# fabianschenk/REVO

Hardware: AMD Instinct MI355X
Metric: tracked frames/sec at 640x480, 4-level pyramid; ATE vs reference (higher is better)
Workload: dtype f32

## Files before the change

### revo_amd/csrc/revo_batch.hip

```cpp
#include "revo_host_impl.h"

static bool env_defer() {
  return env_int("REVO_EDT_DEFER", 1, 0, 1) && env_int("REVO_DEFER", 2, 0, 3) != 0;
}
extern "C" int revo_batch_create(revo_ctx* c, int n_pairs, revo_batch** out) {
  if (!c || !out || n_pairs <= 0) return fail(REVO_ERR_INVALID_ARG, "bad argument");
  HIPCHECK(hipSetDevice(c->device));
  Partial<revo_batch> b(new revo_batch());
  b->ctx.hold(c); b->n_pairs = n_pairs;
  { FrameSet* fs = nullptr; TRY(frameset_create(c, 2 * n_pairs, false, &fs)); b->fs.reset(fs); }
  TRY(b->stream.create());
  TRY(b->ev0.create(hipEventDefault)); TRY(b->ev1.create(hipEventDefault));
  TRY(b->descs.create());
  TRY(b->trk.create());
  b->cluster = pick_cluster(c, n_pairs);
  b->defer = env_defer();
  TRY(b->d_mail.alloc(mail_bytes(n_pairs, b->cluster) / sizeof(unsigned long long)));
  HIPCHECK(hipMemset(b->d_mail, 0, mail_bytes(n_pairs, b->cluster)));
  for (int f = 0; f < 2 * n_pairs; ++f) b->views.push_back(revo_pyr{c, b->fs.get(), f, false, (f % 2) == 0, 0.0, false, false});
  TRY(b->descs.reserve(n_pairs, b->stream));
  TRY(b->h_flags.alloc(n_pairs));
  for (int i = 0; i < n_pairs; ++i) fill_desc(&b->descs.h[i], &b->views[2 * i], &b->views[2 * i + 1], nullptr, nullptr);
  HIPCHECK(hipStreamSynchronize(c->stream));
  HIPCHECK(hipStreamSynchronize(nullptr));
  *out = b.release();
  return REVO_OK;
}
revo_batch::~revo_batch() {
  hipSetDevice(ctx->device);
  if (stream) hipStreamSynchronize(stream);
}
extern "C" void revo_batch_destroy(revo_batch* b) {
  if (b) HandleDelete()(b);
}

static int batch_wait_tracker(revo_batch* b, hipStream_t s) { return b->trk.wait_elsewhere(s); }
static int batch_wait_build(revo_batch* b, hipStream_t s) {
  return b->defer ? REVO_OK : b->fs->ready.wait_elsewhere(s);
}
static int batch_mark_tracker(revo_batch* b, hipStream_t s) { return b->trk.record(s); }

static int enqueue_batch_tail(revo_batch* b, hipStream_t s) {
  const PyrGeom& g = b->ctx->geom;
  if (b->defer) {
    std::lock_guard<std::mutex> lk(b->fs->edt_mu);
    b->fs->edt_pending = true; b->fs->edt_count = b->n_pairs;
    b->fs->ref_lists_pending = true;
  } else {
    launch_tile_points(g, b->fs->p, b->fs->B, s);
    launch_keyframe(g, b->fs->p, 0, 2, b->n_pairs, s);
  }
  return REVO_OK;
}

static int batch_build(revo_batch* b, const uint8_t* d_bgr, const float* d_depth, const uint16_t* d_depth_u16, float alpha,
                       void* stream, bool borrow) {
  HIPCHECK(hipSetDevice(b->ctx->device));
  hipStream_t s = stream ? (hipStream_t)stream : b->stream;
  TRY(wait_edt_before_rebuild(b->fs.get(), s));
  TRY(batch_wait_tracker(b, s));
  enqueue_build(b->ctx, b->fs.get(), d_bgr, d_depth, d_depth_u16, alpha, s, borrow, false, 0, -1, b->defer);
  TRY(enqueue_batch_tail(b, s));
  HIPCHECK(hipGetLastError());
  TRY(b->fs->mark_built(s));
  for (auto& v : b->views) { v.table_built = false; v.ref_list_built = false; }
  return REVO_OK;
}
static int batch_build_f32(revo_batch* b, const uint8_t* d_bgr, const float* d_depth, void* stream, bool borrow) {
  if (!b || !d_bgr || !d_depth) return fail(REVO_ERR_INVALID_ARG, "null argument");
  return batch_build(b, d_bgr, d_depth, nullptr, 0.f, stream, borrow);
}
extern "C" int revo_batch_build(revo_batch* b, const uint8_t* d_bgr, const float* d_depth, void* stream) {
  return batch_build_f32(b, d_bgr, d_depth, stream, false);
}
extern "C" int revo_batch_build_borrow(revo_batch* b, const uint8_t* d_bgr, const float* d_depth, void* stream) {
  return batch_build_f32(b, d_bgr, d_depth, stream, true);
}

static int batch_upload_init(revo_batch* b, const float* h_init_RT, hipStream_t s) {
  if (!h_init_RT && b->identity_uploaded) return REVO_OK;
  b->identity_uploaded = (h_init_RT == nullptr);
  TRY(b->descs.reserve(b->n_pairs, s));
  for (int i = 0; i < b->n_pairs; ++i) {
    PairDesc& d = b->descs.h[i];
    if (h_init_RT) { memcpy(d.R, h_init_RT + 12 * i, sizeof(float) * 9); memcpy(d.T, h_init_RT + 12 * i + 9, sizeof(float) * 3); }
    else { memset(d.R, 0, sizeof(d.R)); d.R[0] = d.R[4] = d.R[8] = 1.f; memset(d.T, 0, sizeof(d.T)); }
  }
  return b->descs.upload(b->n_pairs, s);
}

extern "C" int revo_batch_prepare(revo_batch* b, void* stream) {
  if (!b) return fail(REVO_ERR_INVALID_ARG, "null argument");
  HIPCHECK(hipSetDevice(b->ctx->device));
  hipStream_t s = stream ? (hipStream_t)stream : b->stream;
  return run_pending_edt(b->ctx, b->fs.get(), s);
}

extern "C" int revo_batch_track_only(revo_batch* b, const float* h_init_RT, revo_pair_result* d_results, void* stream) {
  if (!b || !d_results) return fail(REVO_ERR_INVALID_ARG, "null argument");
  HIPCHECK(hipSetDevice(b->ctx->device));
  hipStream_t s = stream ? (hipStream_t)stream : b->stream;
  TRY(batch_wait_tracker(b, s));
  int rc = batch_upload_init(b, h_init_RT, s);
  if (rc) return rc;
  TrackParams tp = b->ctx->tp;
  tp.eval_only = 0;
  TRY(batch_wait_build(b, s));
  TRY(run_pending_edt(b->ctx, b->fs.get(), s));
  b->last_results = d_results;
  rc = chained_track_launch(b->ctx->device, b->ctx->knobs.track_depth, s, [&](unsigned* d_resident) {
    if (b->tev0) (void)hipEventRecord(b->tev0, s);
    const int n_wg = launch_track(b->descs.d, tp, d_results, nullptr, b->n_pairs, b->d_mail, &b->mail_epoch, b->cluster, d_resident, s);
    if (b->tev1) (void)hipEventRecord(b->tev1, s);
    b->tev0 = b->tev1 = nullptr;
    return n_wg;
  });
  if (rc) return rc;
  return batch_mark_tracker(b, s);
}
extern "C" void revo_batch_time_next_grid_(revo_batch* b, void* ev0, void* ev1) {
  if (b) { b->tev0 = (hipEvent_t)ev0; b->tev1 = (hipEvent_t)ev1; }
}

extern "C" int revo_batch_build_u16(revo_batch* b, const uint8_t* d_bgr, const uint16_t* d_depth_raw,
                                    double depth_scale_factor, void* stream) {
  if (!b || !d_bgr || !d_depth_raw) return fail(REVO_ERR_INVALID_ARG, "null argument");
  if (!(depth_scale_factor > 0.0)) return fail(REVO_ERR_INVALID_ARG, "depth_scale_factor must be positive");
  return batch_build(b, d_bgr, nullptr, d_depth_raw, (float)(1.0f / depth_scale_factor), stream, false);
}

extern "C" int revo_batch_track(revo_batch* b, const uint8_t* d_bgr, const float* d_depth, const float* h_init_RT,
                                revo_pair_result* d_results, void* stream) {
  int rc = revo_batch_build(b, d_bgr, d_depth, stream);
  if (rc) return rc;
  return revo_batch_track_only(b, h_init_RT, d_results, stream);
}

extern "C" int revo_batch_sync(revo_batch* b, void* stream) {
  if (!b) return fail(REVO_ERR_INVALID_ARG, "null batch");
  HIPCHECK(hipSetDevice(b->ctx->device));
  hipStream_t s = stream ? (hipStream_t)stream : b->stream;
  HIPCHECK(hipStreamSynchronize(s));
  if (b->fs->edt_pending) { int rc2 = run_pending_edt(b->ctx, b->fs.get(), s); if (rc2) return rc2; HIPCHECK(hipStreamSynchronize(s)); }
// ... 1 lines not shown
    TRY(batch_wait_tracker(b, s));
    HIPCHECK(hipMemcpyAsync(b->h_flags, b->last_results, sizeof(revo_pair_result) * b->n_pairs, hipMemcpyDeviceToHost, s));
    HIPCHECK(hipStreamSynchronize(s));
    b->last_results = nullptr;
    for (int i = 0; i < b->n_pairs; ++i)
      if (b->h_flags[i].flags & 8)
        return fail(REVO_ERR_HIP, "tracker: pair " + std::to_string(i) + ": the workgroups of the pair could not exchange "
                    "partial sums in time (device shared with another process?) -- its pose is not valid");
  }
  return REVO_OK;
}

int infows_create(int n, bool own_out, std::unique_ptr<InfoWs>* out) {
  Partial<InfoWs> w(new InfoWs());
  w->n = n;
  TRY(w->descs.reserve(n, nullptr));
  TRY(w->rt.reserve(n, nullptr));
  TRY(w->d_part.alloc(INFO_PART_DOUBLES * INFO_MAX_GROUPS * (size_t)n));
  TRY(w->d_cnt.alloc(INFO_MAX_GROUPS * (size_t)n));
  TRY(w->d_ticket.alloc(align_up((size_t)n, 4)));
  if (own_out) {
    TRY(w->d_out.alloc(n));
    TRY(w->h_out.alloc(n));
  }
  TRY(w->rt.create());
  TRY(w->ev_done.create());
  out->reset(w.release());
  return REVO_OK;
}
InfoParams info_params(const TrackParams& tp, int lvl) {
  InfoParams ip;
  ip.fx = tp.cam[lvl].fx; ip.fy = tp.cam[lvl].fy; ip.cx = tp.cam[lvl].cx; ip.cy = tp.cam[lvl].cy;
  ip.w = tp.cam[lvl].w; ip.h = tp.cam[lvl].h;
  ip.edge_distance = tp.edge_distance[lvl]; ip.huber_edge = tp.huber_edge;
  ip.use_edge_filter = tp.use_edge_filter; ip.level = lvl;
  return ip;
}
int infows_upload_rt(InfoWs* w, int n, const float* h_RT, hipStream_t s) {
  TRY(w->rt.reserve(n, s));
  for (int i = 0; i < n; ++i) {
    memcpy(w->rt.h[i].v, h_RT + 12 * i, sizeof(float) * 12);
    memset(w->rt.h[i].v + 12, 0, sizeof(float) * 4);
  }
  return w->rt.upload(n, s);
}

extern "C" int revo_batch_pair_info(revo_batch* b, const revo_pair_result* d_results, const float* h_RT, int lvl,
                                    revo_pair_info* d_info, void* stream) {
  if (!b || !d_info) return fail(REVO_ERR_INVALID_ARG, "null argument");
  if ((d_results != nullptr) == (h_RT != nullptr)) return fail(REVO_ERR_INVALID_ARG, "exactly one of d_results and h_RT must be given");
  if ((uintptr_t)d_info % 16) return fail(REVO_ERR_INVALID_ARG, "d_info is not 16-byte aligned");
  revo_ctx* c = b->ctx;
  if (lvl < 0 || lvl >= c->geom.n_levels) return fail(REVO_ERR_LEVEL, "level out of range");
  HIPCHECK(hipSetDevice(c->device));
  hipStream_t s = stream ? (hipStream_t)stream : b->stream;
  if (!b->info_ws) {
    TRY(infows_create(b->n_pairs, false, &b->info_ws));
    HIPCHECK(hipMemcpy(b->info_ws->descs.d, b->descs.h, sizeof(PairDesc) * b->n_pairs, hipMemcpyHostToDevice));
  }
  InfoWs* w = b->info_ws.get();
  TRY(batch_wait_tracker(b, s));
  if (h_RT) TRY(infows_upload_rt(w, b->n_pairs, h_RT, s));
  TRY(batch_wait_build(b, s));
  TRY(run_pending_edt(c, b->fs.get(), s));
  InfoParams ip;
  { std::lock_guard<std::mutex> lk(c->mu); ip = info_params(c->tp, lvl); }
  launch_pair_info(w->descs.d, h_RT ? (const void*)w->rt.d : (const void*)d_results, h_RT ? 16 : (int)(sizeof(revo_pair_result) / 4),
                   h_RT ? 12 : (int)(offsetof(revo_pair_result, flags) / 4), ip, b->n_pairs, w->d_part, w->d_cnt, w->d_ticket, d_info, s);
  HIPCHECK(hipGetLastError());
  return batch_mark_tracker(b, s);
}

extern "C" int revo_batch_profile_build(revo_batch* b, const uint8_t* d_bgr, const float* d_depth, int reps, revo_stage_times* out) {
  if (!b || !d_bgr || !d_depth || !out || reps <= 0) return fail(REVO_ERR_INVALID_ARG, "bad argument");
  revo_ctx* c = b->ctx;
  HIPCHECK(hipSetDevice(c->device));
  hipStream_t s = b->stream;
  TRY(wait_edt_before_rebuild(b->fs.get(), s));
  TRY(batch_wait_tracker(b, s));
  memset(out, 0, sizeof(*out));
  PyrGeom g = c->geom;
  g.frame0 = 0;
  FrameSet* fs = b->fs.get();
  const int B = fs->B, L = g.n_levels;
  fs->p.depth[0] = const_cast<float*>(d_depth);
  struct Stage { const char* name; int a, w; };
  std::vector<Stage> st;
  st.push_back({"k_gray_depth", 0, 0});
  for (int l = 1; l < L; ++l) st.push_back({"k_pyrdown_gray", l, 1});
  st.push_back({"k_canny_nms4", 0, 0});
  st.push_back({"hysteresis", 0, 0});
  st.push_back({"k_fill", 0, 0});
  const bool stage = c->knobs.stage_edge_depths && fs->p.stage[0] != nullptr && L > 1;
  PyrGeom gp = g;
  gp.pts_staged = stage ? 1 : 0;
  if (stage) st.push_back({"k_edge_prefix", 0, 0});
  for (int l = 1; l < L; ++l) st.push_back({"k_pyrdown_depth", l, 2});
  st.push_back({"k_tile_count", 0, 1});
  st.push_back({"k_pts_tiles", 0, 2});
  st.push_back({"k_edt_cols", 0, 1});
  st.push_back({"k_edt_rows", 0, 2});
  const int n = (int)st.size();
  if (n > REVO_MAX_STAGES) return fail(REVO_ERR_CAPACITY, "too many stages");
  std::vector<OwnedEvent> ev(n + 1);
  for (auto& e : ev) TRY(e.create(hipEventDefault));
  std::vector<double> sum(n, 0.0);
  for (int r = 0; r < reps; ++r) {
    HIPCHECK(hipEventRecord(ev[0], s));
    for (int i = 0; i < n; ++i) {
      const std::string nm = st[i].name;
      if (nm == "k_gray_depth") launch_gray_depth(g, fs->p, d_bgr, d_depth, nullptr, 0.f, B, s);
      else if (nm == "k_pyrdown_gray") launch_pyrdown(g, fs->p, st[i].a, B, s, 1);
      else if (nm == "k_pyrdown_depth") launch_pyrdown(g, fs->p, st[i].a, B, s, 2, stage);
      else if (nm == "k_edge_prefix") launch_edge_prefix(g, fs->p, B, s);
      else if (nm == "k_canny_nms4") launch_canny_nms(g, fs->p, B, s);
      else if (nm == "hysteresis") launch_hyst(g, fs->p, B, s);
      else if (nm == "k_fill") launch_fill(g, fs->p, B, s);
      else if (nm == "k_tile_count" || nm == "k_pts_tiles") launch_tile_points(gp, fs->p, B, s, st[i].w);
      else launch_keyframe(g, fs->p, 0, 2, b->n_pairs, s, st[i].w);
      HIPCHECK(hipGetLastError());
      HIPCHECK(hipEventRecord(ev[i + 1], s));
    }
    HIPCHECK(hipStreamSynchronize(s));
    for (int i = 0; i < n; ++i) {
      float ms = 0.f;
      HIPCHECK(hipEventElapsedTime(&ms, ev[i], ev[i + 1]));
      sum[i] += ms * 1e3;
    }
  }
  out->n = n;
  for (int i = 0; i < n; ++i) {
    out->us[i] = (float)(sum[i] / reps);
    if (std::string(st[i].name).rfind("k_pyrdown", 0) == 0) snprintf(out->name[i], sizeof(out->name[i]), "%s[%d]", st[i].name, st[i].a);
    else snprintf(out->name[i], sizeof(out->name[i]), "%s", st[i].name);
  }
  {
    std::lock_guard<std::mutex> lk(fs->edt_mu);
    fs->edt_pending = false;
    fs->ref_lists_pending = false;
    TRY(fs->edt.record(s));
    fs->ref.recorded = false;
  }
  TRY(fs->mark_built(s));
  for (auto& v : b->views) { v.table_built = false; v.ref_list_built = false; }
  return REVO_OK;
}

extern "C" int revo_batch_frame(revo_batch* b, int frame, revo_pyr** out) {
  if (!b || !out || frame < 0 || frame >= 2 * b->n_pairs) return fail(REVO_ERR_INVALID_ARG, "bad frame index");
  *out = &b->views[frame];
  return REVO_OK;
}

extern "C" int revo_batch_time_tracker(revo_batch* b, const float* h_init_RT, revo_pair_result* d_results, void* stream,
                                       int reps, float* ms_mean) {
  if (!b || !d_results || !ms_mean || reps <= 0) return fail(REVO_ERR_INVALID_ARG, "bad argument");
  HIPCHECK(hipSetDevice(b->ctx->device));
  hipStream_t s = stream ? (hipStream_t)stream : b->stream;
  TRY(batch_wait_tracker(b, s));
  int rc = batch_upload_init(b, h_init_RT, s);
  if (rc) return rc;
  TrackParams tp = b->ctx->tp;
  tp.eval_only = 0;
  TRY(batch_wait_build(b, s));
  TRY(run_pending_edt(b->ctx, b->fs.get(), s));
  float total = 0.f;
  for (int r = 0; r < reps; ++r) {
    HIPCHECK(hipEventRecord(b->ev0, s));
    rc = chained_track_launch(b->ctx->device, b->ctx->knobs.track_depth, s, [&](unsigned* d_resident) {
      return launch_track(b->descs.d, tp, d_results, nullptr, b->n_pairs, b->d_mail, &b->mail_epoch, b->cluster, d_resident, s);
    });
    if (rc) return rc;
    HIPCHECK(hipEventRecord(b->ev1, s));
    HIPCHECK(hipEventSynchronize(b->ev1));
    float ms = 0.f;
    HIPCHECK(hipEventElapsedTime(&ms, b->ev0, b->ev1));
    total += ms;
  }
  *ms_mean = total / (float)reps;
  return batch_mark_tracker(b, s);
}
```

### revo_amd/csrc/revo_dev.h

```cpp
#pragma once
#include <hip/hip_runtime.h>
#include <stdint.h>
#include "../../include/revo_hip.h"

#define REVO_L REVO_MAX_LEVELS

struct LevelGeom {
  int w, h;
  int npix;
  float fx, fy, cx, cy;
  int patch;
  int hist_w, hist_h;
  int nchunk;
  int chunk_rows;
  int wpr;
  int nms_block_base;
  int has_orig;
  int pix_base;
  int edt_rows;
  int edt_block_base;
  int strip_base;
  int cc_base;
  int band_rows, nbands, band_base;
};

struct PyrGeom {
  int frame0;
  int fstride;
  int n_levels;
  int total_nms_blocks, total_pix, total_edt_blocks, total_strips, total_cc;
  int total_bands, any_banded;
  int hyst_force;
  int hyst_heavy_runs;
  int total_tiles;
  int pts_staged;
  float depth_min, depth_max;
  int canny_low, canny_high;
  int use_edge_hist;
  float n_percentage;
  double fill_thr[REVO_L];
  LevelGeom lv[REVO_L];
};

struct FramePlanes {
  uint8_t* gray[REVO_L];
  float* depth[REVO_L];
  uint2* cs[REVO_L];
  uint8_t* edges[REVO_L];
  uint8_t* edges_orig[REVO_L];
  int* scratch[REVO_L];
  float4* pts[REVO_L];
  float4* pts_trk[REVO_L];
  float* dt[REVO_L];
  float4* table[REVO_L];
  uint8_t* hist[REVO_L];
  int* chunk[REVO_L];
  unsigned* cmask[REVO_L];
  uint8_t* vb[REVO_L];
  int* npts;
  int* hist_nz;
  int* strip_tot;
  uint32_t* ebits[REVO_L];
  int* need_full;
  int* hyst_heavy;
  int* tile_base;
  float* stage[REVO_L];
  unsigned short* epre[REVO_L];
  int* stage_base;
};

struct PairDesc {
  const float4* pts[REVO_L];
  const int* npts;
  const float* dt[REVO_L];
  float R[9];
  float T[3];
};

struct TrackParams {
  int pyr_min_lvl, pyr_max_lvl;
  int lvl_begin, lvl_end;
  int check_init;
  int eval_only;
  int kspec[REVO_L];
  int redundant_n;
  float lambda_success_fac, lambda_fail_fac;
  float lambda_initial[REVO_L], step_size_min[REVO_L], convergence_eps[REVO_L];
  int max_its[REVO_L];
  float edge_distance[REVO_L];
  float huber_edge;
  int use_edge_filter;
  struct { float fx, fy, cx, cy; int w, h; } cam[REVO_L];
  int exact_sums;
};

struct EvalOut {
  float A[36];
  float b[6];
  float error;
  float mean_err;
  float sum_w, sum_u;
  int good, bad;
};

#define REVO_MAX_WIDTH 2048
#define NMS_ROWS 6
#define EDT_ROW_PX 1280
#define EDT_ROW_THREADS (EDT_ROW_PX / 4)
#ifndef REVO_HYST_LDS_MAX
#define REVO_HYST_LDS_MAX 158720
#endif
#ifndef TRACK_THREADS
#define TRACK_THREADS 512
#endif
#ifndef TRACK_MAX_CLUSTER
#define TRACK_MAX_CLUSTER 32
#endif
#define TRACK_KMAX 4
#define TRACK_NVAL 48
#define TRACK_NVAL_X 132
#define TRACK_MAIL_NVAL TRACK_NVAL_X

void launch_gray_depth(const PyrGeom& g, const FramePlanes& p, const uint8_t* d_bgr, const float* d_depth_f32,
                       const uint16_t* d_depth_u16, float u16_alpha, int B, hipStream_t s);
void launch_pyrdown(const PyrGeom& g, const FramePlanes& p, int lvl, int B, hipStream_t s, int parts = 3, bool stage_edges = false);
void launch_edge_prefix(const PyrGeom& g, const FramePlanes& p, int B, hipStream_t s);
void launch_canny_nms(const PyrGeom& g, const FramePlanes& p, int B, hipStream_t s);
void launch_hyst(const PyrGeom& g, const FramePlanes& p, int B, hipStream_t s);
void launch_fill(const PyrGeom& g, const FramePlanes& p, int B, hipStream_t s);
void launch_compact(const PyrGeom& g, const FramePlanes& p, int B, hipStream_t s);
void launch_tile_points(const PyrGeom& g, const FramePlanes& p, int B, hipStream_t s, int which = 3);
void launch_pyrdown_bgr(const uint8_t* src, int w, int h, uint8_t* dst, hipStream_t s);
void launch_colored_pcl(const PyrGeom& g, const FramePlanes& p, int frame, int lvl, int dense, const uint8_t* bgr_lvl,
                        int* chunk, unsigned* cmask, int* total, int cap, float* out8, hipStream_t s);
void launch_keyframe(const PyrGeom& g, const FramePlanes& p, int f0, int fstride, int count, hipStream_t s, int which = 3);
int launch_track(const PairDesc* d_descs, const TrackParams& prm, revo_pair_result* d_out, EvalOut* d_eval,
                 int n_pairs, unsigned long long* d_mail, unsigned* epoch_io, int cluster, unsigned* d_resident, hipStream_t s);
void launch_track_gate(unsigned* d_resident, unsigned want, hipStream_t s);
int launch_track_one(const PairDesc& desc, const TrackParams& prm, revo_pair_result* out, EvalOut* eval_out,
                     unsigned long long* d_mail, unsigned* epoch_io, int cluster, unsigned* seq_ptr, unsigned seq_val,
                     unsigned* d_resident, hipStream_t s);
void launch_solve6(const float* d_Ab , int n, float* d_x , hipStream_t s);
int track_blocks_per_cu();
void launch_grad_table(const PyrGeom& g, const FramePlanes& p, int f0, int fstride, int count, hipStream_t s);
struct VoteArgs { float RT[3][12]; const float4* pts[3]; const int* n[3]; };
void launch_vote(const PyrGeom& g, const FramePlanes& curr, int curr_frame, int lvl, int n_clouds, const VoteArgs& va,
                 int* d_marks , int* d_hist8 , unsigned* d_done ,
                 int* h_out8 , unsigned seq_val, int use_orig_edges,
                 hipStream_t s);
void launch_copy_cloud(float4* dst, const float4* src, int* dst_n, const int* src_n, hipStream_t s);
struct VoteDesc {
  float RT[3][12]; const float4* pts[3]; const int* n[3]; int n_clouds;
  const uint8_t* edges; const float* depth;
  int* marks; int* hist8; unsigned* done;
  int* host_out;
};
struct CloudCopyDesc { float4* dst; const float4* src; int* dst_n; const int* src_n; };
struct CopySeg { const void* src; void* dst; size_t bytes; };
void launch_vote_multi(const PyrGeom& g, int lvl, int n, const VoteDesc* d_descs, unsigned seq_val, hipStream_t s);
void launch_copy_cloud_multi(int n, const CloudCopyDesc* d_descs, hipStream_t s);
void launch_copy_segments(int n, const CopySeg* d_segs, hipStream_t s);

#define INFO_THREADS 256
#define INFO_CHUNK 1024
#define INFO_MAX_GROUPS 32
#define INFO_PART_DOUBLES 64
struct InfoParams {
  float fx, fy, cx, cy;
  int w, h;
  float edge_distance, huber_edge;
  int use_edge_filter, level;
};
static inline int info_groups(int npix) {
  const int g = (npix + 8 * INFO_CHUNK - 1) / (8 * INFO_CHUNK);
  return g < 1 ? 1 : (g > INFO_MAX_GROUPS ? INFO_MAX_GROUPS : g);
}
void launch_pair_info(const PairDesc* d_descs, const void* d_pose, int pose_stride, int flag_word, const InfoParams& prm,
                      int n_pairs, double* d_part, int* d_cnt, unsigned* d_ticket, revo_pair_info* d_out, hipStream_t s);
```

### revo_amd/csrc/revo_frame.hip

```cpp
#include "revo_host_impl.h"

typedef unsigned v4u __attribute__((ext_vector_type(4)));
__global__ void __launch_bounds__(256) k_upload_rows(uint8_t* __restrict__ dst, const uint8_t* __restrict__ src, size_t src_stride,
                                                     size_t row_bytes, int rows) {
  const size_t vec = row_bytes / 16, tail0 = vec * 16;
  for (int y = blockIdx.y; y < rows; y += gridDim.y) {
    const uint8_t* s = src + (size_t)y * src_stride;
    uint8_t* d = dst + (size_t)y * row_bytes;
    const bool aligned = (((uintptr_t)s | (uintptr_t)d) & 15) == 0;
    if (aligned) {
      for (size_t i = blockIdx.x * blockDim.x + threadIdx.x; i < vec; i += (size_t)gridDim.x * blockDim.x)
        ((v4u*)d)[i] = __builtin_nontemporal_load((const v4u*)s + i);
      for (size_t i = tail0 + blockIdx.x * blockDim.x + threadIdx.x; i < row_bytes; i += (size_t)gridDim.x * blockDim.x) d[i] = s[i];
    } else {
      for (size_t i = blockIdx.x * blockDim.x + threadIdx.x; i < row_bytes; i += (size_t)gridDim.x * blockDim.x) d[i] = s[i];
    }
  }
}
static hipError_t upload_rows(void* dst, const void* src, size_t src_stride, size_t row_bytes, int rows, int max_blocks, hipStream_t s) {
  void* dsrc = nullptr;
  hipError_t e = hipHostGetDevicePointer(&dsrc, const_cast<void*>(src), 0);
  if (e != hipSuccess) { (void)hipGetLastError(); return e; }
  if (src_stride == row_bytes) {
    const size_t bytes = row_bytes * rows;
// ... 41 lines not shown
    std::lock_guard<std::mutex> lk(c->mu);
    c->framesets_created += 1;
  }
  const size_t brow = (size_t)w * 3, drow = (size_t)w * (is_u16 ? 2 : 4);
  hipStream_t bs = c->build_stream;
  auto page_locked = [](const void* p) {
    hipPointerAttribute_t at;
    if (hipPointerGetAttributes(&at, p) != hipSuccess) { (void)hipGetLastError(); return false; }
    return at.type == hipMemoryTypeHost;
  };
  const bool direct = c->knobs.direct_h2d && page_locked(bgr) && page_locked(depth) &&
                      page_locked(bgr + (size_t)(h - 1) * bgr_stride + brow - 1) &&
                      page_locked((const char*)depth + (size_t)(h - 1) * depth_stride + drow - 1);
  sec.lap(1);
  if (direct) {
    {
      std::lock_guard<std::mutex> lk(c->mu);
      if (!c->frame_copy_stream) TRY(c->frame_copy_stream.create());
    }
    TRY(fs->h2d.create());
    hipStream_t cs = c->frame_copy_stream;
    TRY(fs->ready.wait(cs));
    TRY(fs->wait_previous_users(cs));
    sec.lap(6);
    if (c->knobs.h2d_kernel && upload_rows(fs->d_bgr, bgr, bgr_stride, brow, h, c->knobs.upload_blocks, cs) == hipSuccess) {}
    else if (bgr_stride == brow) HIPCHECK(hipMemcpyAsync(fs->d_bgr, bgr, brow * h, hipMemcpyHostToDevice, cs));
    else HIPCHECK(hipMemcpy2DAsync(fs->d_bgr, brow, bgr, bgr_stride, brow, h, hipMemcpyHostToDevice, cs));
    sec.lap(7);
    if (c->knobs.h2d_kernel && upload_rows(fs->d_depth, depth, depth_stride, drow, h, c->knobs.upload_blocks, cs) == hipSuccess) {}
    else if (depth_stride == drow) HIPCHECK(hipMemcpyAsync(fs->d_depth, depth, drow * h, hipMemcpyHostToDevice, cs));
    else HIPCHECK(hipMemcpy2DAsync(fs->d_depth, drow, depth, depth_stride, drow, h, hipMemcpyHostToDevice, cs));
    sec.lap(8);
    HIPCHECK(hipEventRecord(fs->h2d, cs));
    sec.lap(9);
    HIPCHECK(hipStreamWaitEvent(bs, fs->h2d, 0));
    sec.lap(2);
    TRY(wait_event_polled(fs->h2d));
    sec.lap(3);
  } else {
    TRY(fs->ready.sync());
    for (int y = 0; y < h; ++y) memcpy(fs->h_bgr + (size_t)y * brow, bgr + (size_t)y * bgr_stride, brow);
    for (int y = 0; y < h; ++y) memcpy((char*)fs->h_depth.p + (size_t)y * drow, (const char*)depth + (size_t)y * depth_stride, drow);
    TRY(fs->wait_previous_users(bs));
    HIPCHECK(hipMemcpyAsync(fs->d_bgr, fs->h_bgr, brow * h, hipMemcpyHostToDevice, bs));
    HIPCHECK(hipMemcpyAsync(fs->d_depth, fs->h_depth, drow * h, hipMemcpyHostToDevice, bs));
  }
  const float alpha = is_u16 ? (float)(1.0f / scale) : 0.0f;
  enqueue_build(c, fs, fs->d_bgr, is_u16 ? nullptr : fs->d_depth, is_u16 ? (const uint16_t*)fs->d_depth : nullptr, alpha, bs, true);
  HIPCHECK(hipGetLastError());
  TRY(fs->mark_built(bs));
  sec.lap(4);
  revo_pyr* p = new revo_pyr{c, fs, 0, true, false, ts, false, false};
  ctx_ref(c);
  *out = p;
  return REVO_OK;
}

extern "C" int revo_pyramid_create(revo_ctx* ctx, const uint8_t* bgr, size_t bgr_stride, const float* depth_m,
                                   size_t depth_stride, double timestamp, revo_pyr** out) {
  return pyramid_create_common(ctx, bgr, bgr_stride, depth_m, depth_stride, false, 1.0, timestamp, out);
}
extern "C" int revo_pyramid_create_u16(revo_ctx* ctx, const uint8_t* bgr, size_t bgr_stride, const uint16_t* depth_raw,
                                       size_t depth_stride, double depth_scale_factor, double timestamp, revo_pyr** out) {
  if (!(depth_scale_factor > 0)) return fail(REVO_ERR_INVALID_ARG, "depth_scale_factor must be > 0");
  return pyramid_create_common(ctx, bgr, bgr_stride, depth_raw, depth_stride, true, depth_scale_factor, timestamp, out);
}

extern "C" void revo_pyramid_destroy(revo_pyr* p) {
  if (!p) return;
  if (p->owns_fs) {
    hipSetDevice(p->ctx->device);
    std::lock_guard<std::mutex> lk(p->ctx->mu);
    p->fs->release_to(p->ctx->pool, p->ctx->stream, p->ctx->vote_stream);
  }
  revo_ctx* c = p->owns_fs ? p->ctx : nullptr;
  delete p;
  if (c) ctx_unref(c);
}

extern "C" int revo_pyramid_make_keyframe(revo_pyr* p) {
  if (!p) return fail(REVO_ERR_INVALID_ARG, "null pyramid");
  HIPCHECK(hipSetDevice(p->ctx->device));
  TRY(wait_ready(p->ctx, p));
  if (!p->dt_ready) launch_keyframe(p->ctx->geom, p->fs->p, p->frame, 1, 1, p->ctx->stream);
  HIPCHECK(hipGetLastError());
  p->dt_ready = false;
  p->is_kf = true;
  p->table_built = false;
  return REVO_OK;
}
extern "C" int revo_pyramid_prepare_keyframe_(revo_pyr* p) {
  if (!p) return fail(REVO_ERR_INVALID_ARG, "null pyramid");
  if (!p->owns_fs || p->is_kf || p->dt_ready) return REVO_OK;
  HIPCHECK(hipSetDevice(p->ctx->device));
  TRY(wait_ready(p->ctx, p));
  launch_keyframe(p->ctx->geom, p->fs->p, p->frame, 1, 1, p->ctx->stream);
  HIPCHECK(hipGetLastError());
  p->dt_ready = true;
  return REVO_OK;
}
extern "C" int revo_pyramid_is_keyframe(const revo_pyr* p) { return p && p->is_kf; }
extern "C" double revo_pyramid_timestamp(const revo_pyr* p) { return p ? p->ts : 0.0; }

extern "C" int revo_pyramid_read(revo_pyr* p, revo_plane what, int lvl, void* dst, size_t cap, size_t* count) {
  if (!p) return fail(REVO_ERR_INVALID_ARG, "null pyramid");
  revo_ctx* c = p->ctx;
  HIPCHECK(hipSetDevice(c->device));
  if (lvl < 0 || lvl >= c->geom.n_levels) return fail(REVO_ERR_LEVEL, "level out of range");
  const LevelGeom& v = c->geom.lv[lvl];
  const FramePlanes& P = p->fs->p;
  const size_t f = (size_t)p->frame;
  TRY(wait_ready(c, p));
  HIPCHECK(hipStreamSynchronize(c->stream));
  const void* src = nullptr;
  size_t n = v.npix, esz = 1;
  switch (what) {
    case REVO_PLANE_GRAY: src = P.gray[lvl] + f * v.npix; break;
    case REVO_PLANE_DEPTH: src = P.depth[lvl] + f * v.npix; esz = 4; break;
    case REVO_PLANE_EDGES: src = P.edges[lvl] + f * v.npix; break;
    case REVO_PLANE_EDGES_ORIG:
      src = (v.has_orig ? P.edges_orig[lvl] : P.edges[lvl]) + f * v.npix;
      break;
    case REVO_PLANE_DT:
      if (!p->is_kf) return fail(REVO_ERR_NOT_KEYFRAME, "distance transform not built: call makeKeyframe");
      src = P.dt[lvl] + f * v.npix; esz = 4; break;
    case REVO_PLANE_GRADTABLE:
      if (!p->is_kf) return fail(REVO_ERR_NOT_KEYFRAME, "optimizationStructure not built");
      if (!p->table_built) {
        launch_grad_table(c->geom, P, p->frame, 1, 1, c->stream);
        HIPCHECK(hipGetLastError());
        HIPCHECK(hipStreamSynchronize(c->stream));
        p->table_built = true;
      }
      src = P.table[lvl] + f * v.npix; esz = 16; break;
    case REVO_PLANE_EDGES3D: {
      if (!p->ref_list_built) {
        PyrGeom g1 = c->geom;
        g1.frame0 = p->frame;
        launch_compact(g1, P, 1, c->stream);
        HIPCHECK(hipGetLastError());
        HIPCHECK(hipStreamSynchronize(c->stream));
        p->ref_list_built = true;
      }
      int np = 0;
      HIPCHECK(hipMemcpy(&np, P.npts + f * REVO_L + lvl, sizeof(int), hipMemcpyDeviceToHost));
      n = (size_t)np; src = P.pts[lvl] + f * v.npix; esz = 16; break;
    }
    case REVO_PLANE_EDGES3D_TILED: {
      int np = 0;
      HIPCHECK(hipMemcpy(&np, P.npts + f * REVO_L + lvl, sizeof(int), hipMemcpyDeviceToHost));
      n = (size_t)np; src = P.pts_trk[lvl] + f * v.npix; esz = 16; break;
    }
    case REVO_PLANE_HIST:
      if (v.patch <= 0) { n = 0; src = P.hist[lvl]; break; }
      n = (size_t)v.hist_w * v.hist_h; src = P.hist[lvl] + f * n; break;
    default: return fail(REVO_ERR_INVALID_ARG, "unknown plane");
  }
  if (count) *count = n;
  if (dst) {
    if (n * esz > cap) return fail(REVO_ERR_CAPACITY, "host buffer too small");
    if (n) HIPCHECK(hipMemcpy(dst, src, n * esz, hipMemcpyDeviceToHost));
  }
  return REVO_OK;
}

extern "C" int revo_pyramid_colored_pcl(revo_pyr* p, int lvl, int dense, float* dst8, size_t cap_points, size_t* count) {
  if (!p) return fail(REVO_ERR_INVALID_ARG, "null pyramid");
  revo_ctx* c = p->ctx;
  HIPCHECK(hipSetDevice(c->device));
  if (lvl < 0 || lvl >= c->geom.n_levels) return fail(REVO_ERR_LEVEL, "level out of range");
  if (!(p->owns_fs || p->has_colour) || !p->fs->d_bgr)
    return fail(REVO_ERR_INVALID_ARG, "batch views keep no colour image (rgbFullSize): use revo_pyramid_create");
  TRY(wait_ready(c, p));
  std::lock_guard<std::mutex> lk(c->mu);
  const PyrGeom& g = c->geom;
  const size_t n0 = g.lv[0].npix, slots = (size_t)g.lv[0].w * g.lv[0].nchunk;
  if (!c->d_pcl) {
    size_t off = 0;
    auto take = [&](size_t bytes) { size_t o = off; off += (bytes + 255) & ~(size_t)255; return o; };
    const size_t o_out = take(n0 * 32), o_a = take(n0 / 4 * 3 + 3), o_b = take(n0 / 16 * 3 + 3), o_ch = take(slots * 4),
                 o_m = take(slots * 4), o_t = take(4);
    TRY(c->d_pcl.alloc(off));
    c->d_pcl_out = (float*)(c->d_pcl + o_out);
    c->d_pcl_clr[0] = (uint8_t*)(c->d_pcl + o_a); c->d_pcl_clr[1] = (uint8_t*)(c->d_pcl + o_b);
    c->d_pcl_chunk = (int*)(c->d_pcl + o_ch); c->d_pcl_mask = (unsigned*)(c->d_pcl + o_m); c->d_pcl_total = (int*)(c->d_pcl + o_t);
  }
  hipStream_t s = c->stream;
  const uint8_t* clr = p->fs->d_bgr + (size_t)p->frame * n0 * 3;
  for (int l = 0; l < lvl; ++l) {
    uint8_t* d = c->d_pcl_clr[l & 1];
    launch_pyrdown_bgr(clr, g.lv[l].w, g.lv[l].h, d, s);
    clr = d;
  }
  const int cap = (int)std::min<size_t>(dst8 ? cap_points : 0, (size_t)g.lv[lvl].npix);
  launch_colored_pcl(g, p->fs->p, p->frame, lvl, dense ? 1 : 0, clr, c->d_pcl_chunk, c->d_pcl_mask, c->d_pcl_total,
                     dst8 ? cap : g.lv[lvl].npix, c->d_pcl_out, s);
  HIPCHECK(hipGetLastError());
  int total = 0;
  HIPCHECK(hipMemcpyAsync(&total, c->d_pcl_total, sizeof(int), hipMemcpyDeviceToHost, s));
  HIPCHECK(hipStreamSynchronize(s));
  if (count) *count = (size_t)total;
  if (dst8) {
    if ((size_t)total > cap_points) return fail(REVO_ERR_CAPACITY, "host buffer too small");
    if (total) HIPCHECK(hipMemcpy(dst8, c->d_pcl_out, (size_t)total * 32, hipMemcpyDeviceToHost));
  }
  return REVO_OK;
}

extern "C" int revo_map_source_(revo_pyr* p, MapSource* out) {
  if (!p || !out) return fail(REVO_ERR_INVALID_ARG, "null pyramid");
  revo_ctx* c = p->ctx;
  HIPCHECK(hipSetDevice(c->device));
  if (!(p->owns_fs || p->has_colour) || !p->fs->d_bgr)
    return fail(REVO_ERR_INVALID_ARG, "batch views keep no colour image (rgbFullSize): use revo_pyramid_create");
  TRY(wait_ready(c, p));
  const size_t n0 = c->geom.lv[0].npix, f = (size_t)p->frame;
  out->ctx = c;
  out->depth = p->fs->p.depth[0] + f * n0;
  out->edges = p->fs->p.edges[0] + f * n0;
  out->bgr = p->fs->d_bgr + f * n0 * 3;
  return REVO_OK;
}
extern "C" int revo_map_source_kind_(const revo_pyr* p, const revo_ctx** ctx, int* batch_view) {
  if (!p || !ctx || !batch_view) return fail(REVO_ERR_INVALID_ARG, "null pyramid");
  *ctx = p->ctx;
  *batch_view = (!(p->owns_fs || p->has_colour) || !p->fs->d_bgr) ? 1 : 0;
  return REVO_OK;
}
extern "C" int revo_map_ctx_geom_(const revo_ctx* c, MapCtxGeom* out) {
  if (!c || !out) return fail(REVO_ERR_INVALID_ARG, "null context");
  const LevelGeom& l = c->geom.lv[0];
  *out = MapCtxGeom{c->device, l.w, l.h, l.fx, l.fy, l.cx, l.cy, c->geom.depth_min, c->geom.depth_max, (void*)c->stream};
  return REVO_OK;
}
```

### revo_amd/csrc/revo_host.hip

```cpp
#include "revo_host_impl.h"

static thread_local std::string g_err;
extern "C" const char* revo_last_error(void) { return g_err.c_str(); }
extern "C" const char* revo_version(void) { return "0.1.0 gfx950"; }
extern "C" void revo_set_error_(const char* msg) { g_err = msg ? msg : ""; }

extern "C" void revo_pyr_settings_default(revo_pyr_settings* s) {
  memset(s, 0, sizeof(*s));
  s->width = 640; s->height = 480;
  s->fx = 517.306408f; s->fy = 516.469215f; s->cx = 318.643040f; s->cy = 255.313989f;
  s->pyr_min_lvl = 2; s->pyr_max_lvl = 0;
  s->canny_threshold1 = 150; s->canny_threshold2 = 100;
  s->depth_min = 0.1f; s->depth_max = 5.2f;
  s->use_edge_hist = 1; s->n_percentage = 0.3f;
  s->hist_patch[0] = 20; s->hist_patch[1] = 10; s->hist_patch[2] = 5;
}
extern "C" void revo_opt_settings_default(revo_opt_settings* s) {
  memset(s, 0, sizeof(*s));
  s->lambda_success_fac = 0.5f; s->lambda_fail_fac = 2.0f;
  const float ed[6] = {30, 20, 10, 5, 5, 5};
  for (int i = 0; i < REVO_L; ++i) {
    s->lambda_initial[i] = 0.f; s->step_size_min[i] = 1e-16f; s->convergence_eps[i] = 0.999f;
    s->max_its_per_lvl[i] = 100; s->edge_distance_lvl[i] = ed[i];
  }
// ... 161 lines not shown
  const int prev = (int)((ch.n + TRACK_MAX_DEPTH - 1) % TRACK_MAX_DEPTH), cur = (int)(ch.n % TRACK_MAX_DEPTH);
  if (depth > 1 && ch.n > 0 && ch.has[prev] && ch.st[prev] != s) launch_track_gate(ch.d_resident, ch.started_total, s);
  const int n_wg = launch(f, ch.d_resident);
  HIPCHECK(hipGetLastError());
  ch.started_total += (unsigned)n_wg;
  HIPCHECK(hipEventRecord(ch.ev[cur], s));
  ch.has[cur] = true;
  ch.st[cur] = s;
  ch.n += 1;
  return REVO_OK;
}
extern "C" int revo_debug_gate_timeouts_(int device) {
  TrackChain& ch = g_chain[device & 63];
  std::lock_guard<std::mutex> lk(ch.mu);
  if (!ch.d_resident) return -1;
  unsigned v = 0;
  if (hipMemcpy(&v, ch.d_resident + 1, sizeof(unsigned), hipMemcpyDeviceToHost) != hipSuccess) return -2;
  return (int)v;
}
extern "C" int revo_debug_census_(int device, unsigned out3[3]) {
  TrackChain& ch = g_chain[device & 63];
  std::lock_guard<std::mutex> lk(ch.mu);
  if (!ch.d_resident || !out3) return -1;
  if (hipMemcpy(out3, ch.d_resident, 2 * sizeof(unsigned), hipMemcpyDeviceToHost) != hipSuccess) return -2;
  out3[2] = ch.started_total;
  return 0;
}
int frameset_create(revo_ctx* c, int B, bool with_staging, FrameSet** out, bool host_staging) {
  const PyrGeom& g = c->geom;
  Partial<FrameSet> fs(new FrameSet());
  fs->B = B;
  for (int pass = 0; pass < 2; ++pass) {
    size_t off = 0;
    auto take = [&](size_t bytes) -> void* {
      void* p = pass ? (void*)(fs->blob + off) : nullptr;
      off = align_up(off + bytes, 256);
      return p;
    };
    for (int l = 0; l < g.n_levels; ++l) {
      const LevelGeom& v = g.lv[l];
      const size_t n = (size_t)v.npix * B;
      fs->p.gray[l] = (uint8_t*)take(n);
      fs->p.depth[l] = (float*)take(n * 4);
      fs->p.cs[l] = (uint2*)take((size_t)v.h * v.wpr * 8 * B);
      fs->p.edges[l] = (uint8_t*)take(n);
      fs->p.edges_orig[l] = (uint8_t*)take(n);
      fs->p.scratch[l] = (int*)take(n * 4);
      fs->p.pts[l] = (float4*)take(n * 16);
      fs->p.pts_trk[l] = (float4*)take(n * 16);
      fs->p.dt[l] = (float*)take(n * 4);
      fs->p.table[l] = (float4*)take(n * 16);
      fs->p.hist[l] = (uint8_t*)take((size_t)std::max(1, v.hist_w * v.hist_h) * B);
      fs->p.chunk[l] = (int*)take((size_t)v.w * v.nchunk * B * 4);
      fs->p.cmask[l] = (unsigned*)take((size_t)v.w * v.nchunk * B * 4);
      fs->p.vb[l] = (uint8_t*)take((n + 7) / 8);
      fs->p.ebits[l] = (uint32_t*)take((size_t)v.h * v.wpr * 4 * B);
      if (B > 1 && l < g.n_levels - 1) {
        fs->p.stage[l] = (float*)take(n * 4);
        fs->p.epre[l] = (unsigned short*)take((size_t)v.h * v.wpr * 2 * B);
      }
    }
    fs->own_depth0 = fs->p.depth[0];
    fs->p.npts = (int*)take(sizeof(int) * REVO_L * B);
    fs->p.hist_nz = (int*)take(sizeof(int) * REVO_L * B);
    fs->p.strip_tot = (int*)take(sizeof(int) * (size_t)g.total_strips * B);
    fs->p.tile_base = (int*)take(sizeof(int) * (size_t)g.total_tiles * B);
    fs->p.need_full = (int*)take(sizeof(int) * REVO_L * B);
    fs->p.hyst_heavy = (int*)take(sizeof(int) * B);
    fs->p.stage_base = (int*)take(sizeof(int) * (size_t)g.total_tiles * B);
    if (with_staging) {
      fs->d_bgr = (uint8_t*)take((size_t)g.lv[0].npix * 3 * B);
      fs->d_depth = (float*)take((size_t)g.lv[0].npix * 4 * B);
    }
    if (!pass) {
      fs->blob_bytes = off;
      hipError_t e = hipMalloc((void**)&fs->blob.p, off);
      if (e != hipSuccess) return fail(REVO_ERR_HIP, std::string("hipMalloc: ") + hipGetErrorString(e));
    }
  }
  if (with_staging && host_staging) {
    TRY(fs->h_bgr.alloc((size_t)g.lv[0].npix * 3 * B));
    TRY(fs->h_depth.alloc((size_t)g.lv[0].npix * B));
  }
  for (StreamMark* m : {&fs->ready, &fs->free_trk, &fs->free_vote, &fs->edt, &fs->ref}) TRY(m->create());
  hipMemsetAsync(fs->p.npts, 0, sizeof(int) * REVO_L * B, c->stream);
  HIPCHECK(hipStreamSynchronize(c->stream));
  *out = fs.release();
  return REVO_OK;
}

void enqueue_build(revo_ctx* c, FrameSet* fs, const uint8_t* d_bgr, const float* d_depth_f32, const uint16_t* d_depth_u16,
                   float alpha, hipStream_t s, bool borrow_depth, bool with_points, int frame0, int nframes, bool gray_only) {
  PyrGeom g = c->geom;
  g.frame0 = frame0;
  const int B = nframes < 0 ? fs->B : nframes;
  fs->p.depth[0] = (borrow_depth && d_depth_f32) ? const_cast<float*>(d_depth_f32) : fs->own_depth0;
  launch_gray_depth(g, fs->p, d_bgr, d_depth_f32, d_depth_u16, alpha, B, s);
  for (int l = 1; l < g.n_levels; ++l) launch_pyrdown(g, fs->p, l, B, s, gray_only ? 1 : 3);
  launch_canny_nms(g, fs->p, B, s);
  launch_hyst(g, fs->p, B, s);
  launch_fill(g, fs->p, B, s);
  if (with_points) launch_tile_points(g, fs->p, B, s);
}

extern "C" int revo_ctx_create(int device, const revo_pyr_settings* pyr, const revo_opt_settings* opt,
                               const revo_tracker_settings* trk, revo_ctx** out) {
  if (!pyr || !out) return fail(REVO_ERR_INVALID_ARG, "null argument");
  int ndev = 0;
  if (hipGetDeviceCount(&ndev) != hipSuccess || ndev <= 0)
    return fail(REVO_ERR_HIP, "no HIP device: librevo_hip has no CPU fallback");
  if (device < 0 || device >= ndev) return fail(REVO_ERR_INVALID_ARG, "device ordinal out of range");
  HIPCHECK(hipSetDevice(device));
  Partial<revo_ctx> owner(new revo_ctx());
  revo_ctx* c = owner.get();
  c->device = device;
  c->ps = *pyr;
  c->knobs.track_depth = env_track_depth();
  c->knobs.cluster_one = env_int("REVO_TRACK_CLUSTER_ONE", 0, 0, TRACK_MAX_CLUSTER);
  c->knobs.redundant_one = env_int("REVO_TRACK_REDUNDANT_ONE", 1024, 0, 1 << 30);
  c->knobs.direct_h2d = env_int("REVO_DIRECT_H2D", 1, 0, 1);
  c->knobs.stage_edge_depths = env_int("REVO_STAGE_EDGE_DEPTHS", 0, 0, 1);
  {
    const char* e1 = getenv("REVO_TRACK_KSPEC_ONE");
    const char* eb = getenv("REVO_TRACK_KSPEC");
    const size_t n1 = e1 ? strlen(e1) : 0;
    c->knobs.kspec_one_set = n1 > 0 || !(eb && *eb);
    for (int i = 0; i < REVO_L; ++i) {
      int k = i < 2 ? 3 : TRACK_KMAX;
      if (n1 == 1) k = e1[0] - '0'; else if (n1 > 1) k = e1[std::min<size_t>(i, n1 - 1)] - '0';
      c->knobs.kspec_one[i] = std::max(1, std::min(TRACK_KMAX, k));
    }
  }
  c->knobs.upload_blocks = env_int("REVO_UPLOAD_BLOCKS", 64, 1, 4096);
  c->knobs.h2d_kernel = env_int("REVO_H2D_KERNEL", 0, 0, 1);
  c->knobs.h2d_max_run_mb = env_int("REVO_H2D_MAX_RUN_MB", 64, 1, 4096);
  if (opt) c->os = *opt; else revo_opt_settings_default(&c->os);
  if (trk) c->ts = *trk; else revo_tracker_settings_default(&c->ts);
  std::string why;
  if (build_geom(c->ps, &c->geom, &why)) return fail(REVO_ERR_INVALID_ARG, why);
  build_track_params(c, &c->tp);
  TRY(c->stream.create());
  TRY(c->build_stream.create());
  TRY(c->vote_stream.create());
  TRY(c->ev_vote.create());
  TRY(c->h_desc.alloc(1));
  TRY(c->h_res.alloc(3));
  TRY(c->h_seq.alloc(4));
  memset(c->h_seq, 0, sizeof(unsigned) * 4);
  TRY(c->h_eval.alloc(1));
  hipDeviceProp_t prop;
  HIPCHECK(hipGetDeviceProperties(&prop, device));
  c->num_cus = prop.multiProcessorCount;
  c->blocks_per_cu = std::min(track_blocks_per_cu(), 2);
  TRY(c->d_mail.alloc(mail_bytes(1, TRACK_MAX_CLUSTER) / sizeof(unsigned long long)));
  HIPCHECK(hipMemset(c->d_mail, 0, mail_bytes(1, TRACK_MAX_CLUSTER)));
  size_t maxpix = 0;
  for (int l = 0; l < c->geom.n_levels; ++l) maxpix = std::max(maxpix, (size_t)c->geom.lv[l].npix);
  TRY(c->d_marks.alloc(maxpix));
  TRY(c->d_hist8.alloc(8));
  TRY(c->d_vote_done.alloc(1));
  HIPCHECK(hipMemset(c->d_marks, 0, sizeof(int) * maxpix));
  HIPCHECK(hipMemset(c->d_hist8, 0, sizeof(int) * 8));
  HIPCHECK(hipMemset(c->d_vote_done, 0, sizeof(unsigned)));
  TRY(c->h_hist8.alloc(16));
  memset(c->h_hist8, 0, sizeof(int) * 16);
  HIPCHECK(hipDeviceSynchronize());
  *out = owner.release();
  return REVO_OK;
}

revo_ctx::~revo_ctx() {
  hipSetDevice(device);
  for (hipStream_t s : {(hipStream_t)build_stream, (hipStream_t)stream, (hipStream_t)vote_stream, (hipStream_t)frame_copy_stream})
    if (s) (void)hipStreamSynchronize(s);
  for (auto& p : past) past_free(p);
  for (auto& p : past_pool) past_free(p);
  for (FrameSet* fs : pool) delete fs;
}
void ctx_ref(revo_ctx* c) { c->refs.fetch_add(1); }
void ctx_unref(revo_ctx* c) { if (c->refs.fetch_sub(1) == 1) HandleDelete()(c); }
extern "C" void revo_ctx_destroy(revo_ctx* c) {
  if (!c) return;
  pairs_jobs_release(c);
  ctx_unref(c);
}
extern "C" int revo_ctx_reserve_framesets_(revo_ctx* c, int total) {
  if (!c) return fail(REVO_ERR_INVALID_ARG, "null context");
  HIPCHECK(hipSetDevice(c->device));
  for (;;) {
    {
      std::lock_guard<std::mutex> lk(c->mu);
      if (c->framesets_created >= total) return REVO_OK;
      c->framesets_created += 1;
    }
    FrameSet* fs = nullptr;
    const int rc = frameset_create(c, 1, true, &fs);
    std::lock_guard<std::mutex> lk(c->mu);
    if (rc) { c->framesets_created -= 1; return rc; }
    c->pool.push_back(fs);
  }
}
extern "C" int revo_ctx_device_(const revo_ctx* c) { return c ? c->device : -1; }
extern "C" void revo_ctx_retain_(revo_ctx* c) { if (c) ctx_ref(c); }
extern "C" void revo_ctx_release_(revo_ctx* c) { if (c) ctx_unref(c); }

extern "C" int revo_ctx_set_tracker(revo_ctx* c, const revo_opt_settings* opt, const revo_tracker_settings* trk) {
  if (!c) return fail(REVO_ERR_INVALID_ARG, "null context");
  std::lock_guard<std::mutex> lk(c->mu);
  if (opt) c->os = *opt;
  if (trk) c->ts = *trk;
  const int exact = c->tp.exact_sums;
  build_track_params(c, &c->tp);
  c->tp.exact_sums = exact;
  while (!c->past.empty()) { c->past_pool.push_back(c->past.front()); c->past.pop_front(); }
  return REVO_OK;
}

extern "C" int revo_ctx_histogram_level(const revo_ctx* c) { return c ? c->ts.histogram_level : -1; }

extern "C" int revo_ctx_set_exact_sums(revo_ctx* c, int on) {
  if (!c) return fail(REVO_ERR_INVALID_ARG, "null context");
  std::lock_guard<std::mutex> lk(c->mu);
  c->tp.exact_sums = on ? 1 : 0;
  return REVO_OK;
}
extern "C" int revo_ctx_exact_sums(const revo_ctx* c) { return c ? c->tp.exact_sums : -1; }

extern "C" int revo_ctx_camera(const revo_ctx* c, int lvl, float out6[6]) {
  if (!c || !out6) return fail(REVO_ERR_INVALID_ARG, "null argument");
  if (lvl < 0 || lvl >= c->geom.n_levels) return fail(REVO_ERR_LEVEL, "level out of range");
  const LevelGeom& v = c->geom.lv[lvl];
  out6[0] = v.fx; out6[1] = v.fy; out6[2] = v.cx; out6[3] = v.cy; out6[4] = (float)v.w; out6[5] = (float)v.h;
  return REVO_OK;
}

static void enqueue_list_side(revo_ctx* c, FrameSet* fs, int f0, int fstride, int count, hipStream_t s) {
  PyrGeom gp = c->geom;
  gp.frame0 = f0; gp.fstride = fstride;
  const bool stage = c->knobs.stage_edge_depths && fs->p.stage[0] != nullptr && c->geom.n_levels > 1;
  if (stage) launch_edge_prefix(gp, fs->p, count, s);
  for (int l = 1; l < c->geom.n_levels; ++l) launch_pyrdown(gp, fs->p, l, count, s, 2, stage);
  gp.pts_staged = stage ? 1 : 0;
  launch_tile_points(gp, fs->p, count, s);
}
int run_pending_edt(revo_ctx* c, FrameSet* fs, hipStream_t s, bool need_ref_lists) {
  std::lock_guard<std::mutex> lk(fs->edt_mu);
  bool behind_build = false;
  if (!fs->edt_pending) {
    TRY(fs->edt.wait_elsewhere(s));
  } else {
    TRY(fs->ready.wait(s));
    behind_build = true;
    enqueue_list_side(c, fs, 1, 2, fs->edt_count, s);
    launch_keyframe(c->geom, fs->p, 0, 2, fs->edt_count, s);
    HIPCHECK(hipGetLastError());
    TRY(fs->edt.record(s));
    fs->edt_pending = false;
  }
  if (!need_ref_lists) return REVO_OK;
  if (!fs->ref_lists_pending) return fs->ref.wait_elsewhere(s);
  if (!behind_build) TRY(fs->ready.wait(s));
  enqueue_list_side(c, fs, 0, 2, fs->edt_count, s);
  HIPCHECK(hipGetLastError());
  TRY(fs->ref.record(s));
  fs->ref_lists_pending = false;
  return REVO_OK;
}
int wait_edt_before_rebuild(FrameSet* fs, hipStream_t s) {
  std::lock_guard<std::mutex> lk(fs->edt_mu);
  TRY(fs->edt.wait_elsewhere(s));
  return fs->ref.wait_elsewhere(s);
}
int wait_event_polled(hipEvent_t ev) {
  const auto t0 = std::chrono::steady_clock::now();
  for (unsigned spin = 0;; ++spin) {
    const hipError_t e = hipEventQuery(ev);
    if (e == hipSuccess) return REVO_OK;
    if (e != hipErrorNotReady) { (void)hipGetLastError(); return fail(REVO_ERR_HIP, std::string("hipEventQuery: ") + hipGetErrorString(e)); }
    (void)hipGetLastError();
    for (int k = 0; k < 32; ++k) __builtin_ia32_pause();
    if ((spin & 1023) == 1023 && std::chrono::steady_clock::now() - t0 > std::chrono::seconds(2)) break;
  }
  HIPCHECK(hipEventSynchronize(ev));
  return REVO_OK;
}
static std::atomic<unsigned long long> g_wait_fallbacks{0}, g_wait_max_ns{0}, g_wait_calls{0};
extern "C" void revo_debug_wait_stats_(unsigned long long out[3]) {
  out[0] = g_wait_calls.load(); out[1] = g_wait_fallbacks.load(); out[2] = g_wait_max_ns.load();
}
int wait_seq(hipStream_t s, volatile unsigned* word, unsigned want) {
  static const int spin_limit = env_int("REVO_WAIT_SPINS", 200000, 1000, 2000000000);
  const auto t0 = std::chrono::steady_clock::now();
  g_wait_calls.fetch_add(1, std::memory_order_relaxed);
  auto note = [&]() {
    const unsigned long long ns = (unsigned long long)std::chrono::duration_cast<std::chrono::nanoseconds>(std::chrono::steady_clock::now() - t0).count();
    unsigned long long cur = g_wait_max_ns.load(std::memory_order_relaxed);
    while (ns > cur && !g_wait_max_ns.compare_exchange_weak(cur, ns)) {}
  };
  for (int spin = 0; spin < spin_limit; ++spin) {
    if (*word == want) { std::atomic_thread_fence(std::memory_order_acquire); note(); return REVO_OK; }
    __builtin_ia32_pause();
  }
  g_wait_fallbacks.fetch_add(1, std::memory_order_relaxed);
  HIPCHECK(hipStreamSynchronize(s));
  note();
  if (*word != want) return fail(REVO_ERR_HIP, "a kernel finished without publishing its result");
  return REVO_OK;
}
```

### revo_amd/csrc/revo_host_impl.h

```cpp
#pragma once
#include <hip/hip_runtime.h>

#include <cmath>
#include <cstdio>
#include <chrono>
#include <cstring>
#include <atomic>
#include <deque>
#include <mutex>
#include <string>
#include <vector>

#include "revo_dev.h"
#include "revo_internal.h"
#include "revo_mat4.h"
#include "revo_multi.h"
#include "revo_map.h"

struct FrameSet {
  int B = 0;
  DevMem<char> blob;
  size_t blob_bytes = 0;
  FramePlanes p{};
  float* own_depth0 = nullptr;
  uint8_t* d_bgr = nullptr;
  float* d_depth = nullptr;
  PinnedMem<uint8_t> h_bgr;
  PinnedMem<float> h_depth;
  StreamMark ready;
  std::mutex edt_mu;
  std::atomic<bool> edt_pending{false};
  int edt_count = 0;
  StreamMark edt;
  std::atomic<bool> ref_lists_pending{false};
  StreamMark ref;
  StreamMark free_trk;
  StreamMark free_vote;
  OwnedEvent h2d;
  int wait_previous_users(hipStream_t s) const { TRY(free_trk.wait(s)); return free_vote.wait(s); }
  int mark_built(hipStream_t s) { return ready.record(s); }
  void release_to(std::vector<FrameSet*>& pool, hipStream_t trk, hipStream_t vote) {
    (void)free_trk.record(trk);
    (void)free_vote.record(vote);
    pool.push_back(this);
  }
};

struct InfoRt { float v[16]; };
struct InfoWs {
  int n = 0;
  HostRows<PairDesc> descs;
  HostRows<InfoRt> rt;
  DevMem<double> d_part; DevMem<int> d_cnt; DevMem<unsigned> d_ticket;
  DevMem<revo_pair_info> d_out; PinnedMem<revo_pair_info> h_out;
  OwnedEvent ev_done;
};

struct Past {
  float4* d_pts; int* d_n; int n; float T_w[16]; double ts;
  size_t cap;
};

struct Knobs {
  int track_depth;
  int cluster_one;
  int redundant_one;
  int direct_h2d;
  int h2d_max_run_mb;
  bool kspec_one_set;
  int kspec_one[REVO_L];
  int upload_blocks;
  int h2d_kernel;
  int stage_edge_depths;
};

struct revo_ctx {
  std::atomic<int> refs{1};
  int device;
  Knobs knobs;
  revo_pyr_settings ps; revo_opt_settings os; revo_tracker_settings ts;
  PyrGeom geom;
  TrackParams tp;
  std::mutex mu;
  int framesets_created = 0;
  unsigned seq_next = 1;
  unsigned mail_epoch = 0;
  int num_cus, blocks_per_cu;
  unsigned long long jobs_submitted = 0;
  float* d_pcl_out; uint8_t* d_pcl_clr[2]; int* d_pcl_chunk; unsigned* d_pcl_mask; int* d_pcl_total;
  OwnedStream stream;
  std::unique_ptr<InfoWs> info_ws;
  DevMem<char> d_pcl;
  DevMem<unsigned> d_vote_done; PinnedMem<int> h_hist8; DevMem<int> d_hist8; DevMem<int> d_marks;
  DevMem<unsigned long long> d_mail;
  PinnedMem<unsigned> h_seq;
  PinnedMem<EvalOut> h_eval;
  PinnedMem<revo_pair_result> h_res;
  PinnedMem<PairDesc> h_desc;
  std::vector<FrameSet*> pool;
  OwnedStream build_stream;
  std::vector<Past> past_pool;
  std::deque<Past> past;
  OwnedStream frame_copy_stream;
  std::vector<struct revo_pairs_job*> jobs;
  OwnedStream copy_stream2, copy_stream, pair_streams[2];
  OwnedEvent ev_vote;
  OwnedStream vote_stream;
  ~revo_ctx();
};
void ctx_ref(revo_ctx* c);
void ctx_unref(revo_ctx* c);
struct CtxRef {
  revo_ctx* c = nullptr;
  ~CtxRef() { if (c) ctx_unref(c); }
  void hold(revo_ctx* x) { ctx_ref(x); c = x; }
  revo_ctx* operator->() const { return c; }
  operator revo_ctx*() const { return c; }
};

struct revo_pyr {
  revo_ctx* ctx;
  FrameSet* fs;
  int frame;
  bool owns_fs;
  bool is_kf;
  double ts;
  bool table_built;
  bool ref_list_built;
  bool dt_ready = false;
  bool has_colour = false;
};

struct revo_batch {
  CtxRef ctx;
  int n_pairs = 0;
  std::unique_ptr<FrameSet> fs;
  std::vector<revo_pyr> views;
  OwnedStream stream;
  StreamMark trk;
  OwnedEvent ev1, ev0;
  std::unique_ptr<InfoWs> info_ws;
  DevMem<unsigned long long> d_mail;
  HostRows<PairDesc> descs;
  PinnedMem<revo_pair_result> h_flags;
  unsigned mail_epoch = 0;
  bool identity_uploaded = false;
  int cluster = 1;
  bool defer = true;
  hipEvent_t tev0 = nullptr, tev1 = nullptr;
  const revo_pair_result* last_results = nullptr;
  ~revo_batch();
};

int pick_cluster(const revo_ctx* c, int n_pairs);
int chained_track_launch_(int device, int depth, hipStream_t s, int (*launch)(void* f, unsigned* d_resident), void* f);
template <typename F>
int chained_track_launch(int device, int depth, hipStream_t s, F&& launch) {
  return chained_track_launch_(device, depth, s, [](void* f, unsigned* d) { return (*(std::remove_reference_t<F>*)f)(d); }, (void*)&launch);
}
int wait_seq(hipStream_t s, volatile unsigned* word, unsigned want);
int wait_event_polled(hipEvent_t ev);
int frameset_create(revo_ctx* c, int B, bool with_staging, FrameSet** out, bool host_staging = true);
void enqueue_build(revo_ctx* c, FrameSet* fs, const uint8_t* d_bgr, const float* d_depth_f32, const uint16_t* d_depth_u16,
                   float alpha, hipStream_t s, bool borrow_depth = false, bool with_points = true, int frame0 = 0,
                   int nframes = -1, bool gray_only = false);
int run_pending_edt(revo_ctx* c, FrameSet* fs, hipStream_t s, bool need_ref_lists = false);
int wait_edt_before_rebuild(FrameSet* fs, hipStream_t s);
int decode_track(const revo_pair_result& r, float R[9], float T[3], float* err, int* status, revo_residual_info* info, int32_t* iters);
int past_take(std::vector<Past>& pool, size_t need, size_t cap, Past* out, bool newest = false);
void past_free(Past& p);
int infows_create(int n, bool own_out, std::unique_ptr<InfoWs>* out);
InfoParams info_params(const TrackParams& tp, int lvl);
int infows_upload_rt(InfoWs* w, int n, const float* h_RT, hipStream_t s);
void pairs_jobs_release(revo_ctx* c);

inline size_t align_up(size_t v, size_t a) { return (v + a - 1) / a * a; }
inline size_t mail_bytes(int n_pairs, int cluster) { return sizeof(unsigned long long) * (size_t)n_pairs * 2 * cluster * TRACK_MAIL_NVAL; }

inline void fill_desc(PairDesc* d, const revo_pyr* ref, const revo_pyr* curr, const float* R, const float* T) {
  const PyrGeom& g = ref->ctx->geom;
  memset(d, 0, sizeof(*d));
  for (int l = 0; l < g.n_levels; ++l) {
    d->pts[l] = curr->fs->p.pts_trk[l] + (size_t)curr->frame * g.lv[l].npix;
    d->dt[l] = ref->fs->p.dt[l] + (size_t)ref->frame * g.lv[l].npix;
  }
  d->npts = curr->fs->p.npts + (size_t)curr->frame * REVO_L;
  if (R) memcpy(d->R, R, sizeof(float) * 9); else { d->R[0] = d->R[4] = d->R[8] = 1.f; }
  if (T) memcpy(d->T, T, sizeof(float) * 3);
}

inline int check_pair(const revo_ctx* c, const revo_pyr* ref, const revo_pyr* curr) {
  if (!c || !ref || !curr) return fail(REVO_ERR_INVALID_ARG, "null argument");
  if (ref->ctx != c || curr->ctx != c) return fail(REVO_ERR_INVALID_ARG, "pyramid belongs to another context");
  if (!ref->is_kf) return fail(REVO_ERR_NOT_KEYFRAME, "optimizationStructure not built! (reference frame is not a keyframe)");
  return REVO_OK;
}

inline int wait_ready_on(revo_ctx* c, const revo_pyr* p, hipStream_t s) {
  TRY(p->fs->ready.wait(s));
  return run_pending_edt(c, p->fs, s, (p->frame & 1) == 0);
}
inline int wait_ready(revo_ctx* c, const revo_pyr* p) { return wait_ready_on(c, p, c->stream); }

struct RowCopier {
  hipMemcpyKind kind; int rows; hipStream_t stream; size_t max_run;
  char* dst = nullptr; const char* src = nullptr; size_t bytes = 0;
  hipError_t flush() {
    if (!bytes) return hipSuccess;
    const hipError_t e = hipMemcpyAsync(dst, src, bytes, kind, stream);
    bytes = 0;
    return e;
  }
  hipError_t add(void* d, const void* s, size_t src_stride, size_t row_bytes) {
    if (src_stride != row_bytes) {
      const hipError_t e = flush();
      if (e != hipSuccess) return e;
      return hipMemcpy2DAsync(d, row_bytes, s, src_stride, row_bytes, rows, kind, stream);
    }
    const size_t n = row_bytes * rows;
    if (bytes && bytes + n <= max_run && src + bytes == (const char*)s && dst + bytes == (char*)d) { bytes += n; return hipSuccess; }
    const hipError_t e = flush();
    if (e != hipSuccess) return e;
    dst = (char*)d; src = (const char*)s; bytes = n;
    return hipSuccess;
  }
};

inline void vote_cloud_pose(const float inv[16], const Past& past, float RT[12]) {
  float tf[16];
  mat4_mul(inv, past.T_w, tf);
  for (int cc = 0; cc < 3; ++cc) for (int r = 0; r < 3; ++r) RT[cc * 3 + r] = tf[cc * 4 + r];
  RT[9] = tf[12]; RT[10] = tf[13]; RT[11] = tf[14];
}
inline int vote_decide(const int32_t ov[4], int nframes, float* ratio) {
  const float wts[4] = {0.f, 1.f, 1.25f, 1.5f};
  float overlapMeasure = 0.0f;
  const int hsize = 1 + nframes;
  for (int k = 1; k < hsize; ++k) overlapMeasure += (ov[k] * wts[k]);
  if (ratio) *ratio = nframes >= 3 && ov[0] > 0 ? overlapMeasure / (float)ov[0] : INFINITY;
  return (overlapMeasure >= ov[0] || hsize < 4) ? REVO_TRACKER_STATE_OK : REVO_TRACKER_STATE_NEW_KF;
}
```

### revo_amd/csrc/revo_mdev.hip

```cpp
#include "revo_host_impl.h"

struct revo_mdev {
  CtxRef c;
  int S = 0, cluster = 1, hl = 0;
  TrackParams tp;
  revo_tracker_settings ts;
  std::vector<revo_pyr> kf_views;
  std::vector<FrameSet*> pool, all;
  unsigned mail_epoch = 0;
  unsigned seq = 0;
  std::vector<std::deque<Past>> past;
  std::vector<Past> past_pool;
  size_t cloud_cap = 0;
  OwnedEvent ev_trk, ev_h2d, ev_prod;
  std::unique_ptr<InfoWs> info_ws;
  HostRows<CopySeg> segs;
  HostRows<CloudCopyDesc> cdesc;
  PinnedMem<int> h_vout;
  DevMem<unsigned> d_done; DevMem<int> d_hist8; DevMem<int> d_marks;
  HostRows<VoteDesc> vdesc;
  DevMem<unsigned long long> d_mail;
  PinnedMem<revo_pair_result> h_res; DevMem<revo_pair_result> d_res;
  HostRows<PairDesc> descs;
  std::unique_ptr<FrameSet> kf;
// ... 101 lines not shown
  hipSetDevice(c->device);
  fs->release_to(m->pool, c->stream, c->vote_stream);
}

extern "C" int revo_mdev_track_(revo_mdev* m, int n, MultiTrack* pairs) {
  if (n <= 0) return REVO_OK;
  revo_ctx* c = m->c;
  HIPCHECK(hipSetDevice(c->device));
  hipStream_t s = c->stream;
  FrameSet* waited[64];
  int nw = 0;
  for (int i = 0; i < n; ++i) {
    FrameSet* fs = (FrameSet*)pairs[i].set;
    const revo_pyr curr{c, fs, pairs[i].frame, false, false, 0.0, false, false};
    fill_desc(&m->descs.h[i], &m->kf_views[pairs[i].stream], &curr, pairs[i].R, pairs[i].T);
    bool seen = false;
    for (int k = 0; k < nw && !seen; ++k) seen = waited[k] == fs;
    if (!seen) {
      TRY(fs->ready.wait(s));
      if (nw < 64) waited[nw++] = fs;
    }
  }
  TRY(m->descs.upload(n, s, false));
  if (m->mail_epoch > 0xffffffffu - 4 * 8192u) {
    HIPCHECK(hipMemsetAsync(m->d_mail, 0, mail_bytes(m->S, m->cluster), s));
    m->mail_epoch = 0;
  }
  int rc = chained_track_launch(c->device, c->knobs.track_depth, s, [&](unsigned* d_resident) {
    return launch_track(m->descs.d, m->tp, m->d_res, nullptr, n, m->d_mail, &m->mail_epoch, m->cluster, d_resident, s);
  });
  if (rc) return rc;
  HIPCHECK(hipMemcpyAsync(m->h_res, m->d_res, sizeof(revo_pair_result) * n, hipMemcpyDeviceToHost, s));
  HIPCHECK(hipEventRecord(m->ev_trk, s));
  if ((rc = wait_event_polled(m->ev_trk))) return rc;
  for (int i = 0; i < n; ++i) {
    const revo_pair_result& r = m->h_res[i];
    if (r.flags & 8)
      return fail(REVO_ERR_HIP, "tracker: stream " + std::to_string(pairs[i].stream) + ": the workgroups of the pair could not exchange "
                  "partial sums in time (device shared with another process?) -- its pose is not valid");
    if ((rc = decode_track(r, pairs[i].R, pairs[i].T, nullptr, &pairs[i].status, nullptr, nullptr))) return rc;
  }
  return REVO_OK;
}

extern "C" int revo_mdev_pair_info_enqueue_(revo_mdev* m, int n) {
  if (n <= 0) return REVO_OK;
  revo_ctx* c = m->c;
  HIPCHECK(hipSetDevice(c->device));
  if (!m->info_ws) TRY(infows_create(m->S, true, &m->info_ws));
  InfoWs* w = m->info_ws.get();
  hipStream_t s = c->stream;
  launch_pair_info(m->descs.d, m->d_res, (int)(sizeof(revo_pair_result) / 4), (int)(offsetof(revo_pair_result, flags) / 4),
                   info_params(m->tp, 0), n, w->d_part, w->d_cnt, w->d_ticket, w->d_out, s);
  HIPCHECK(hipGetLastError());
  HIPCHECK(hipMemcpyAsync(w->h_out, w->d_out, sizeof(revo_pair_info) * n, hipMemcpyDeviceToHost, s));
  HIPCHECK(hipEventRecord(w->ev_done, s));
  return REVO_OK;
}
extern "C" int revo_mdev_pair_info_wait_(revo_mdev* m, int n, revo_pair_info* out) {
  if (n <= 0) return REVO_OK;
  if (!m->info_ws) return fail(REVO_ERR_INVALID_ARG, "no information launch to wait for");
  const int rc = wait_event_polled(m->info_ws->ev_done);
  if (rc) return rc;
  memcpy(out, m->info_ws->h_out, sizeof(revo_pair_info) * n);
  return REVO_OK;
}

extern "C" int revo_mdev_vote_(revo_mdev* m, int n, MultiVote* votes) {
  revo_ctx* c = m->c;
  HIPCHECK(hipSetDevice(c->device));
  const int nfh = m->ts.n_frames_hist_voting;
  hipStream_t vs = c->vote_stream;
  TRY(m->vdesc.reserve(m->S, vs));
  int nv = 0, idx[1024];
  const LevelGeom& lv = c->geom.lv[m->hl];
  const int use_orig = lv.has_orig;
  for (int i = 0; i < n; ++i) {
    MultiVote& v = votes[i];
    v.status = REVO_TRACKER_STATE_OK;
    const std::deque<Past>& past = m->past[v.stream];
    if (past.empty() || !m->ts.check_tracking_results) continue;
    FrameSet* fs = (FrameSet*)v.set;
    TRY(fs->ready.wait_elsewhere(vs));
    VoteDesc& d = m->vdesc.h[nv];
    memset(&d, 0, sizeof(d));
    float inv[16];
    mat4_inverse(v.T_w_curr, inv);
    int nframes = 0;
    for (int fr = 0; fr < nfh && fr < (int)past.size() && fr < 3; ++fr) {
      vote_cloud_pose(inv, past[fr], d.RT[fr]);
      d.pts[fr] = past[fr].d_pts;
      d.n[fr] = past[fr].d_n;
      ++nframes;
    }
    d.n_clouds = nframes;
    const size_t f = (size_t)v.frame * lv.npix;
    d.edges = (use_orig ? fs->p.edges_orig[m->hl] : fs->p.edges[m->hl]) + f;
    d.depth = fs->p.depth[m->hl] + f;
    d.marks = m->d_marks + (size_t)v.stream * m->cloud_cap;
    d.hist8 = m->d_hist8 + 8 * v.stream;
    d.done = m->d_done + v.stream;
    d.host_out = m->h_vout + 16 * v.stream;
    idx[nv++] = i;
  }
  if (!nv) return REVO_OK;
  const unsigned seq = ++m->seq ? m->seq : ++m->seq;
  TRY(m->vdesc.upload(nv, vs));
  launch_vote_multi(c->geom, m->hl, nv, m->vdesc.d, seq, vs);
  HIPCHECK(hipGetLastError());
  for (int k = 0; k < nv; ++k) {
    MultiVote& v = votes[idx[k]];
    const int* o = m->h_vout + 16 * v.stream;
    { int rc = wait_seq(vs, (volatile unsigned*)(o + 8), seq); if (rc) return rc; }
    v.status = vote_decide(o + 4, m->vdesc.h[k].n_clouds, nullptr);
  }
  return REVO_OK;
}

extern "C" int revo_mdev_add_clouds_(revo_mdev* m, int n, const MultiFrame* f) {
  if (n <= 0) return REVO_OK;
  revo_ctx* c = m->c;
  HIPCHECK(hipSetDevice(c->device));
  hipStream_t vs = c->vote_stream;
  TRY(m->cdesc.reserve(n, vs));
  const size_t keep = 3 + (size_t)std::max(0, m->ts.n_frames_hist_voting);
  for (int i = 0; i < n; ++i) {
    FrameSet* fs = (FrameSet*)f[i].set;
    TRY(fs->ready.wait_elsewhere(vs));
    Past p{};
    TRY(past_take(m->past_pool, m->cloud_cap, m->cloud_cap, &p, true));
    const size_t fr = (size_t)f[i].frame;
    m->cdesc.h[i] = CloudCopyDesc{p.d_pts, fs->p.pts_trk[m->hl] + fr * m->cloud_cap, p.d_n, fs->p.npts + fr * REVO_L + m->hl};
    p.n = -1;
    memcpy(p.T_w, f[i].T_w, sizeof(float) * 16);
    p.ts = f[i].ts;
    std::deque<Past>& q = m->past[f[i].stream];
    q.push_back(p);
    if (q.size() > keep) { m->past_pool.push_back(q[3]); q.erase(q.begin() + 3); }
  }
  TRY(m->cdesc.upload(n, vs));
  launch_copy_cloud_multi(n, m->cdesc.d, vs);
  HIPCHECK(hipGetLastError());
  return REVO_OK;
}

extern "C" void revo_mdev_clear_past_(revo_mdev* m, int stream, int keep) {
  if (keep < 0) keep = m->ts.n_frames_hist_voting;
  std::deque<Past>& q = m->past[stream];
  while ((int)q.size() > std::max(0, keep)) { m->past_pool.push_back(q.front()); q.pop_front(); }
}

extern "C" int revo_mdev_promote_(revo_mdev* m, int n, const MultiFrame* f) {
  if (n <= 0) return REVO_OK;
  revo_ctx* c = m->c;
  HIPCHECK(hipSetDevice(c->device));
  hipStream_t s = c->stream;
  const PyrGeom& g = c->geom;
  std::vector<CopySeg> segs;
  for (int i = 0; i < n; ++i) {
    FrameSet* src = (FrameSet*)f[i].set;
    TRY(src->ready.wait_elsewhere(s));
    const size_t sf = (size_t)f[i].frame, df = (size_t)f[i].stream;
    const FramePlanes& a = src->p;
    const FramePlanes& b = m->kf->p;
    auto add = [&](const void* sp, void* dp, size_t per_frame) {
      if (per_frame) segs.push_back(CopySeg{(const char*)sp + sf * per_frame, (char*)dp + df * per_frame, per_frame});
    };
    for (int l = 0; l < g.n_levels; ++l) {
      const LevelGeom& v = g.lv[l];
      const size_t np = (size_t)v.npix, words = (size_t)v.h * v.wpr, cols = (size_t)v.w * v.nchunk;
      add(a.gray[l], b.gray[l], np);
      add(a.depth[l], b.depth[l], np * 4);
      add(a.cs[l], b.cs[l], words * 8);
      add(a.edges[l], b.edges[l], np);
      add(a.edges_orig[l], b.edges_orig[l], np);
      add(a.pts_trk[l], b.pts_trk[l], np * 16);
      if (v.patch > 0) add(a.hist[l], b.hist[l], (size_t)v.hist_w * v.hist_h);
      add(a.chunk[l], b.chunk[l], cols * 4);
      add(a.cmask[l], b.cmask[l], cols * 4);
      if (l < g.n_levels - 1) add(a.vb[l], b.vb[l], np / 8);
    }
    add(a.npts, b.npts, sizeof(int) * REVO_L);
    add(a.hist_nz, b.hist_nz, sizeof(int) * REVO_L);
    add(a.strip_tot, b.strip_tot, sizeof(int) * (size_t)g.total_strips);
    add(a.tile_base, b.tile_base, sizeof(int) * (size_t)g.total_tiles);
    add(src->d_bgr, m->kf->d_bgr, (size_t)g.lv[0].npix * 3);
  }
  TRY(m->segs.reserve((int)segs.size(), s));
  memcpy(m->segs.h, segs.data(), sizeof(CopySeg) * segs.size());
  TRY(m->segs.upload((int)segs.size(), s));
  launch_copy_segments((int)segs.size(), m->segs.d, s);
  for (int i = 0; i < n; ++i) {
    launch_keyframe(g, m->kf->p, f[i].stream, 1, 1, s);
    revo_pyr& v = m->kf_views[f[i].stream];
    v.ts = f[i].ts; v.table_built = false; v.ref_list_built = false;
  }
  HIPCHECK(hipGetLastError());
  return REVO_OK;
}

extern "C" revo_pyr* revo_mdev_keyframe_(revo_mdev* m, int stream) { return &m->kf_views[stream]; }
```

### revo_amd/csrc/revo_pyramid.hip

```cpp
#include "revo_dev.h"
#include "revo_nms_px.h"
#include "revo_edt_px.h"
#include <type_traits>

namespace {

#ifdef REVO_BUILD_PRIO
#define BUILD_PRIO() __builtin_amdgcn_s_setprio(REVO_BUILD_PRIO)
#else
#define BUILD_PRIO()
#endif

__device__ __forceinline__ int level_of(const PyrGeom& g, int v, int LevelGeom::*base) {
  int l = 0;
#pragma unroll
  for (int k = 1; k < REVO_L; ++k)
    if (k < g.n_levels && v >= g.lv[k].*base) l = k;
  return l;
}
__device__ __forceinline__ int clampi(int v, int lo, int hi) { return v < lo ? lo : (v > hi ? hi : v); }
__device__ __forceinline__ int reflect101(int i, int n) {
  if (i < 0) i = -i;
  if (i >= n) i = 2 * n - 2 - i;
  return i;
}

__device__ __forceinline__ uint32_t gray4(uint32_t a, uint32_t b, uint32_t c) {
  const int B0 = a & 255, G0 = (a >> 8) & 255, R0 = (a >> 16) & 255, B1 = a >> 24;
  const int G1 = b & 255, R1 = (b >> 8) & 255, B2 = (b >> 16) & 255, G2 = b >> 24;
  const int R2 = c & 255, B3 = (c >> 8) & 255, G3 = (c >> 16) & 255, R3 = c >> 24;
  const uint32_t y0 = (uint32_t)(B0 * 1868 + G0 * 9617 + R0 * 4899 + 8192) >> 14;
  const uint32_t y1 = (uint32_t)(B1 * 1868 + G1 * 9617 + R1 * 4899 + 8192) >> 14;
  const uint32_t y2 = (uint32_t)(B2 * 1868 + G2 * 9617 + R2 * 4899 + 8192) >> 14;
  const uint32_t y3 = (uint32_t)(B3 * 1868 + G3 * 9617 + R3 * 4899 + 8192) >> 14;
  return y0 | (y1 << 8) | (y2 << 16) | (y3 << 24);
}
__global__ void __launch_bounds__(256) k_gray_depth(const uint8_t* __restrict__ bgr, const float* __restrict__ depth_f32,
                                                    const uint16_t* __restrict__ depth_u16, float alpha,
                                                    uint8_t* __restrict__ gray, float* __restrict__ depth_out, int npix, int frame0) {
  BUILD_PRIO();
  const int f = frame0 + blockIdx.z;
  const int g16 = blockIdx.x * 256 + threadIdx.x;
  if (g16 * 16 >= npix) return;
  const uint4* src = reinterpret_cast<const uint4*>(bgr + (size_t)f * npix * 3) + (size_t)g16 * 3;
  const uint4 p = src[0], q = src[1], r = src[2];
  reinterpret_cast<uint4*>(gray + (size_t)f * npix)[g16] =
      make_uint4(gray4(p.x, p.y, p.z), gray4(p.w, q.x, q.y), gray4(q.z, q.w, r.x), gray4(r.y, r.z, r.w));
  if (depth_out == depth_f32) return;
  float4* dst = reinterpret_cast<float4*>(depth_out + (size_t)f * npix) + (size_t)g16 * 4;
  if (depth_u16) {
    const uint4* raw = reinterpret_cast<const uint4*>(depth_u16 + (size_t)f * npix) + (size_t)g16 * 2;
    const uint4 u = raw[0], v = raw[1];
    const uint32_t wds[8] = {u.x, u.y, u.z, u.w, v.x, v.y, v.z, v.w};
#pragma unroll
    for (int k = 0; k < 4; ++k) {
      float4 d;
      d.x = (float)(wds[2 * k] & 0xffff) * alpha + 0.0f;
      d.y = (float)(wds[2 * k] >> 16) * alpha + 0.0f;
      d.z = (float)(wds[2 * k + 1] & 0xffff) * alpha + 0.0f;
      d.w = (float)(wds[2 * k + 1] >> 16) * alpha + 0.0f;
      dst[k] = d;
    }
  } else {
    const float4* in = reinterpret_cast<const float4*>(depth_f32 + (size_t)f * npix) + (size_t)g16 * 4;
    const float4 d0 = in[0], d1 = in[1], d2 = in[2], d3 = in[3];
    dst[0] = d0; dst[1] = d1; dst[2] = d2; dst[3] = d3;
  }
}

struct EdgeStage {
  const uint2* cs;
  const unsigned short* epre;
  const int* base;
  float* out;
  int wpr, tiles_total;
};
template <bool GRAY, bool DEPTH, bool STAGE = false>
__global__ void __launch_bounds__(256) k_pyrdown(const uint8_t* __restrict__ src, int sw, int sh, uint8_t* __restrict__ dst,
                                                 int dw, int dh, const float* __restrict__ dsrc, float* __restrict__ ddst, int frame0,
                                                 int fstride, uint8_t* __restrict__ vsrc, float dmin, float dmax, EdgeStage es) {
  BUILD_PRIO();
  static_assert(!STAGE || DEPTH, "staging rides on the depth half");
  const int f = frame0 + fstride * blockIdx.z;
  src += (size_t)f * sw * sh;
  dst += (size_t)f * dw * dh;
// ... 165 lines not shown
  auto load_raw = [&](int r) -> Raw {
    const uint32_t rr = (uint32_t)clampi(r, 0, h - 1);
    Raw q;
    q.m0 = *reinterpret_cast<const uint32_t*>(gray + (__umul24(rr, (uint32_t)w) + (uint32_t)xo));
    q.prev = *reinterpret_cast<const uint32_t*>(gray + (__umul24(rr, (uint32_t)w) + (uint32_t)o_prev));
    q.next = *reinterpret_cast<const uint32_t*>(gray + (__umul24(rr, (uint32_t)w) + (uint32_t)o_next));
    return q;
  };
  const uint32_t sel_prev = has_prev ? 0x03020100u : 0x04040404u, sel_next = has_next ? 0x03020100u : 0x07070707u;
  auto make_hrow = [&](Raw q) -> HRow4 {
    return hrow4(__builtin_amdgcn_perm(q.m0, q.prev, sel_prev), q.m0, __builtin_amdgcn_perm(q.m0, q.next, sel_next));
  };
  HRow4 H0, H1, H2;
  MRow4 M0, M1, M2;
  DRow4 D0, D1, D2;
  {
    const Raw r0 = load_raw(y0 - 2), r1 = load_raw(y0 - 1), r2 = load_raw(y0), r3 = load_raw(y0 + 1);
    H0 = make_hrow(r0); H1 = make_hrow(r1); H2 = make_hrow(r2);
    mag_row4(H0, H1, H2, has_prev, has_next, active && y0 - 1 >= 0, M0, D0);
    H0 = make_hrow(r3);
  }
  Raw ahead = load_raw(y0 + 2);
  mag_row4(H1, H2, H0, has_prev, has_next, active, M1, D1);
  uint2* out = pl.cs[l] + (size_t)f * h * lv.wpr;
  const uint32_t ow = (uint32_t)y0 * (uint32_t)lv.wpr + (uint32_t)(xg >> 3);
  const int sh = 4 * (threadIdx.x & 7);
  const int low_high = max(g.canny_low, g.canny_high);
  auto emit = [&](int i, uint32_t cb, uint32_t sb) {
    uint32_t cw = cb << sh, sw = sb << sh;
    cw |= (uint32_t)__builtin_amdgcn_update_dpp(0, (int)cw, 0xB1, 0xf, 0xf, true);
    sw |= (uint32_t)__builtin_amdgcn_update_dpp(0, (int)sw, 0xB1, 0xf, 0xf, true);
    cw |= (uint32_t)__builtin_amdgcn_update_dpp(0, (int)cw, 0x4E, 0xf, 0xf, true);
    sw |= (uint32_t)__builtin_amdgcn_update_dpp(0, (int)sw, 0x4E, 0xf, 0xf, true);
    cw |= (uint32_t)__builtin_amdgcn_update_dpp(0, (int)cw, 0x141, 0xf, 0xf, true);
    sw |= (uint32_t)__builtin_amdgcn_update_dpp(0, (int)sw, 0x141, 0xf, 0xf, true);
    if ((threadIdx.x & 7) == 0 && y0 + i < h) out[ow + (uint32_t)(i * lv.wpr)] = make_uint2(cw, sw);
  };
#define NMS_STEP4(i, Ha, Hb, Hc, Ma, Mb, Mc, Db, Dc)                                  \
  {                                                                                   \
    Hc = make_hrow(ahead);                                                            \
    if ((i) < NMS_R - 1) ahead = load_raw(y0 + (i) + 3);                              \
    mag_row4(Ha, Hb, Hc, has_prev, has_next, active && y0 + (i) + 1 < h, Mc, Dc);      \
    uint32_t cb, sb;                                                                  \
    nms_row4(Ma, Mb, minus1_row4(Mb), Mc, minus1_row4(Mc), Db, g.canny_low, low_high, &cb, &sb); \
    emit((i), cb, sb);                                                                \
  }
  NMS_STEP4(0, H2, H0, H1, M0, M1, M2, D1, D2)
  NMS_STEP4(1, H0, H1, H2, M1, M2, M0, D2, D0)
  NMS_STEP4(2, H1, H2, H0, M2, M0, M1, D0, D1)
  NMS_STEP4(3, H2, H0, H1, M0, M1, M2, D1, D2)
  NMS_STEP4(4, H0, H1, H2, M1, M2, M0, D2, D0)
  NMS_STEP4(5, H1, H2, H0, M2, M0, M1, D0, D1)
#undef NMS_STEP4
}

#ifndef HYST_THREADS
#define HYST_THREADS 1024
#endif
__device__ __forceinline__ uint32_t dil3(uint32_t a, uint32_t al, uint32_t ar) {
  return a | __builtin_amdgcn_alignbit(a, al, 31) | __builtin_amdgcn_alignbit(ar, a, 1);
}
__device__ __forceinline__ uint32_t run_fill(uint32_t C, uint32_t S) {
  const uint32_t up = ((C + S) ^ C) & C;
  const uint32_t rC = __builtin_bitreverse32(C), rS = __builtin_bitreverse32(S);
  const uint32_t dn = __builtin_bitreverse32(((rC + rS) ^ rC) & rC);
  return up | dn | S;
}
__device__ __forceinline__ int hist_wide_tile(const uint32_t* row, int pitch, int patch, int last, uint32_t ma, uint32_t mb) {
  int cnt = 0;
  for (int y = 0; y < patch; ++y, row += pitch) {
    cnt += __popc(row[0] & ma) + __popc(row[last] & mb);
    for (int k = 1; k < last; ++k) cnt += __popc(row[k]);
  }
  return cnt;
}

#ifdef REVO_HYST_PROFILE
#define HP(i) if (threadIdx.x == 0) hp[i] = clock64()
#define HA(i) if (threadIdx.x == 0) { const long long now_ = clock64(); ha[i] += now_ - hlast; hlast = now_; }
#else
#define HP(i)
#define HA(i)
#endif
template <bool C_IN_LDS, bool E_GLOBAL = false>
__device__ __forceinline__ void hyst_level(const PyrGeom& g, const FramePlanes& pl, const int l, const int f, uint32_t* s_mem) {
  static_assert(!(C_IN_LDS && E_GLOBAL), "the candidate bitmap is in LDS only when the edge bitmap is");
#ifdef REVO_HYST_PROFILE
  long long hp[12], ha[8], hlast = 0;
  for (int i = 0; i < 12; ++i) hp[i] = 0;
  for (int i = 0; i < 8; ++i) ha[i] = 0;
  int dbg_sweeps = 0, dbg_bands = 0;
#endif
  HP(0);
  const LevelGeom& lv = g.lv[l];
  const int w = lv.w, h = lv.h, wpr = lv.wpr;
  const int pitch = wpr;
  const int nwords = h * wpr;
  const int e_words = (h + 2) * pitch + 2;
  uint32_t* Cl = s_mem;
  uint32_t* Ebase = C_IN_LDS ? s_mem + (REVO_HYST_LDS_MAX / 4 - e_words)
                  : (E_GLOBAL ? reinterpret_cast<uint32_t*>(pl.scratch[l] + (size_t)f * g.lv[l].npix) : s_mem);
  uint32_t* E = Ebase + 1;
  const uint2* cs = pl.cs[l] + (size_t)f * h * wpr;
  const int tid = threadIdx.x;
  for (int i = tid; i < pitch + 1; i += HYST_THREADS) { Ebase[i] = 0u; Ebase[e_words - 1 - i] = 0u; }
  for (int i = tid; i < nwords; i += HYST_THREADS) {
    const uint2 v = cs[i];
    E[pitch + i] = v.y;
    if (C_IN_LDS) Cl[i] = v.x & ~v.y;
  }
  __syncthreads();
  HP(1);
  bool done = false;
#ifdef REVO_HYST_PROFILE
  int dbg_runs = -1, dbg_t = 0, dbg_a = 0;
#endif
  if (C_IN_LDS) {
    unsigned short* Bs = reinterpret_cast<unsigned short*>(Cl + nwords);
    uint32_t* parent = Cl + nwords + (nwords + 2) / 2;
    const int table_words = (int)(REVO_HYST_LDS_MAX / 4) - (nwords + (nwords + 2) / 2);
    const int cap = min(table_words / 2, table_words - e_words);
    const int cap_keep = (table_words - e_words) / 2;
    __shared__ int s_wsum[HYST_THREADS / 64];
    __shared__ int s_total, s_promoted;
#ifdef REVO_HYST_PROFILE
    __shared__ int s_dbg[4];
    if (tid < 4) s_dbg[tid] = 0;
#endif
    auto weak = [&](int wi) -> uint32_t { return Cl[wi]; };
    auto starts = [](uint32_t wk) -> uint32_t { return wk & ~(wk << 1); };
    const float inv_wpr = 1.0f / (float)wpr;
    const uint32_t FLAG = 0x80000000u, IDM = 0x7fffffffu;
#ifdef REVO_HYST_PROFILE
    hlast = clock64();
#endif
    for (int sweep = 0; sweep < 64 && !done; ++sweep) {
#ifdef REVO_HYST_PROFILE
      ++dbg_sweeps;
#endif
      {
        const int wpt = (nwords + HYST_THREADS - 1) / HYST_THREADS;
        const int w0 = min(nwords, tid * wpt), w1 = min(nwords, w0 + wpt);
        int mine = 0;
        for (int wi = w0; wi < w1; ++wi) mine += __popc(starts(weak(wi)));
        int incl = mine;
#pragma unroll
        for (int o = 1; o < 64; o <<= 1) {
          const int v = __shfl_up(incl, o);
          if ((tid & 63) >= o) incl += v;
        }
        __syncthreads();
        if ((tid & 63) == 63) s_wsum[tid >> 6] = incl;
        if (tid == 0) s_promoted = 0;
        __syncthreads();
        int before = incl - mine;
        for (int k = 0; k < (tid >> 6); ++k) before += s_wsum[k];
        if (tid == HYST_THREADS - 1) { s_total = before + mine; Bs[nwords] = (unsigned short)min(65535, before + mine); }
        for (int wi = w0; wi < w1; ++wi) {
          Bs[wi] = (unsigned short)before;
          before += __popc(starts(weak(wi)));
        }
        __syncthreads();
      }
      const int nruns = s_total;
      HA(0);
#ifdef REVO_HYST_PROFILE
      if (sweep == 0) dbg_runs = nruns;
// ... 144 lines not shown
    __syncthreads();
  }
  if (!done) {
    __shared__ unsigned short s_list[HYST_THREADS];
    __shared__ unsigned char s_act[2][HYST_THREADS];
    __shared__ int s_n;
  const int max_strips = HYST_THREADS / wpr;
  const int rpt = (h + max_strips - 1) / max_strips;
  const int nstrips = (h + rpt - 1) / rpt;
  const int n_items = nstrips * wpr;
  s_act[0][tid] = 0; s_act[1][tid] = 0;
  if (tid == 0) s_n = 0;
  __syncthreads();
  int n_list = n_items;
#ifndef REVO_HYST_MAXIT
#define REVO_HYST_MAXIT 8192
#endif
  for (int it = 0; it < REVO_HYST_MAXIT; ++it) {
    const int wb = it & 1;
    bool changed = false;
    if (tid < n_list) {
      const int item = it == 0 ? tid : (int)s_list[tid];
      const int strip = item / wpr, c = item - strip * wpr;
      const int r0 = strip * rpt, r1 = min(h, r0 + rpt) - 1;
      uint32_t* Ec = E + pitch + c;
      const uint32_t lm = c > 0 ? ~0u : 0u, rm = c < wpr - 1 ? ~0u : 0u;
      auto Cat = [&](int r) -> uint32_t { return C_IN_LDS ? (Cl[r * wpr + c] | Ec[r * pitch]) : cs[r * wpr + c].x; };
      uint32_t prev_d = dil3(Ec[(r0 - 1) * pitch], Ec[(r0 - 1) * pitch - 1] & lm, Ec[(r0 - 1) * pitch + 1] & rm);
      uint32_t cur = Ec[r0 * pitch], cl = Ec[r0 * pitch - 1] & lm, cr = Ec[r0 * pitch + 1] & rm;
      for (int r = r0; r <= r1; ++r) {
        const uint32_t nx = Ec[(r + 1) * pitch], nl = Ec[(r + 1) * pitch - 1] & lm, nr = Ec[(r + 1) * pitch + 1] & rm;
        const uint32_t Cw = Cat(r);
        const uint32_t hz = __builtin_amdgcn_alignbit(cur, cl, 31) | __builtin_amdgcn_alignbit(cr, cur, 1);
        const uint32_t F = run_fill(Cw, cur | (Cw & (prev_d | dil3(nx, nl, nr) | hz)));
        if (F != cur) { Ec[r * pitch] = F; changed = true; }
        prev_d = dil3(F, cl, cr);
        cur = nx; cl = nl; cr = nr;
      }
      prev_d = dil3(cur, cl, cr);
      cur = Ec[r1 * pitch]; cl = Ec[r1 * pitch - 1] & lm; cr = Ec[r1 * pitch + 1] & rm;
      for (int r = r1; r >= r0; --r) {
        const uint32_t nx = Ec[(r - 1) * pitch], nl = Ec[(r - 1) * pitch - 1] & lm, nr = Ec[(r - 1) * pitch + 1] & rm;
        const uint32_t Cw = Cat(r);
        const uint32_t hz = __builtin_amdgcn_alignbit(cur, cl, 31) | __builtin_amdgcn_alignbit(cr, cur, 1);
        const uint32_t F = run_fill(Cw, cur | (Cw & (prev_d | dil3(nx, nl, nr) | hz)));
        if (F != cur) { Ec[r * pitch] = F; changed = true; }
        prev_d = dil3(F, cl, cr);
        cur = nx; cl = nl; cr = nr;
      }
      if (changed) s_act[wb][item] = 1;
    }
    if (!__syncthreads_or(changed ? 1 : 0)) break;
    bool act = false;
    if (tid < n_items) {
      const int strip = tid / wpr, c = tid - strip * wpr;
      const unsigned char* a = s_act[wb];
#pragma unroll
      for (int ds = -1; ds <= 1; ++ds)
#pragma unroll
        for (int dc = -1; dc <= 1; ++dc) {
          const int ss = strip + ds, cc = c + dc;
          if (ss >= 0 && ss < nstrips && cc >= 0 && cc < wpr) act = act || a[ss * wpr + cc] != 0;
        }
    }
    const unsigned long long m = __ballot(act);
    int base = 0;
    if ((tid & 63) == 0 && m) base = atomicAdd(&s_n, __popcll(m));
    base = __shfl(base, 0);
    if (act) s_list[base + __popcll(m & ((1ull << (tid & 63)) - 1ull))] = (unsigned short)tid;
    s_act[wb ^ 1][tid] = 0;
    __syncthreads();
    n_list = s_n;
    __syncthreads();
    if (tid == 0) s_n = 0;
  }
  __syncthreads();
  }
  __syncthreads();
  HP(5);
  uint8_t* edges = pl.edges[l] + (size_t)f * lv.npix;
  uint8_t* orig = lv.has_orig ? pl.edges_orig[l] + (size_t)f * lv.npix : nullptr;
  const bool rows16 = (w & 15) == 0;
  const float inv_w = 1.0f / (float)w;
  for (int i = tid; i < lv.npix / 16; i += HYST_THREADS) {
    const int p = i * 16;
    int y = (int)(((float)p + 0.5f) * inv_w);
    y += (y + 1) * w <= p ? 1 : (y * w > p ? -1 : 0);
    const int x = p - y * w;
    uint32_t o[4];
    if (rows16) {
      const uint32_t bits = (E[(y + 1) * pitch + (x >> 5)] >> (x & 31)) & 0xffffu;
#pragma unroll
      for (int q = 0; q < 4; ++q) o[q] = ((((bits >> (4 * q)) & 0xfu) * 0x00204081u) & 0x01010101u) * 0xffu;
    } else {
#pragma unroll
      for (int q = 0; q < 4; ++q) {
        int xx = x + 4 * q, yy = y;
        while (xx >= w) { xx -= w; yy += 1; }
        const uint32_t bits = (E[(yy + 1) * pitch + (xx >> 5)] >> (xx & 31)) & 0xfu;
        o[q] = ((bits * 0x00204081u) & 0x01010101u) * 0xffu;
      }
    }
    const uint4 v = make_uint4(o[0], o[1], o[2], o[3]);
    *reinterpret_cast<uint4*>(edges + p) = v;
    if (orig) *reinterpret_cast<uint4*>(orig + p) = v;
  }
  {
    uint2* csw = pl.cs[l] + (size_t)f * h * wpr;
    for (int i = tid; i < nwords; i += HYST_THREADS) csw[i].y = E[pitch + i];
  }
  HP(6);
  if (lv.patch > 0) {
    const int ntiles = lv.hist_w * lv.hist_h;
    int nz = 0;
    const float inv_hw = 1.0f / (float)lv.hist_w;
    for (int t0 = 0; t0 < ntiles; t0 += HYST_THREADS) {
      const int t = t0 + tid;
      if (t < ntiles) {
        int ty = (int)(((float)t + 0.5f) * inv_hw);
        ty += (ty + 1) * lv.hist_w <= t ? 1 : (ty * lv.hist_w > t ? -1 : 0);
        const int tx = t - ty * lv.hist_w;
        const int xa = tx * lv.patch, xb = xa + lv.patch;
        const int wa = xa >> 5, wb = (xb - 1) >> 5;
        const uint32_t ma = ~0u << (xa & 31), mb = (xb & 31) ? ~0u >> (32 - (xb & 31)) : ~0u;
        const uint32_t m0 = wa == wb ? ma & mb : ma, m1 = wb > wa + 1 ? ~0u : (wb > wa ? mb : 0u), m2 = wb > wa + 1 ? mb : 0u;
        const int o1 = wb > wa ? 1 : 0, o2 = wb > wa + 1 ? 2 : 0;
        const uint32_t* row = E + (ty * lv.patch + 1) * pitch + wa;
        int cnt = 0;
        if (wb - wa > 2) cnt = hist_wide_tile(row, pitch, lv.patch, wb - wa, ma, mb);
        else
        for (int y = 0; y < lv.patch; ++y, row += pitch) cnt += __popc(row[0] & m0) + __popc(row[o1] & m1) + __popc(row[o2] & m2);
        const uint8_t v = (uint8_t)(cnt & 255);
        pl.hist[l][(size_t)f * ntiles + t] = v;
        nz += v != 0;
      }
    }
    __shared__ int s_nz;
    if (tid == 0) s_nz = 0;
    __syncthreads();
    if (nz) atomicAdd(&s_nz, nz);
    __syncthreads();
    if (tid == 0) pl.hist_nz[f * REVO_L + l] = s_nz;
  }
#ifdef REVO_HYST_PROFILE
  HP(7);
  if (threadIdx.x == 0 && l == 0 && f < 64)
    printf("hyst f=%d: load %lld uf_total %lld [scan %lld record %lld link %lld compress %lld flag %lld resolve %lld] runs %d sweeps %d bands %d uf %d rebuild %lld out %lld hist %lld touched %d atomics %d\n", f,
           hp[1] - hp[0], hp[5] - hp[1], ha[0], ha[1], ha[2], ha[3], ha[4], ha[5], dbg_runs, dbg_sweeps, dbg_bands, (int)done, ha[6], hp[6] - hp[5], hp[7] - hp[6], dbg_t, dbg_a);
#endif
}
template <bool C_IN_LDS, bool E_GLOBAL = false>
__global__ void __launch_bounds__(HYST_THREADS) k_hyst(PyrGeom g, FramePlanes pl, int only_flagged, int n_frames) {
  BUILD_PRIO();
  extern __shared__ uint32_t s_mem[];
  const int n_items = g.n_levels * n_frames;
  if (only_flagged) {
    __shared__ int s_any;
    if (threadIdx.x == 0) s_any = 0;
    __syncthreads();
    for (int item = threadIdx.x; item < n_items; item += HYST_THREADS)
      if (pl.need_full[(g.frame0 + item % n_frames) * REVO_L + item / n_frames]) s_any = 1;
    __syncthreads();
    if (!s_any) return;
  }
  for (int item = blockIdx.x; item < n_items; item += gridDim.x) {
    const int l = item / n_frames;
    const int f = g.frame0 + item % n_frames;
    if (only_flagged && !pl.need_full[f * REVO_L + l]) continue;
    hyst_level<C_IN_LDS, E_GLOBAL>(g, pl, l, f, s_mem);
    __syncthreads();
  }
}

#ifndef HB_THREADS
#define HB_THREADS 1024
#endif
#ifndef HB_LDS_WORDS
#define HB_LDS_WORDS 16384
#endif
struct BandRef { int l, R0, R1; };
__device__ __forceinline__ BandRef band_ref(const PyrGeom& g, int bi) {
  int l = 0;
#pragma unroll
  for (int k = 1; k < REVO_L; ++k)
    if (k < g.n_levels && bi >= g.lv[k].band_base) l = k;
  const LevelGeom& lv = g.lv[l];
  const int b = bi - lv.band_base;
  BandRef r;
  r.l = l; r.R0 = b * lv.band_rows; r.R1 = min(lv.h, r.R0 + lv.band_rows);
  return r;
}
__device__ __forceinline__ int band_capb(const LevelGeom& lv) {
  const int hb = lv.band_rows, nwb = hb * lv.wpr;
  const int table_words = HB_LDS_WORDS - (nwb + (nwb + 2) / 2);
  const int e_words = (hb + 2) * lv.wpr + 2;
  int cap = min(table_words / 2, table_words - e_words);
  cap = min(cap, 65535);
  const int h_last = lv.h - (lv.nbands - 1) * lv.band_rows;
  cap = min(cap, ((h_last * lv.w - 4 - 2 * lv.wpr) / 8) * 5);
  return max(cap, 0) & ~31;
}
struct BandRec { int* hdr; int* bs_first; int* bs_last; uint32_t* flags; unsigned short* root; uint32_t* rec; };
__device__ __forceinline__ BandRec band_rec(const FramePlanes& pl, const LevelGeom& lv, int l, int f, int R0, int capb) {
  int* base = pl.scratch[l] + (size_t)f * lv.npix + (size_t)R0 * lv.w;
  BandRec r;
  r.hdr = base; r.bs_first = base + 4; r.bs_last = base + 4 + lv.wpr;
  r.flags = reinterpret_cast<uint32_t*>(base + 4 + 2 * lv.wpr);
  r.root = reinterpret_cast<unsigned short*>(base + 4 + 2 * lv.wpr + capb / 32);
  r.rec = reinterpret_cast<uint32_t*>(base + 4 + 2 * lv.wpr + capb / 32 + capb / 2);
  return r;
}

__device__ __forceinline__ void hyst_band(const PyrGeom& g, const FramePlanes& pl, const BandRef br, const int f, uint32_t* s_mem) {
  __shared__ int s_wsum[HB_THREADS / 64];
  __shared__ int s_total;
  const int l = br.l;
  const LevelGeom& lv = g.lv[l];
  const int h = lv.h, wpr = lv.wpr, pitch = wpr;
  const int hb = br.R1 - br.R0, nwb = hb * wpr, e_words = (hb + 2) * pitch + 2;
  const int tid = threadIdx.x;
  uint32_t* Cl = s_mem;
  uint32_t* Ebase = s_mem + (HB_LDS_WORDS - e_words);
  uint32_t* E = Ebase + 1;
  const uint2* cs = pl.cs[l] + ((size_t)f * h + br.R0) * wpr;
  const int capb = band_capb(lv);
  const BandRec rec_out = band_rec(pl, lv, l, f, br.R0, capb);
  auto load_e = [&](bool with_cl) {
    if (tid == 0) { Ebase[0] = 0u; Ebase[e_words - 1] = 0u; }
    for (int c = tid; c < wpr; c += HB_THREADS) {
      E[c] = br.R0 > 0 ? cs[c - wpr].y : 0u;
      E[(hb + 1) * pitch + c] = br.R1 < h ? cs[nwb + c].y : 0u;
    }
    for (int i0 = tid; i0 < nwb; i0 += 4 * HB_THREADS) {
      uint2 v[4];
#pragma unroll
      for (int k = 0; k < 4; ++k) v[k] = cs[min(i0 + k * HB_THREADS, nwb - 1)];
#pragma unroll
      for (int k = 0; k < 4; ++k) {
        const int i = i0 + k * HB_THREADS;
        if (i < nwb) {
          if (with_cl) { E[pitch + i] = v[k].y; Cl[i] = v[k].x & ~v[k].y; }
          else E[pitch + i] = v[k].y | (v[k].x & ~Cl[i]);
        }
      }
    }
  };
  load_e(true);
  __syncthreads();
  unsigned short* Bs = reinterpret_cast<unsigned short*>(Cl + nwb);
  uint32_t* parent = Cl + nwb + (nwb + 2) / 2;
  const int table_words = HB_LDS_WORDS - (nwb + (nwb + 2) / 2);
  const int cap_keep = (table_words - e_words) / 2;
// ... 82 lines not shown
    }
    __syncthreads();
    for (int me = tid; me < nr; me += HB_THREADS) {
      parent[me] = key_of(find(me));
      rec_out.rec[me] = rec[me];
    }
    __syncthreads();
    if (nr > cap_keep) {
      load_e(false);
      __syncthreads();
    }
    for (int wi = tid; wi < nwb; wi += HB_THREADS) {
      const uint32_t wk = Cl[wi];
      if (!wk) continue;
      int r = (int)(((float)wi + 0.5f) * inv_wpr);
      r += (r + 1) * wpr <= wi ? 1 : (r * wpr > wi ? -1 : 0);
      const int c = wi - r * wpr;
      const uint32_t lm = c > 0 ? ~0u : 0u, rm = c < wpr - 1 ? ~0u : 0u;
      const uint32_t* Xc = E + pitch + wi;
      const uint32_t sd = dil3(Xc[-pitch], Xc[-pitch - 1] & lm, Xc[-pitch + 1] & rm) | dil3(Xc[pitch], Xc[pitch - 1] & lm, Xc[pitch + 1] & rm) |
                          __builtin_amdgcn_alignbit(Xc[0], Xc[-1] & lm, 31) | __builtin_amdgcn_alignbit(Xc[1] & rm, Xc[0], 1);
      if (!(wk & sd)) continue;
      const uint32_t touched = run_fill(wk, wk & sd);
      int me = (int)Bs[wi];
      for (uint32_t m = starts(wk); m; m &= m - 1, ++me)
        if (touched & m & (0u - m)) {
          uint32_t* root = &parent[parent[me] & 0xffffu];
          if (!(*root & FLAG)) atomicOr(root, FLAG);
        }
    }
    __syncthreads();
    for (int wi = tid; wi < nwb; wi += HB_THREADS) {
      const uint32_t wk = Cl[wi];
      if (!wk) continue;
      int me = (int)Bs[wi];
      uint32_t prom = 0;
      for (uint32_t m = starts(wk); m; m &= m - 1, ++me)
        if (parent[parent[me] & 0xffffu] & FLAG) prom |= m & (0u - m);
      if (prom) E[pitch + wi] |= run_fill(wk, prom);
    }
    __syncthreads();
  }
  uint32_t* eb = pl.ebits[l] + ((size_t)f * h + br.R0) * wpr;
  for (int i = tid; i < nwb; i += HB_THREADS) eb[i] = E[pitch + i];
  if (tid == 0) { rec_out.hdr[0] = nr; rec_out.hdr[1] = 0; rec_out.hdr[2] = 1; }
  for (int c = tid; c < wpr; c += HB_THREADS) { rec_out.bs_first[c] = Bs[c]; rec_out.bs_last[c] = Bs[(hb - 1) * wpr + c]; }
  for (int i = tid; i < (nr + 31) / 32; i += HB_THREADS) {
    uint32_t bits = 0;
    for (int k = 0; k < 32; ++k) {
      const int me = 32 * i + k;
      if (me < nr && (int)(parent[me] & 0xffffu) == me && (parent[me] & FLAG)) bits |= 1u << k;
    }
    rec_out.flags[i] = bits;
  }
  for (int me = tid; me < nr; me += HB_THREADS) rec_out.root[me] = (unsigned short)(parent[me] & 0xffffu);
}
__global__ void __launch_bounds__(HB_THREADS) k_hyst_band(PyrGeom g, FramePlanes pl) {
  extern __shared__ uint32_t s_mem[];
  const int nB = gridDim.x / g.total_bands;
  hyst_band(g, pl, band_ref(g, blockIdx.x / nB), g.frame0 + blockIdx.x % nB, s_mem);
}

__device__ __forceinline__ bool hyst_frame_is_heavy(const PyrGeom& g, const FramePlanes& pl, int f) {
  __shared__ int s_cnt[HYST_THREADS / 64];
  const LevelGeom& lv = g.lv[0];
  const int nwords = lv.h * lv.wpr;
  const uint2* cs = pl.cs[0] + (size_t)f * nwords;
  int mine = 0;
  for (int i = threadIdx.x; i < nwords; i += HYST_THREADS) {
    const uint2 v = cs[i];
    const uint32_t wk = v.x & ~v.y;
    mine += __popc(wk & ~(wk << 1));
  }
#pragma unroll
  for (int o = 32; o >= 1; o >>= 1) mine += __shfl_xor(mine, o);
  __syncthreads();
  if ((threadIdx.x & 63) == 0) s_cnt[threadIdx.x >> 6] = mine;
  __syncthreads();
  int total = 0;
#pragma unroll
  for (int k = 0; k < HYST_THREADS / 64; ++k) total += s_cnt[k];
  return total >= g.hyst_heavy_runs;
}
__global__ void __launch_bounds__(HYST_THREADS) k_hyst_mixed(PyrGeom g, FramePlanes pl, int n_frames) {
  static_assert(HB_THREADS == HYST_THREADS, "one workgroup shape for both paths");
  extern __shared__ uint32_t s_mem[];
  const int nb0 = g.lv[0].nbands;
  const int n_band_wg = nb0 * n_frames;
  if ((int)blockIdx.x < n_band_wg) {
    const int f = g.frame0 + blockIdx.x % n_frames;
    if (!hyst_frame_is_heavy(g, pl, f)) return;
    hyst_band(g, pl, band_ref(g, blockIdx.x / n_frames), f, s_mem);
    return;
  }
  const int item = blockIdx.x - n_band_wg;
  const int l = item / n_frames, f = g.frame0 + item % n_frames;
  if (l == 0) {
    const bool heavy = hyst_frame_is_heavy(g, pl, f);
    if (threadIdx.x == 0) pl.hyst_heavy[f] = heavy ? 1 : 0;
    if (heavy) return;
  }
  hyst_level<true>(g, pl, l, f, s_mem);
}

#define HS_THREADS 256
#define HS_MAX_BANDS 32
#define HS_MAX_PAIRS 6144
__global__ void __launch_bounds__(HS_THREADS) k_hyst_seam(PyrGeom g, FramePlanes pl, int mixed) {
  extern __shared__ uint32_t s_fl[];
  __shared__ uint2 s_pair[HS_MAX_PAIRS];
  __shared__ int s_npairs;
  __shared__ int s_changed_band[HS_MAX_BANDS];
  const int nB = mixed ? gridDim.x : gridDim.x / g.n_levels;
  const int l = blockIdx.x / nB;
  const int f = g.frame0 + blockIdx.x % nB;
  const LevelGeom& lv = g.lv[l];
  const int nb = lv.nbands;
  if (nb <= 1 || pl.need_full[f * REVO_L + l]) return;
  if (mixed && !pl.hyst_heavy[f]) return;
  const int wpr = lv.wpr, h = lv.h;
  const int tid = threadIdx.x;
  const int capb = band_capb(lv), fw = capb / 32;
  const uint2* cs = pl.cs[l] + (size_t)f * h * wpr;
  for (int b = 0; b < nb; ++b) {
    const BandRec rb = band_rec(pl, lv, l, f, b * lv.band_rows, capb);
    const int n = (rb.hdr[0] + 31) / 32;
    for (int i = tid; i < fw; i += HS_THREADS) s_fl[b * fw + i] = i < n ? rb.flags[i] : 0u;
  }
  if (tid < HS_MAX_BANDS) s_changed_band[tid] = 0;
  if (tid == 0) s_npairs = 0;
  __syncthreads();
  auto starts = [](uint32_t wk) -> uint32_t { return wk & ~(wk << 1); };
  auto weak_at = [&](int y, int c) -> uint32_t { if (c < 0 || c >= wpr) return 0u; const uint2 v = cs[(size_t)y * wpr + c]; return v.x & ~v.y; };
  for (int item = tid; item < (nb - 1) * wpr; item += HS_THREADS) {
    const int sm = item / wpr, c = item - sm * wpr;
    const int yb = (sm + 1) * lv.band_rows, ya = yb - 1;
    const uint32_t Wa = weak_at(ya, c);
    const uint32_t Wl = weak_at(yb, c - 1), Wm = weak_at(yb, c), Wr = weak_at(yb, c + 1);
    if (!Wa || !(Wm | (Wl >> 31) | (Wr & 1u))) continue;
    const BandRec ra = band_rec(pl, lv, l, f, sm * lv.band_rows, capb);
    const BandRec rbb = band_rec(pl, lv, l, f, yb, capb);
    int ida = ra.bs_last[c];
    const int idm = rbb.bs_first[c], idl = c > 0 ? rbb.bs_first[c - 1] : 0, idr = c < wpr - 1 ? rbb.bs_first[c + 1] : 0;
    for (uint32_t m = starts(Wa); m; m &= m - 1, ++ida) {
      const int bit = __ffs(m) - 1;
      const uint32_t t2 = ~(Wa >> bit);
      const int len = t2 ? __ffs(t2) - 1 : 32 - bit;
      const uint32_t ma = (0xffffffffu >> (32 - len)) << bit;
      int roota = -1;
      for (int side = 0; side < 3; ++side) {
        int idb0; uint32_t Wb, hits;
        if (side == 0) { Wb = Wm; hits = Wm & (ma | (ma << 1) | (ma >> 1)); idb0 = idm; }
        else if (side == 1) { Wb = Wl; hits = (ma & 1u) ? (Wl & 0x80000000u) : 0u; idb0 = idl; }
        else { Wb = Wr; hits = (ma >> 31) ? (Wr & 1u) : 0u; idb0 = idr; }
        while (hits) {
          const int hb2 = __ffs(hits) - 1;
          const uint32_t upto = (2u << hb2) - 1u;
          const int k = __popc(starts(Wb) & upto) - 1;
          const uint32_t gap = ~Wb & upto;
          const int first = gap ? 32 - __clz(gap) : 0;
          const uint32_t t3 = ~(Wb >> first);
          const int lenb = t3 ? __ffs(t3) - 1 : 32 - first;
          hits &= ~((0xffffffffu >> (32 - lenb)) << first);
          if (roota < 0) roota = ra.root[ida];
          const int rootb = rbb.root[idb0 + k];
          const int slot = atomicAdd(&s_npairs, 1);
          if (slot < HS_MAX_PAIRS) s_pair[slot] = make_uint2((uint32_t)sm, (uint32_t)roota | ((uint32_t)rootb << 16));
        }
      }
    }
  }
  __syncthreads();
  const int np = s_npairs;
  if (np > HS_MAX_PAIRS) {
    if (tid == 0) pl.need_full[f * REVO_L + l] = 1;
    return;
  }
  for (int it = 0; it < 65536; ++it) {
    bool changed = false;
    for (int i = tid; i < np; i += HS_THREADS) {
      const uint2 pr = s_pair[i];
      const int sm = (int)pr.x, roota = (int)(pr.y & 0xffffu), rootb = (int)(pr.y >> 16);
      uint32_t* fa = s_fl + sm * fw;
      uint32_t* fb = s_fl + (sm + 1) * fw;
      const bool A = (fa[roota >> 5] >> (roota & 31)) & 1u, Bf = (fb[rootb >> 5] >> (rootb & 31)) & 1u;
      if (A != Bf) {
        if (!A) { atomicOr(&fa[roota >> 5], 1u << (roota & 31)); s_changed_band[sm] = 1; }
        else { atomicOr(&fb[rootb >> 5], 1u << (rootb & 31)); s_changed_band[sm + 1] = 1; }
        changed = true;
      }
    }
    if (!__syncthreads_or(changed ? 1 : 0)) break;
  }
  __syncthreads();
  for (int b = 0; b < nb; ++b) {
    if (!s_changed_band[b]) continue;
    const BandRec rb = band_rec(pl, lv, l, f, b * lv.band_rows, capb);
    const int n = (rb.hdr[0] + 31) / 32;
    for (int i = tid; i < n; i += HS_THREADS) rb.flags[i] = s_fl[b * fw + i];
    if (tid == 0) rb.hdr[1] = 1;
  }
}

#define HO_THREADS 512
__global__ void __launch_bounds__(HO_THREADS) k_hyst_out(PyrGeom g, FramePlanes pl, int mixed) {
  extern __shared__ uint32_t s_mem[];
  const int nB = gridDim.x / (mixed ? g.lv[0].nbands : g.total_bands);
  const BandRef br = band_ref(g, blockIdx.x / nB);
  const int f = g.frame0 + blockIdx.x % nB;
  const int l = br.l;
  if (pl.need_full[f * REVO_L + l]) return;
  if (mixed && !pl.hyst_heavy[f]) return;
  const LevelGeom& lv = g.lv[l];
  const int w = lv.w, h = lv.h, wpr = lv.wpr, pitch = wpr;
  const int hb = br.R1 - br.R0, nwb = hb * wpr;
  const int tid = threadIdx.x;
  uint32_t* E = s_mem;
  uint32_t* eb = pl.ebits[l] + ((size_t)f * h + br.R0) * wpr;
  for (int i = tid; i < nwb; i += HO_THREADS) E[i] = eb[i];
  const BandRec rb = band_rec(pl, lv, l, f, br.R0, band_capb(lv));
  const bool promote = rb.hdr[1] != 0;
  __syncthreads();
  if (promote) {
    const int nr = rb.hdr[0];
    for (int me = tid; me < nr; me += HO_THREADS) {
      const int root = rb.root[me];
      if ((rb.flags[root >> 5] >> (root & 31)) & 1u) {
        const uint32_t rc = rb.rec[me];
        atomicOr(&E[rc >> 10], (0xffffffffu >> (31u - (rc & 31u))) << ((rc >> 5) & 31u));
      }
    }
    __syncthreads();
  }
  uint8_t* edges = pl.edges[l] + (size_t)f * lv.npix + (size_t)br.R0 * w;
  uint8_t* orig = lv.has_orig ? pl.edges_orig[l] + (size_t)f * lv.npix + (size_t)br.R0 * w : nullptr;
  const bool rows16 = (w & 15) == 0;
  const float inv_w = 1.0f / (float)w;
  for (int i = tid; i < hb * w / 16; i += HO_THREADS) {
    const int p = i * 16;
    int y = (int)(((float)p + 0.5f) * inv_w);
    y += (y + 1) * w <= p ? 1 : (y * w > p ? -1 : 0);
    const int x = p - y * w;
    uint32_t o[4];
    if (rows16) {
      const uint32_t bits = (E[y * pitch + (x >> 5)] >> (x & 31)) & 0xffffu;
#pragma unroll
      for (int q = 0; q < 4; ++q) o[q] = ((((bits >> (4 * q)) & 0xfu) * 0x00204081u) & 0x01010101u) * 0xffu;
    } else {
#pragma unroll
      for (int q = 0; q < 4; ++q) {
        int xx = x + 4 * q, yy = y;
        while (xx >= w) { xx -= w; yy += 1; }
        const uint32_t bits = (E[yy * pitch + (xx >> 5)] >> (xx & 31)) & 0xfu;
        o[q] = ((bits * 0x00204081u) & 0x01010101u) * 0xffu;
      }
    }
    const uint4 v = make_uint4(o[0], o[1], o[2], o[3]);
    *reinterpret_cast<uint4*>(edges + p) = v;
    if (orig) *reinterpret_cast<uint4*>(orig + p) = v;
  }
  {
    uint2* csw = pl.cs[l] + ((size_t)f * h + br.R0) * wpr;
    for (int i = tid; i < nwb; i += HO_THREADS) csw[i].y = E[i];
  }
  if (lv.patch > 0) {
    const int ty0 = br.R0 / lv.patch, ty1 = min(lv.hist_h, br.R1 / lv.patch);
    const int ntiles = max(0, ty1 - ty0) * lv.hist_w;
    int nz = 0;
    for (int t = tid; t < ntiles; t += HO_THREADS) {
      const int ty = ty0 + t / lv.hist_w, tx = t % lv.hist_w;
      const int xa = tx * lv.patch, xb = xa + lv.patch;
      const int wa = xa >> 5, wb = (xb - 1) >> 5;
      const uint32_t ma = ~0u << (xa & 31), mb = (xb & 31) ? ~0u >> (32 - (xb & 31)) : ~0u;
      const uint32_t m0 = wa == wb ? ma & mb : ma, m1 = wb > wa + 1 ? ~0u : (wb > wa ? mb : 0u), m2 = wb > wa + 1 ? mb : 0u;
      const int o1 = wb > wa ? 1 : 0, o2 = wb > wa + 1 ? 2 : 0;
      const uint32_t* row = E + (ty * lv.patch - br.R0) * pitch + wa;
      int cnt = 0;
      if (wb - wa > 2) cnt = hist_wide_tile(row, pitch, lv.patch, wb - wa, ma, mb);
      else
      for (int y = 0; y < lv.patch; ++y, row += pitch) cnt += __popc(row[0] & m0) + __popc(row[o1] & m1) + __popc(row[o2] & m2);
      const uint8_t v = (uint8_t)(cnt & 255);
      pl.hist[l][(size_t)f * lv.hist_w * lv.hist_h + (size_t)ty * lv.hist_w + tx] = v;
      nz += v != 0;
    }
#pragma unroll
    for (int o = 32; o > 0; o >>= 1) nz += __shfl_xor(nz, o);
    if ((tid & 63) == 0 && nz) atomicAdd(&pl.hist_nz[f * REVO_L + l], nz);
  }
}

__global__ void __launch_bounds__(1024) k_fill(PyrGeom g, FramePlanes pl, int only_level) {
  BUILD_PRIO();
  const int f = g.frame0 + blockIdx.z;
  const int la = only_level ? only_level : 1, lb = only_level ? only_level + 1 : g.n_levels;
  for (int l = la; l < lb; ++l) {
    const LevelGeom lv = g.lv[l], lf = g.lv[l - 1];
    if (!(g.use_edge_hist && lv.patch > 0 && lf.patch > 0)) continue;
    const float frac = (float)pl.hist_nz[f * REVO_L + l] / (float)(lv.hist_w * lv.hist_h);
    if (frac < g.n_percentage) {
      const uint8_t* top = pl.edges[l - 1] + (size_t)f * lf.npix;
      uint8_t* mod = pl.edges[l] + (size_t)f * lv.npix;
      const uint8_t* hist = pl.hist[l] + (size_t)f * lv.hist_w * lv.hist_h;
      const double thr = g.fill_thr[l];
      const int cw = lf.w / 2, ch = lf.h / 2;
      for (int i = blockIdx.x * 1024 + threadIdx.x; i < cw * ch; i += gridDim.x * 1024) {
        const int y = i / cw, x = i % cw;
        const int yy = 2 * y + 1, xx = 2 * x + 1;
        const int ty = yy / lf.patch, tx = xx / lf.patch;
        if (ty >= lv.hist_h || tx >= lv.hist_w) continue;
        if ((double)hist[(size_t)ty * lv.hist_w + tx] < thr && top[(size_t)yy * lf.w + xx] > 0) {
          mod[(size_t)y * lv.w + x] = 255;
          atomicOr(&(pl.cs[l] + (size_t)f * lv.h * lv.wpr)[(size_t)y * lv.wpr + (x >> 5)].y, 1u << (x & 31));
        }
      }
    }
    __syncthreads();
  }
}

__device__ __forceinline__ uint32_t tile_transpose32(uint32_t v, int r) {
#pragma unroll
  for (int k = 16; k >= 1; k >>= 1) {
    const uint32_t mk = k == 16 ? 0x0000ffffu : k == 8 ? 0x00ff00ffu : k == 4 ? 0x0f0f0f0fu : k == 2 ? 0x33333333u : 0x55555555u;
    const uint32_t t = (uint32_t)__shfl_xor((int)v, k);
    v = (r & k) ? ((v & ~mk) | ((t >> k) & mk)) : ((v & mk) | ((t & mk) << k));
  }
  return v;
}

__device__ __forceinline__ bool depth_ok(float Z, float dmin, float dmax) {
  return isfinite(Z) && Z > dmin && Z < dmax;
}

#define CW_COLS 64
#define CW_LANES 16
#ifndef CW_LANES_COUNT
#define CW_LANES_COUNT 8
#endif
#define CW_MAXCHUNK 64
#define CW_STAGE 4096
template <bool WRITE>
__global__ void __launch_bounds__(CW_COLS * (WRITE ? CW_LANES : CW_LANES_COUNT)) k_compact_walk(PyrGeom g, FramePlanes pl) {
  constexpr int LANES = WRITE ? CW_LANES : CW_LANES_COUNT;
  __shared__ int s_cnt[CW_COLS * CW_MAXCHUNK];
  __shared__ unsigned s_mask[CW_COLS * CW_MAXCHUNK];
  __shared__ float4 s_pts[WRITE ? CW_STAGE : 1];
  const int nB = gridDim.x / g.total_strips;
  const int sx = blockIdx.x / nB;
  const int f = g.frame0 + blockIdx.x % nB;
  const int l = level_of(g, sx, &LevelGeom::strip_base);
  const LevelGeom& lv = g.lv[l];
  const int strip = sx - lv.strip_base;
  const int tid = threadIdx.x, xl = tid & (CW_COLS - 1), cl = tid / CW_COLS;
  const int x = strip * CW_COLS + xl;
  const int ncols = min(CW_COLS, lv.w - strip * CW_COLS);
  const int nslots = ncols * lv.nchunk;
  const size_t slot0 = (size_t)f * lv.w * lv.nchunk + (size_t)strip * CW_COLS * lv.nchunk;
  const float* depth = pl.depth[l] + (size_t)f * lv.npix;
  if (!WRITE) {
    const uint8_t* edges = pl.edges[l] + (size_t)f * lv.npix;
    const bool bit_tiles = l < g.n_levels - 1 && (lv.w & 31) == 0 && lv.chunk_rows == 32;
    if (bit_tiles) {
      const uint2* csw = pl.cs[l] + (size_t)f * lv.h * lv.wpr;
      const uint32_t* vw = reinterpret_cast<const uint32_t*>(pl.vb[l] + (size_t)f * (lv.npix >> 3));
      const int lane = tid & 63, r = lane & 31;
      const int wc = strip * (CW_COLS / 32) + (lane >> 5);
      for (int c = cl; c < lv.nchunk; c += LANES) {
        const int y = c * 32 + r;
        uint32_t v = 0;
        if (y < lv.h && wc < lv.wpr) v = csw[(size_t)y * lv.wpr + wc].y & vw[(size_t)y * lv.wpr + wc];
        v = tile_transpose32(v, r);
        if (x < lv.w) {
          s_mask[xl * lv.nchunk + c] = v;
          s_cnt[xl * lv.nchunk + c] = __popc(v);
        }
      }
    } else
    if (x < lv.w) {
      for (int c = cl; c < lv.nchunk; c += LANES) {
        const int yb = c * lv.chunk_rows, ye = min(lv.h, yb + lv.chunk_rows);
        unsigned em = 0;
#pragma unroll 8
        for (int y = yb; y < ye; ++y) em |= (edges[(size_t)y * lv.w + x] ? 1u : 0u) << (y - yb);
        unsigned vm = 0;
        if (l < g.n_levels - 1) {
          const uint8_t* vb = pl.vb[l] + (size_t)f * (lv.npix >> 3);
          const int vpitch = lv.w >> 3;
          if (em) {
#pragma unroll 8
            for (int y = yb; y < ye; ++y) vm |= ((unsigned)(vb[(size_t)y * vpitch + (x >> 3)] >> (x & 7)) & 1u) << (y - yb);
            vm &= em;
          }
        } else
        for (unsigned m = em; m;) {
          int b[4];
          float Z[4];
#pragma unroll
          for (int j = 0; j < 4; ++j) {
            b[j] = m ? __ffs(m) - 1 : -1;
// ... 350 lines not shown
  if (i >= dw * dh) return;
  const int x = i % dw, y = i / dw;
  const int kk[5] = {1, 4, 6, 4, 1};
  int acc[3] = {0, 0, 0};
#pragma unroll
  for (int j = 0; j < 5; ++j) {
    const uint8_t* row = src + (size_t)reflect101(2 * y + j - 2, h) * w * 3;
    int rs[3] = {0, 0, 0};
#pragma unroll
    for (int t = 0; t < 5; ++t) {
      const uint8_t* px = row + (size_t)reflect101(2 * x + t - 2, w) * 3;
      rs[0] += kk[t] * px[0]; rs[1] += kk[t] * px[1]; rs[2] += kk[t] * px[2];
    }
    acc[0] += kk[j] * rs[0]; acc[1] += kk[j] * rs[1]; acc[2] += kk[j] * rs[2];
  }
  uint8_t* o = dst + (size_t)i * 3;
  o[0] = (uint8_t)((acc[0] + 128) >> 8); o[1] = (uint8_t)((acc[1] + 128) >> 8); o[2] = (uint8_t)((acc[2] + 128) >> 8);
}

template <bool WRITE>
__global__ void __launch_bounds__(256) k_pcl_walk(LevelGeom lv, float dmin, float dmax, const float* __restrict__ depth,
                                                  const uint8_t* __restrict__ edges, const uint8_t* __restrict__ bgr,
                                                  int dense, int* __restrict__ chunk, unsigned* __restrict__ cmask,
                                                  const int* __restrict__ total, int cap, float4* __restrict__ out) {
  const int i = blockIdx.x * 256 + threadIdx.x;
  if (i >= lv.w * lv.nchunk) return;
  const int x = i % lv.w, c = i / lv.w;
  const int yb = c * lv.chunk_rows, ye = min(lv.h, yb + lv.chunk_rows);
  const size_t slot = (size_t)x * lv.nchunk + c;
  if (!WRITE) {
    unsigned vm = 0;
    for (int y = yb; y < ye; ++y) {
      const size_t p = (size_t)y * lv.w + x;
      if ((dense || edges[p]) && depth_ok(depth[p], dmin, dmax)) vm |= 1u << (y - yb);
    }
    cmask[slot] = vm;
    chunk[slot] = __popc(vm);
  } else {
    if (*total > cap) return;
    int o = chunk[slot];
    for (unsigned m = cmask[slot]; m; m &= m - 1) {
      const int y = yb + __ffs(m) - 1;
      const size_t p = (size_t)y * lv.w + x;
      const float Z = depth[p];
      const float X = __fdiv_rn(Z * ((float)x - lv.cx), lv.fx);
      const float Y = __fdiv_rn(Z * ((float)y - lv.cy), lv.fy);
      const uint8_t* px = bgr + p * 3;
      out[2 * o] = make_float4(X, Y, Z, 1.0f);
      out[2 * o + 1] = make_float4(__fdiv_rn((float)px[2], 255.0f), __fdiv_rn((float)px[1], 255.0f),
                                   __fdiv_rn((float)px[0], 255.0f), 1.0f);
      ++o;
    }
  }
}

__global__ void __launch_bounds__(1024) k_pcl_scan(int* chunk, int n, int* total) {
  __shared__ int s_part[1024];
  const int t = block_exclusive_scan(chunk, n, s_part);
  if (threadIdx.x == 0) *total = t;
}

#define EDT_THREADS 1024
#define EDT_COL_GROUPS(h) ((h) > 1024 ? 64 : ((h) > 512 ? 32 : 16))
__global__ void __launch_bounds__(EDT_THREADS) k_edt_cols(PyrGeom g, FramePlanes pl, int f0, int fstride, int nframes) {
  __shared__ int s_first[EDT_THREADS];
  __shared__ int s_last[EDT_THREADS];
  const int f = f0 + (blockIdx.x % nframes) * fstride;
  int l = 0, sidx = blockIdx.x / nframes, ngroups = 16, ncols = 64;
  for (int k = 0; k < g.n_levels; ++k) {
    ngroups = EDT_COL_GROUPS(g.lv[k].h);
    ncols = EDT_THREADS / ngroups;
    const int ns = (g.lv[k].w + ncols - 1) / ncols;
    if (sidx < ns) { l = k; break; }
    sidx -= ns;
  }
  const LevelGeom& lv = g.lv[l];
  const int col = threadIdx.x % ncols, grp = threadIdx.x / ncols;
  const int x = sidx * ncols + col;
  const int rpg = (lv.h + ngroups - 1) / ngroups;
  const int yb = min(lv.h, grp * rpg), ye = min(lv.h, yb + rpg);
  const bool in = x < lv.w;
  const uint8_t* edges = pl.edges[l] + (size_t)f * lv.npix;
  unsigned em = 0;
  if ((lv.w & 31) == 0 && (ncols & 31) == 0) {
    const uint2* csw = pl.cs[l] + (size_t)f * lv.h * lv.wpr;
    const int r = threadIdx.x & 31;
    const int wc = (sidx * ncols + (col & ~31)) >> 5;
    uint32_t v = 0;
    if (yb + r < ye && wc < lv.wpr) v = csw[(size_t)(yb + r) * lv.wpr + wc].y;
    em = tile_transpose32(v, r);
    if (!in) em = 0;
  } else if (in) {
#pragma unroll 8
    for (int y = yb; y < ye; ++y) em |= (edges[(size_t)y * lv.w + x] ? 1u : 0u) << (y - yb);
  }
  s_first[grp * ncols + col] = em ? yb + __ffs(em) - 1 : EDT_INF;
  s_last[grp * ncols + col] = em ? yb + 31 - __clz(em) : -EDT_INF;
  __syncthreads();
  if (!in) return;
  int above = -EDT_INF, below = EDT_INF;
  for (int k = 0; k < grp; ++k) above = max(above, s_last[k * ncols + col]);
  for (int k = ngroups - 1; k > grp; --k) below = min(below, s_first[k * ncols + col]);
  uint16_t* gd = reinterpret_cast<uint16_t*>(pl.scratch[l]) + (size_t)f * lv.npix;
  const int FAR = 1 << 20;
  int du = (above <= -EDT_INF) ? FAR : (yb - above);
  const int dbelow = (below >= EDT_INF) ? FAR : (below - yb);
  for (int y = yb; y < ye; ++y) {
    const int k = y - yb;
    const unsigned hi = em >> k;
    du = (hi & 1u) ? 0 : du;
    const int dn = hi ? __ffs(hi) - 1 : dbelow - k;
    const int m = min(du, dn);
    gd[(size_t)y * lv.w + x] = (uint16_t)(m >= 0xffff ? 0xffff : m);
    du += 1;
  }
}

__global__ void __launch_bounds__(EDT_ROW_THREADS) k_edt_rows(PyrGeom g, FramePlanes pl, int f0, int fstride) {
  extern __shared__ __attribute__((aligned(16))) int s_g2[];
  const int f = f0 + blockIdx.z * fstride;
  const int l = level_of(g, blockIdx.x, &LevelGeom::edt_block_base);
  const LevelGeom lv = g.lv[l];
  const int w = lv.w;
  const int y0 = (blockIdx.x - lv.edt_block_base) * lv.edt_rows;
  const int nr = min(lv.edt_rows, lv.h - y0);
  const int pad = w + 4, pitch = w + 2 * pad;
  const uint2* src = reinterpret_cast<const uint2*>(reinterpret_cast<const uint16_t*>(pl.scratch[l]) + (size_t)f * lv.npix + (size_t)y0 * w);
  const int4 inf4 = make_int4(EDT_INF, EDT_INF, EDT_INF, EDT_INF);
  const int padq = pad >> 2, wq = w >> 2, pitchq = pitch >> 2;
  int4* lds4 = reinterpret_cast<int4*>(s_g2);
  const float inv_wq = __builtin_amdgcn_rcpf((float)wq);
  for (int j = threadIdx.x; j < nr * wq; j += EDT_ROW_THREADS) {
    const uint2 q = src[j];
    const int r = edt_div_small(j, inv_wq), i = j - __mul24(r, wq);
    int4* row4 = lds4 + __mul24(r, pitchq);
    row4[i] = inf4;
    row4[padq + wq + i] = inf4;
    row4[padq + i] = make_int4(edt_g2((int)(q.x & 0xffffu)), edt_g2((int)(q.x >> 16)), edt_g2((int)(q.y & 0xffffu)), edt_g2((int)(q.y >> 16)));
  }
  for (int j = threadIdx.x; j < 2 * nr; j += EDT_ROW_THREADS) lds4[__mul24(j >> 1, pitchq) + ((j & 1) ? padq + 2 * wq : wq)] = inf4;
  __syncthreads();
  float4* dt4 = reinterpret_cast<float4*>(pl.dt[l] + (size_t)f * lv.npix + (size_t)y0 * w);
  const float inv = __builtin_amdgcn_rcpf((float)nr);
  for (int i = threadIdx.x; i < nr * wq; i += EDT_ROW_THREADS) {
    const int q = edt_div_small(i, inv), r = i - __mul24(q, nr);
    int best[4];
    edt_search4(s_g2 + __mul24(r, pitch) + pad, q, w, best);
    dt4[__mul24(r, wq) + q] = make_float4(edt_dt(best[0]), edt_dt(best[1]), edt_dt(best[2]), edt_dt(best[3]));
  }
}

__global__ void __launch_bounds__(256) k_grad_table(PyrGeom g, FramePlanes pl, int f0, int fstride) {
  const int f = f0 + blockIdx.z * fstride;
  const int l = blockIdx.y;
  const LevelGeom& lv = g.lv[l];
  const int i = blockIdx.x * 256 + threadIdx.x;
  if (i >= lv.npix) return;
  const float* dt = pl.dt[l] + (size_t)f * lv.npix;
  float4 o = make_float4(0.f, 0.f, 0.f, 0.f);
  if (i >= lv.w && i < lv.w * (lv.h - 1)) {
    o.x = 0.5f * (dt[i - 1] - dt[i + 1]);
    o.y = 0.5f * (dt[i - lv.w] - dt[i + lv.w]);
    o.z = dt[i];
  }
  pl.table[l][(size_t)f * lv.npix + i] = o;
}

__global__ void __launch_bounds__(256) k_vote_mark(VoteArgs a, float fx, float fy, float cx, float cy, int W, int H,
                                                   int* marks) {
  const int c = blockIdx.y;
  const int n = *a.n[c];
  const float* R = a.RT[c];
  const float* T = R + 9;
  const float4* pts = a.pts[c];
// ... 83 lines not shown
    if (m) marks[i] = 0;
    const float Z = d.depth[i];
    if (depth_ok(Z, dmin, dmax)) {
      const int val = __popc(m);
      atomicAdd(&s_h[val], 1);
      if (d.edges[i] > 0) atomicAdd(&s_h[4 + val], 1);
    }
  }
  __syncthreads();
  if (threadIdx.x < 8 && s_h[threadIdx.x]) atomicAdd(&d.hist8[threadIdx.x], s_h[threadIdx.x]);
  __threadfence();
  __syncthreads();
  if (threadIdx.x == 0) s_last = (atomicAdd(d.done, 1u) == gridDim.x - 1);
  __syncthreads();
  if (s_last) {
    if (threadIdx.x < 8) d.host_out[threadIdx.x] = atomicExch(&d.hist8[threadIdx.x], 0);
    if (threadIdx.x == 0) *d.done = 0u;
    __threadfence_system();
    __syncthreads();
    if (threadIdx.x == 0) *(volatile int*)&d.host_out[8] = (int)seq_val;
  }
}

__global__ void __launch_bounds__(256) k_copy_cloud_multi(const CloudCopyDesc* __restrict__ descs) {
  const CloudCopyDesc& d = descs[blockIdx.y];
  const int n = *d.src_n;
  for (int i = blockIdx.x * 256 + threadIdx.x; i < n; i += gridDim.x * 256) d.dst[i] = d.src[i];
  if (blockIdx.x == 0 && threadIdx.x == 0) *d.dst_n = n;
}

__global__ void __launch_bounds__(256) k_copy_segments(const CopySeg* __restrict__ segs) {
  const CopySeg& sg = segs[blockIdx.y];
  const char* src = (const char*)sg.src;
  char* dst = (char*)sg.dst;
  const size_t bytes = sg.bytes;
  const size_t step = (size_t)gridDim.x * 256;
  if ((((uintptr_t)src | (uintptr_t)dst | bytes) & 15) == 0) {
    const uint4* s4 = (const uint4*)src;
    uint4* d4 = (uint4*)dst;
    for (size_t i = blockIdx.x * 256 + threadIdx.x; i < bytes / 16; i += step) d4[i] = s4[i];
  } else {
    for (size_t i = blockIdx.x * 256 + threadIdx.x; i < bytes; i += step) dst[i] = src[i];
  }
}

}

void launch_gray_depth(const PyrGeom& g, const FramePlanes& p, const uint8_t* d_bgr, const float* d_depth_f32,
                       const uint16_t* d_depth_u16, float u16_alpha, int B, hipStream_t s) {
  const int npix = g.lv[0].npix;
  dim3 grid((npix / 16 + 255) / 256, 1, B);
  hipLaunchKernelGGL(k_gray_depth, grid, dim3(256), 0, s, d_bgr, d_depth_f32, d_depth_u16, u16_alpha, p.gray[0],
                     p.depth[0], npix, g.frame0);
}

void launch_pyrdown(const PyrGeom& g, const FramePlanes& p, int lvl, int B, hipStream_t s, int parts, bool stage_edges) {
  const LevelGeom& d = g.lv[lvl];
  const LevelGeom& sl = g.lv[lvl - 1];
  dim3 grid(((d.w / 4) * ((d.h + 1) / 2) + 255) / 256, 1, B);
  EdgeStage es{};
  if (stage_edges) {
    int tb = 0;
    for (int k = 0; k < lvl - 1; ++k) tb += g.lv[k].wpr * g.lv[k].nchunk;
    es.cs = p.cs[lvl - 1]; es.epre = p.epre[lvl - 1]; es.base = p.stage_base + tb; es.out = p.stage[lvl - 1];
    es.wpr = sl.wpr; es.tiles_total = g.total_tiles;
  }
#define PYRDOWN_ARGS p.gray[lvl - 1], sl.w, sl.h, p.gray[lvl], d.w, d.h, p.depth[lvl - 1], p.depth[lvl], g.frame0, g.fstride, p.vb[lvl - 1], g.depth_min, g.depth_max, es
  if (parts == 1) hipLaunchKernelGGL((k_pyrdown<true, false>), grid, dim3(256), 0, s, PYRDOWN_ARGS);
  else if (parts == 2 && stage_edges) hipLaunchKernelGGL((k_pyrdown<false, true, true>), grid, dim3(256), 0, s, PYRDOWN_ARGS);
  else if (parts == 2) hipLaunchKernelGGL((k_pyrdown<false, true>), grid, dim3(256), 0, s, PYRDOWN_ARGS);
  else hipLaunchKernelGGL((k_pyrdown<true, true>), grid, dim3(256), 0, s, PYRDOWN_ARGS);
#undef PYRDOWN_ARGS
}

void launch_edge_prefix(const PyrGeom& g, const FramePlanes& p, int B, hipStream_t s) {
  if (g.n_levels < 2) return;
  hipLaunchKernelGGL(k_edge_prefix, dim3((g.n_levels - 1) * B), dim3(1024), 0, s, g, p);
}

void launch_canny_nms(const PyrGeom& g, const FramePlanes& p, int B, hipStream_t s) {
  hipLaunchKernelGGL(k_canny_nms4, dim3(g.total_nms_blocks, 1, B), dim3(256), 0, s, g, p);
}

void launch_hyst(const PyrGeom& g, const FramePlanes& p, int B, hipStream_t s) {
  size_t e_bytes = 0, ec_bytes = 0;
  for (int l = 0; l < g.n_levels; ++l) {
    const size_t nw = (size_t)g.lv[l].h * g.lv[l].wpr;
    const size_t e = ((size_t)(g.lv[l].h + 2) * g.lv[l].wpr + 2) * 4, c = (nw + (nw + 2) / 2) * 4;
    e_bytes = e > e_bytes ? e : e_bytes;
    ec_bytes = e + c > ec_bytes ? e + c : ec_bytes;
  }
  static bool attr_set = false;
  if (!attr_set) {
    (void)hipFuncSetAttribute(reinterpret_cast<const void*>(k_hyst<true>), hipFuncAttributeMaxDynamicSharedMemorySize, REVO_HYST_LDS_MAX);
    (void)hipFuncSetAttribute(reinterpret_cast<const void*>(k_hyst<false>), hipFuncAttributeMaxDynamicSharedMemorySize, REVO_HYST_LDS_MAX);
    attr_set = true;
  }
  const int force = g.hyst_force;
  const bool fits_single = ec_bytes + 4096 <= REVO_HYST_LDS_MAX;
  const bool banded = force >= 0 ? force == 1 : !fits_single;
  const int only_flagged = banded && g.total_bands > 0 ? 1 : 0;
  if (only_flagged) {
    static bool attr2 = false;
    if (!attr2) {
      (void)hipFuncSetAttribute(reinterpret_cast<const void*>(k_hyst_band), hipFuncAttributeMaxDynamicSharedMemorySize, HB_LDS_WORDS * 4);
      (void)hipFuncSetAttribute(reinterpret_cast<const void*>(k_hyst_out), hipFuncAttributeMaxDynamicSharedMemorySize, HB_LDS_WORDS * 4);
      (void)hipFuncSetAttribute(reinterpret_cast<const void*>(k_hyst_seam), hipFuncAttributeMaxDynamicSharedMemorySize, 64 * 1024);
      (void)hipGetLastError();
      attr2 = true;
    }
    size_t seam_lds = 4, out_lds = 4;
    for (int l = 0; l < g.n_levels; ++l) {
      const LevelGeom& lv = g.lv[l];
      const size_t nwb = (size_t)lv.band_rows * lv.wpr;
      out_lds = std::max(out_lds, nwb * 4);
      if (lv.nbands > 1) seam_lds = std::max(seam_lds, (size_t)lv.nbands * (size_t)(HB_LDS_WORDS / 2 / 32 + 64) * 4);
    }
    hipLaunchKernelGGL(k_hyst_band, dim3(g.total_bands * B), dim3(HB_THREADS), HB_LDS_WORDS * 4, s, g, p);
    if (g.any_banded) hipLaunchKernelGGL(k_hyst_seam, dim3(g.n_levels * B), dim3(HS_THREADS), seam_lds, s, g, p, 0);
    hipLaunchKernelGGL(k_hyst_out, dim3(g.total_bands * B), dim3(HO_THREADS), out_lds, s, g, p, 0);
  }
  const bool mixed = !banded && fits_single && g.hyst_heavy_runs > 0 && g.total_bands > 0 && g.lv[0].nbands > 1;
  if (mixed) {
    static bool attr3 = false;
    if (!attr3) {
      (void)hipFuncSetAttribute(reinterpret_cast<const void*>(k_hyst_mixed), hipFuncAttributeMaxDynamicSharedMemorySize, REVO_HYST_LDS_MAX);
      (void)hipFuncSetAttribute(reinterpret_cast<const void*>(k_hyst_out), hipFuncAttributeMaxDynamicSharedMemorySize, HB_LDS_WORDS * 4);
      (void)hipFuncSetAttribute(reinterpret_cast<const void*>(k_hyst_seam), hipFuncAttributeMaxDynamicSharedMemorySize, 64 * 1024);
      (void)hipGetLastError();
      attr3 = true;
    }
    const LevelGeom& l0 = g.lv[0];
    const size_t seam_lds = std::max<size_t>(4, (size_t)l0.nbands * (size_t)(HB_LDS_WORDS / 2 / 32 + 64) * 4);
    const size_t out_lds = std::max<size_t>(4, (size_t)l0.band_rows * l0.wpr * 4);
    hipLaunchKernelGGL(k_hyst_mixed, dim3((l0.nbands + g.n_levels) * B), dim3(HYST_THREADS), REVO_HYST_LDS_MAX, s, g, p, B);
    hipLaunchKernelGGL(k_hyst_seam, dim3(B), dim3(HS_THREADS), seam_lds, s, g, p, 1);
    hipLaunchKernelGGL(k_hyst_out, dim3(l0.nbands * B), dim3(HO_THREADS), out_lds, s, g, p, 1);
    hipLaunchKernelGGL(k_hyst<true>, dim3(std::min(32, g.n_levels * B)), dim3(HYST_THREADS), REVO_HYST_LDS_MAX, s, g, p, 1, B);
    return;
  }
  const int n_wg = only_flagged ? std::min(32, g.n_levels * B) : g.n_levels * B;
  if (ec_bytes + 4096 <= REVO_HYST_LDS_MAX)
    hipLaunchKernelGGL(k_hyst<true>, dim3(n_wg), dim3(HYST_THREADS), REVO_HYST_LDS_MAX, s, g, p, only_flagged, B);
  else if (e_bytes <= REVO_HYST_LDS_MAX)
    hipLaunchKernelGGL(k_hyst<false>, dim3(n_wg), dim3(HYST_THREADS), e_bytes, s, g, p, only_flagged, B);
  else
    hipLaunchKernelGGL((k_hyst<false, true>), dim3(n_wg), dim3(HYST_THREADS), 16, s, g, p, only_flagged, B);
}

void launch_fill(const PyrGeom& g, const FramePlanes& p, int B, hipStream_t s) {
  bool any = false;
  for (int l = 1; l < g.n_levels; ++l) any = any || g.lv[l].has_orig;
  if (!any) return;
  if (g.lv[0].npix <= 640 * 480) {
    hipLaunchKernelGGL(k_fill, dim3(1, 1, B), dim3(1024), 0, s, g, p, 0);
    return;
  }
  for (int l = 1; l < g.n_levels; ++l) {
    if (!g.lv[l].has_orig) continue;
    const int n = (g.lv[l - 1].w / 2) * (g.lv[l - 1].h / 2);
    hipLaunchKernelGGL(k_fill, dim3(std::min(64, (n + 1023) / 1024), 1, B), dim3(1024), 0, s, g, p, l);
  }
}

void launch_tile_points(const PyrGeom& g, const FramePlanes& p, int B, hipStream_t s, int which) {
  if (which & 1) hipLaunchKernelGGL(k_tile_count, dim3(g.n_levels * B), dim3(1024), 0, s, g, p);
  const int groups = (g.total_tiles + PT_TILES - 1) / PT_TILES;
  if ((which & 2) && g.pts_staged) hipLaunchKernelGGL(k_pts_tiles<true>, dim3(groups * B), dim3(32 * PT_TILES), 0, s, g, p);
  else if (which & 2) hipLaunchKernelGGL(k_pts_tiles<false>, dim3(groups * B), dim3(32 * PT_TILES), 0, s, g, p);
}

void launch_compact(const PyrGeom& g, const FramePlanes& p, int B, hipStream_t s) {
  dim3 grid(g.total_strips * B);
  hipLaunchKernelGGL(k_compact_walk<false>, grid, dim3(CW_COLS * CW_LANES_COUNT), 0, s, g, p);
  hipLaunchKernelGGL(k_compact_walk<true>, grid, dim3(CW_COLS * CW_LANES), 0, s, g, p);
}

void launch_pyrdown_bgr(const uint8_t* src, int w, int h, uint8_t* dst, hipStream_t s) {
  hipLaunchKernelGGL(k_pyrdown_bgr, dim3(((w / 2) * (h / 2) + 255) / 256), dim3(256), 0, s, src, w, h, dst);
}

void launch_colored_pcl(const PyrGeom& g, const FramePlanes& p, int frame, int lvl, int dense, const uint8_t* bgr_lvl,
                        int* chunk, unsigned* cmask, int* total, int cap, float* out8, hipStream_t s) {
  const LevelGeom& lv = g.lv[lvl];
  const float* depth = p.depth[lvl] + (size_t)frame * lv.npix;
  const uint8_t* edges = p.edges[lvl] + (size_t)frame * lv.npix;
  const int n = lv.w * lv.nchunk;
  dim3 grid((n + 255) / 256);
  hipLaunchKernelGGL(k_pcl_walk<false>, grid, dim3(256), 0, s, lv, g.depth_min, g.depth_max, depth, edges, bgr_lvl, dense,
                     chunk, cmask, total, cap, (float4*)out8);
  hipLaunchKernelGGL(k_pcl_scan, dim3(1), dim3(1024), 0, s, chunk, n, total);
  hipLaunchKernelGGL(k_pcl_walk<true>, grid, dim3(256), 0, s, lv, g.depth_min, g.depth_max, depth, edges, bgr_lvl, dense,
                     chunk, cmask, total, cap, (float4*)out8);
}

void launch_keyframe(const PyrGeom& g, const FramePlanes& p, int f0, int fstride, int count, hipStream_t s, int which) {
  int strips = 0;
  for (int l = 0; l < g.n_levels; ++l) {
    const int ncols = EDT_THREADS / EDT_COL_GROUPS(g.lv[l].h);
    strips += (g.lv[l].w + ncols - 1) / ncols;
  }
  if (which & 1) hipLaunchKernelGGL(k_edt_cols, dim3(strips * count), dim3(EDT_THREADS), 0, s, g, p, f0, fstride, count);
  size_t rows_lds = 0;
  for (int l = 0; l < g.n_levels; ++l) rows_lds = std::max(rows_lds, (size_t)g.lv[l].edt_rows * (3 * g.lv[l].w + 8) * sizeof(int));
  if (which & 2) hipLaunchKernelGGL(k_edt_rows, dim3(g.total_edt_blocks, 1, count), dim3(EDT_ROW_THREADS), rows_lds, s, g, p, f0, fstride);
}

void launch_grad_table(const PyrGeom& g, const FramePlanes& p, int f0, int fstride, int count, hipStream_t s) {
  hipLaunchKernelGGL(k_grad_table, dim3((g.lv[0].npix + 255) / 256, g.n_levels, count), dim3(256), 0, s, g, p, f0, fstride);
}

void launch_vote(const PyrGeom& g, const FramePlanes& curr, int curr_frame, int lvl, int n_clouds, const VoteArgs& va,
                 int* d_marks, int* d_hist8, unsigned* d_done, int* h_out8, unsigned seq_val, int use_orig_edges, hipStream_t s) {
  const LevelGeom& lv = g.lv[lvl];
  if (n_clouds > 0)
    hipLaunchKernelGGL(k_vote_mark, dim3(32, n_clouds), dim3(256), 0, s, va, lv.fx, lv.fy, lv.cx, lv.cy, lv.w, lv.h, d_marks);
  const uint8_t* edges = (use_orig_edges ? curr.edges_orig[lvl] : curr.edges[lvl]) + (size_t)curr_frame * lv.npix;
  hipLaunchKernelGGL(k_vote_hist, dim3(16), dim3(256), 0, s, d_marks, edges,
                     curr.depth[lvl] + (size_t)curr_frame * lv.npix, lv.npix, g.depth_min, g.depth_max, d_hist8, d_done, h_out8,
                     seq_val);
}

void launch_copy_cloud(float4* dst, const float4* src, int* dst_n, const int* src_n, hipStream_t s) {
  hipLaunchKernelGGL(k_copy_cloud, dim3(16), dim3(256), 0, s, dst, src, dst_n, src_n);
}

void launch_vote_multi(const PyrGeom& g, int lvl, int n, const VoteDesc* d_descs, unsigned seq_val, hipStream_t s) {
  const LevelGeom& lv = g.lv[lvl];
  hipLaunchKernelGGL(k_vote_mark_multi, dim3(32, 3, n), dim3(256), 0, s, d_descs, lv.fx, lv.fy, lv.cx, lv.cy, lv.w, lv.h);
  hipLaunchKernelGGL(k_vote_hist_multi, dim3(16, n), dim3(256), 0, s, d_descs, lv.npix, g.depth_min, g.depth_max, seq_val);
}

void launch_copy_cloud_multi(int n, const CloudCopyDesc* d_descs, hipStream_t s) {
  hipLaunchKernelGGL(k_copy_cloud_multi, dim3(16, n), dim3(256), 0, s, d_descs);
}

void launch_copy_segments(int n, const CopySeg* d_segs, hipStream_t s) {
  hipLaunchKernelGGL(k_copy_segments, dim3(64, n), dim3(256), 0, s, d_segs);
}
```

### revo_amd/csrc/revo_single.hip

```cpp
#include "revo_host_impl.h"

static int vote_enqueued(revo_ctx* c, const revo_pyr* p) {
  if (p->owns_fs) return REVO_OK;
  HIPCHECK(hipEventRecord(c->ev_vote, c->vote_stream));
  HIPCHECK(hipStreamWaitEvent(c->stream, c->ev_vote, 0));
  return REVO_OK;
}

static int track_launch(revo_ctx* c, const revo_pyr* ref, const revo_pyr* curr, const float* R, const float* T,
                        const TrackParams& tp, int slot, unsigned* seq_out) {
  fill_desc(c->h_desc, ref, curr, R, T);
  TRY(wait_ready(c, ref)); TRY(wait_ready(c, curr));
  TrackParams tp1 = tp;
  tp1.redundant_n = c->knobs.redundant_one;
  if (c->knobs.kspec_one_set)
    for (int i = 0; i < REVO_L; ++i) tp1.kspec[i] = c->knobs.kspec_one[i];
  const unsigned seq = c->seq_next++;
  if (c->seq_next == 0) c->seq_next = 1;
  const int rc = chained_track_launch(c->device, c->knobs.track_depth, c->stream, [&](unsigned* d_resident) {
    return launch_track_one(*c->h_desc, tp1, c->h_res + slot, c->h_eval, c->d_mail, &c->mail_epoch, pick_cluster(c, 1), c->h_seq + slot,
                            seq, d_resident, c->stream);
  });
  if (rc) return rc;
  *seq_out = seq;
// ... 42 lines not shown
  if (rc) return rc;
  return decode_track(c->h_res[slot & 1], R, T, err, status, nullptr, nullptr);
}

extern "C" int revo_optimizer_track_level(revo_ctx* c, const revo_pyr* ref, const revo_pyr* curr, float R[9], float T[3],
                                          int lvl, revo_residual_info* info, float* err) {
  int rc = check_pair(c, ref, curr);
  if (rc) return rc;
  if (!R || !T) return fail(REVO_ERR_INVALID_ARG, "null pose");
  if (lvl < 0 || lvl >= c->geom.n_levels) return fail(REVO_ERR_LEVEL, "level out of range");
  HIPCHECK(hipSetDevice(c->device));
  std::lock_guard<std::mutex> lk(c->mu);
  TrackParams tp = c->tp;
  tp.lvl_begin = tp.lvl_end = lvl; tp.check_init = 0; tp.eval_only = 0;
  rc = run_single(c, ref, curr, R, T, tp);
  if (rc) return rc;
  return decode_track(c->h_res[SINGLE_SLOT], R, T, err, nullptr, info, nullptr);
}

extern "C" int revo_optimizer_eval(revo_ctx* c, const revo_pyr* ref, const revo_pyr* curr, const float R[9],
                                   const float T[3], int lvl, revo_residual_info* info, float* err, float A[36],
                                   float b[6]) {
  int rc = check_pair(c, ref, curr);
  if (rc) return rc;
  if (!R || !T) return fail(REVO_ERR_INVALID_ARG, "null pose");
  if (lvl < 0 || lvl >= c->geom.n_levels) return fail(REVO_ERR_LEVEL, "level out of range");
  HIPCHECK(hipSetDevice(c->device));
  std::lock_guard<std::mutex> lk(c->mu);
  TrackParams tp = c->tp;
  tp.lvl_begin = tp.lvl_end = lvl; tp.check_init = 0; tp.eval_only = 1;
  rc = run_single(c, ref, curr, R, T, tp);
  if (rc) return rc;
  const EvalOut& e = *c->h_eval;
  if (info) { info->good_pts_edges = e.good; info->bad_pts_edges = e.bad; info->sum_error_unweighted = e.sum_u; info->sum_error_weighted = e.sum_w; }
  if (err) *err = e.mean_err;
  if (A) memcpy(A, e.A, sizeof(float) * 36);
  if (b) memcpy(b, e.b, sizeof(float) * 6);
  return REVO_OK;
}

extern "C" int revo_optimizer_solve6(revo_ctx* c, int n, const float* A36_b6_lambda, float* x6) {
  if (!c || !A36_b6_lambda || !x6 || n <= 0) return fail(REVO_ERR_INVALID_ARG, "bad argument");
  HIPCHECK(hipSetDevice(c->device));
  std::lock_guard<std::mutex> lk(c->mu);
  DevMem<float> in, out;
  float *&d_in = in.p, *&d_out = out.p;
  HIPCHECK(hipMalloc((void**)&d_in, sizeof(float) * 43 * (size_t)n));
  hipError_t e = hipMalloc((void**)&d_out, sizeof(float) * 6 * (size_t)n);
  if (e == hipSuccess) e = hipMemcpyAsync(d_in, A36_b6_lambda, sizeof(float) * 43 * (size_t)n, hipMemcpyHostToDevice, c->stream);
  if (e == hipSuccess) { launch_solve6(d_in, n, d_out, c->stream); e = hipGetLastError(); }
  if (e == hipSuccess) e = hipMemcpyAsync(x6, d_out, sizeof(float) * 6 * (size_t)n, hipMemcpyDeviceToHost, c->stream);
  if (e == hipSuccess) e = hipStreamSynchronize(c->stream);
  if (e != hipSuccess) return fail(REVO_ERR_HIP, std::string("revo_optimizer_solve6: ") + hipGetErrorString(e));
  return REVO_OK;
}

extern "C" int revo_debug_track_profile_(revo_ctx* c, float out13[13]) {
  if (!c || !out13) return REVO_ERR_INVALID_ARG;
  memcpy(out13, c->h_eval->A, sizeof(float) * 13);
  return REVO_OK;
}

extern "C" int revo_tracker_track_frames(revo_ctx* c, const revo_pyr* ref, const revo_pyr* curr, float R[9], float T[3],
                                         float* err, int* status, revo_residual_info* info, int32_t iters[REVO_MAX_LEVELS]) {
  int rc = check_pair(c, ref, curr);
  if (rc) return rc;
  if (!R || !T) return fail(REVO_ERR_INVALID_ARG, "null pose");
  HIPCHECK(hipSetDevice(c->device));
  std::lock_guard<std::mutex> lk(c->mu);
  TrackParams tp = c->tp;
  tp.eval_only = 0;
  rc = run_single(c, ref, curr, R, T, tp);
  if (rc) return rc;
  return decode_track(c->h_res[SINGLE_SLOT], R, T, err, status, info, iters);
}

static int assess_launch(revo_ctx* c, const float T_w_curr[16], const revo_pyr* curr, int* nframes_out, unsigned* seq_out) {
  *nframes_out = -1;
  if (c->past.empty() || !c->ts.check_tracking_results) return REVO_OK;
  const int hl = c->ts.histogram_level;
  if (hl < 0 || hl >= c->geom.n_levels) return fail(REVO_ERR_LEVEL, "histogram_level outside the pyramid");
  hipStream_t vs = c->vote_stream;
  TRY(wait_ready_on(c, curr, vs));
  float inv[16];
  mat4_inverse(T_w_curr, inv);
  int nframes = 0;
  VoteArgs va{};
  for (int fr = 0; fr < c->ts.n_frames_hist_voting && fr < (int)c->past.size() && fr < 3; ++fr) {
    vote_cloud_pose(inv, c->past[fr], va.RT[fr]);
    va.pts[fr] = c->past[fr].d_pts;
    va.n[fr] = c->past[fr].d_n;
    ++nframes;
  }
  const int use_orig = c->geom.lv[hl].has_orig;
  const unsigned seq = c->seq_next++;
  if (c->seq_next == 0) c->seq_next = 1;
  launch_vote(c->geom, curr->fs->p, curr->frame, hl, nframes, va, c->d_marks, c->d_hist8, c->d_vote_done, c->h_hist8, seq,
              use_orig, vs);
  HIPCHECK(hipGetLastError());
  TRY(vote_enqueued(c, curr));
  *nframes_out = nframes;
  *seq_out = seq;
  return REVO_OK;
}
static int assess_wait(revo_ctx* c, int nframes, unsigned seq, int* status, int32_t hist4[4], int32_t overlaps4[4], float* ratio_out) {
  if (status) *status = REVO_TRACKER_STATE_OK;
  if (ratio_out) *ratio_out = INFINITY;
  if (nframes < 0) return REVO_OK;
  hipStream_t vs = c->vote_stream;
  TRY(wait_seq(vs, (volatile unsigned*)(c->h_hist8 + 8), seq));
  const int* hist = c->h_hist8;
  const int* ov = c->h_hist8 + 4;
  if (hist4) memcpy(hist4, hist, sizeof(int32_t) * 4);
  if (overlaps4) memcpy(overlaps4, ov, sizeof(int32_t) * 4);
  const int st = vote_decide(ov, nframes, ratio_out);
  if (status) *status = st;
  return REVO_OK;
}

extern "C" int revo_tracker_assess_quality(revo_ctx* c, const float T_w_curr[16], const revo_pyr* curr, int* status,
                                           int32_t hist4[4], int32_t overlaps4[4]) {
  if (!c || !T_w_curr || !curr) return fail(REVO_ERR_INVALID_ARG, "null argument");
  if (curr->ctx != c) return fail(REVO_ERR_INVALID_ARG, "pyramid belongs to another context");
  if (hist4) memset(hist4, 0, sizeof(int32_t) * 4);
  if (overlaps4) memset(overlaps4, 0, sizeof(int32_t) * 4);
  if (status) *status = REVO_TRACKER_STATE_OK;
  HIPCHECK(hipSetDevice(c->device));
  std::lock_guard<std::mutex> lk(c->mu);
  int nframes = -1;
  unsigned seq = 0;
  int rc = assess_launch(c, T_w_curr, curr, &nframes, &seq);
  if (rc) return rc;
  return assess_wait(c, nframes, seq, status, hist4, overlaps4, nullptr);
}
extern "C" int revo_assess_launch_(revo_ctx* c, const float T_w_curr[16], const revo_pyr* curr, int* nframes_out, unsigned* seq_out) {
  if (!c || !T_w_curr || !curr || curr->ctx != c) return fail(REVO_ERR_INVALID_ARG, "bad argument");
  HIPCHECK(hipSetDevice(c->device));
  std::lock_guard<std::mutex> lk(c->mu);
  return assess_launch(c, T_w_curr, curr, nframes_out, seq_out);
}
extern "C" int revo_assess_wait_(revo_ctx* c, int nframes, unsigned seq, int* status, float* ratio_out) {
  if (!c) return fail(REVO_ERR_INVALID_ARG, "null context");
  return assess_wait(c, nframes, seq, status, nullptr, nullptr, ratio_out);
}

int past_take(std::vector<Past>& pool, size_t need, size_t cap, Past* out, bool newest) {
  for (size_t i = 0; i < pool.size(); ++i) {
    const size_t k = newest ? pool.size() - 1 - i : i;
    if (pool[k].cap >= need) { *out = pool[k]; pool.erase(pool.begin() + k); return REVO_OK; }
  }
  Past p{};
  p.cap = cap;
  HIPCHECK(hipMalloc((void**)&p.d_pts, sizeof(float4) * p.cap));
  hipError_t e = hipMalloc((void**)&p.d_n, sizeof(int));
  if (e != hipSuccess) { past_free(p); return fail(REVO_ERR_HIP, std::string("hipMalloc: ") + hipGetErrorString(e)); }
  *out = p;
  return REVO_OK;
}
void past_free(Past& p) { (void)hipFree(p.d_pts); (void)hipFree(p.d_n); }

extern "C" int revo_tracker_add_old_pcl(revo_ctx* c, const revo_pyr* src, int lvl, const float T_w[16], double ts) {
  if (!c || !src || !T_w) return fail(REVO_ERR_INVALID_ARG, "null argument");
  if (lvl < 0 || lvl >= c->geom.n_levels) return fail(REVO_ERR_LEVEL, "level out of range");
  HIPCHECK(hipSetDevice(c->device));
  std::lock_guard<std::mutex> lk(c->mu);
  hipStream_t vs = c->vote_stream;
// ... 83 lines not shown
```

Before: 120,200.

## Defer byte-per-pixel edge maps and read packed edge bits in build kernels

In the deferred batch path the hysteresis kernels no longer expand the edge bitmap into byte planes. Later consumers (fill, tile counting) read the packed edge bits directly. A separate k_edge_bytes kernel materializes the byte planes only when a consumer needs them (plane reads, voting, keyframe copies), guarded by a new stream mark. The batch build also stops waiting on the tracker before rebuilding and moves that wait into the deferred EDT step, so build can overlap tracking. This adds extra synchronization state and the risk of stale byte planes if some consumer misses the ensure call.

```diff
diff --git a/profiles/submit_wall.py b/profiles/submit_wall.py
--- /dev/null
+++ b/profiles/submit_wall.py
@@ -0,0 +1,67 @@
+#!/usr/bin/env python3
+import argparse
+import os
+import statistics
+import sys
+import time
+
+import numpy as np
+
+ROOT = os.path.dirname(os.path.dirname(os.path.abspath(__file__)))
+sys.path.insert(0, ROOT)
+
+
+def main():
+    ap = argparse.ArgumentParser()
+    ap.add_argument("--pairs", type=int, default=32)
+    ap.add_argument("--width", type=int, default=640)
+    ap.add_argument("--height", type=int, default=480)
+    ap.add_argument("--levels", type=int, default=4)
+    ap.add_argument("--steps", type=int, default=200)
+    ap.add_argument("--warmup", type=int, default=20)
+    ap.add_argument("--repeats", type=int, default=3)
+    a = ap.parse_args()
+    import torch
+    from revo_amd import api, synth
+    from revo_amd.settings import ImgPyramidSettings, TrackerSettings
+    s = ImgPyramidSettings.scaled(a.width, a.height, a.levels)
+    cam = api.CameraPyr(s)
+    api.TrackerNew(TrackerSettings(), s, cam)
+    base = [synth.make_pair(4000 + i, s) for i in range(4)]
+    inputs = []
+    for b in range(4):
+        pairs = [base[(b + i) % len(base)] for i in range(a.pairs)]
+        bgr = torch.from_numpy(np.stack([p[k][0] for p in pairs for k in ("ref", "curr")])).cuda()
+        dep = torch.from_numpy(np.stack([p[k][1] for p in pairs for k in ("ref", "curr")]).astype(np.float32)).cuda()
+        inputs.append((bgr, dep))
+    res = [torch.zeros(a.pairs * 96, dtype=torch.uint8, device="cuda") for _ in range(4)]
+    pipe = api.Pipeline(cam, a.pairs, depth=4)
+    n = [0]
+
+    def submit():
+        bgr, dep = inputs[n[0] % 4]
+        t0 = time.perf_counter()
+        pipe.submit(bgr.data_ptr(), dep.data_ptr(), res[n[0] % 4].data_ptr())
+        t1 = time.perf_counter()
+        n[0] += 1
+        return (t1 - t0) * 1e6
+
+    for _ in range(a.warmup):
+        submit()
+    pipe.drain()
+    print("library %s, %d pairs of %dx%dx%d, %d steps per repeat" % (os.environ.get("REVO_HIP_SO", "(shipped)"), a.pairs, a.width, a.height, a.levels, a.steps))
+    print("repeat   us/step   submit: mean   median      p90      max   share of the loop")
+    for r in range(a.repeats):
+        torch.cuda.synchronize()
+        t0 = time.perf_counter()
+        us = [submit() for _ in range(a.steps)]
+        pipe.drain()
+        wall = (time.perf_counter() - t0) * 1e6
+        us.sort()
+        print("%6d  %8.1f       %9.1f %8.1f %8.1f %8.1f   %5.1f %%" % (r, wall / a.steps, statistics.mean(us), us[len(us) // 2], us[int(len(us) * 0.9)],
+                                                                     us[-1], 100.0 * sum(us) / wall))
+    pipe.close()
+
+
+if __name__ == "__main__":
+    main()
diff --git a/revo_amd/csrc/revo_batch.hip b/revo_amd/csrc/revo_batch.hip
--- a/revo_amd/csrc/revo_batch.hip
+++ b/revo_amd/csrc/revo_batch.hip
@@ -13,6 +13,7 @@
   TRY(b->ev0.create(hipEventDefault)); TRY(b->ev1.create(hipEventDefault));
   TRY(b->descs.create());
   TRY(b->trk.create());
+  b->fs->trk_mark = &b->trk;
   b->cluster = pick_cluster(c, n_pairs);
   b->defer = env_defer();
   TRY(b->d_mail.alloc(mail_bytes(n_pairs, b->cluster) / sizeof(unsigned long long)));
@@ -46,6 +47,7 @@
     std::lock_guard<std::mutex> lk(b->fs->edt_mu);
     b->fs->edt_pending = true; b->fs->edt_count = b->n_pairs;
     b->fs->ref_lists_pending = true;
+    b->fs->edge_bytes_pending = true;
   } else {
     launch_tile_points(g, b->fs->p, b->fs->B, s);
     launch_keyframe(g, b->fs->p, 0, 2, b->n_pairs, s);
@@ -58,7 +60,7 @@
   HIPCHECK(hipSetDevice(b->ctx->device));
   hipStream_t s = stream ? (hipStream_t)stream : b->stream;
   TRY(wait_edt_before_rebuild(b->fs.get(), s));
-  TRY(batch_wait_tracker(b, s));
+  if (!b->defer) TRY(batch_wait_tracker(b, s));
   enqueue_build(b->ctx, b->fs.get(), d_bgr, d_depth, d_depth_u16, alpha, s, borrow, false, 0, -1, b->defer);
   TRY(enqueue_batch_tail(b, s));
   HIPCHECK(hipGetLastError());
@@ -226,6 +228,8 @@
   PyrGeom g = c->geom;
   g.frame0 = 0;
   FrameSet* fs = b->fs.get();
+  g.edge_bytes_lazy = b->defer ? 1 : 0;
+  fs->lazy_edge_bytes = b->defer;
   const int B = fs->B, L = g.n_levels;
   fs->p.depth[0] = const_cast<float*>(d_depth);
   struct Stage { const char* name; int a, w; };
@@ -282,6 +286,7 @@
     std::lock_guard<std::mutex> lk(fs->edt_mu);
     fs->edt_pending = false;
     fs->ref_lists_pending = false;
+    fs->edge_bytes_pending = b->defer;
     TRY(fs->edt.record(s));
     fs->ref.recorded = false;
   }
diff --git a/revo_amd/csrc/revo_dev.h b/revo_amd/csrc/revo_dev.h
--- a/revo_amd/csrc/revo_dev.h
+++ b/revo_amd/csrc/revo_dev.h
@@ -33,6 +33,7 @@
   int hyst_force;
   int hyst_heavy_runs;
   int total_tiles;
+  int edge_bytes_lazy;
   int pts_staged;
   float depth_min, depth_max;
   int canny_low, canny_high;
@@ -128,6 +129,7 @@
 void launch_canny_nms(const PyrGeom& g, const FramePlanes& p, int B, hipStream_t s);
 void launch_hyst(const PyrGeom& g, const FramePlanes& p, int B, hipStream_t s);
 void launch_fill(const PyrGeom& g, const FramePlanes& p, int B, hipStream_t s);
+void launch_edge_bytes(const PyrGeom& g, const FramePlanes& p, int B, hipStream_t s);
 void launch_compact(const PyrGeom& g, const FramePlanes& p, int B, hipStream_t s);
 void launch_tile_points(const PyrGeom& g, const FramePlanes& p, int B, hipStream_t s, int which = 3);
 void launch_pyrdown_bgr(const uint8_t* src, int w, int h, uint8_t* dst, hipStream_t s);
diff --git a/revo_amd/csrc/revo_edge_bits.h b/revo_amd/csrc/revo_edge_bits.h
--- /dev/null
+++ b/revo_amd/csrc/revo_edge_bits.h
@@ -0,0 +1,37 @@
+#pragma once
+#include <stdint.h>
+
+#if defined(__HIPCC__) || defined(__CUDACC__)
+#define EB_HD __host__ __device__ __forceinline__
+#else
+#define EB_HD inline
+#endif
+
+EB_HD uint32_t edge_bits4_to_bytes(uint32_t bits4) { return (((bits4 & 0xfu) * 0x00204081u) & 0x01010101u) * 0xffu; }
+
+template <class WordAt>
+EB_HD void edge_bytes16(WordAt word_at, int w, int wpr, int y, int x, uint32_t o[4]) {
+  if ((w & 15) == 0) {
+    const uint32_t bits = (word_at(y * wpr + (x >> 5)) >> (x & 31)) & 0xffffu;
+    for (int q = 0; q < 4; ++q) o[q] = edge_bits4_to_bytes(bits >> (4 * q));
+  } else {
+    for (int q = 0; q < 4; ++q) {
+      int xx = x + 4 * q, yy = y;
+      while (xx >= w) { xx -= w; yy += 1; }
+      o[q] = edge_bits4_to_bytes(word_at(yy * wpr + (xx >> 5)) >> (xx & 31));
+    }
+  }
+}
+
+EB_HD bool fill_gate_open(int hist_nz, int hist_w, int hist_h, float n_percentage) {
+  return (float)hist_nz / (float)(hist_w * hist_h) < n_percentage;
+}
+template <class TopAt>
+EB_HD bool fill_in_pixel(int y, int x, int finer_patch, int hist_w, int hist_h, const uint8_t* hist, double thr, TopAt top_at) {
+  const int yy = 2 * y + 1, xx = 2 * x + 1;
+  const int ty = yy / finer_patch, tx = xx / finer_patch;
+  if (ty >= hist_h || tx >= hist_w) return false;
+  return (double)hist[(size_t)ty * hist_w + tx] < thr && top_at(yy, xx);
+}
+template <class WordAt>
+EB_HD bool edge_bit(WordAt word_at, int wpr, int y, int x) { return (word_at(y * wpr + (x >> 5)) >> (x & 31)) & 1u; }
diff --git a/revo_amd/csrc/revo_frame.hip b/revo_amd/csrc/revo_frame.hip
--- a/revo_amd/csrc/revo_frame.hip
+++ b/revo_amd/csrc/revo_frame.hip
@@ -147,7 +147,7 @@
   if (!p) return fail(REVO_ERR_INVALID_ARG, "null pyramid");
   HIPCHECK(hipSetDevice(p->ctx->device));
   TRY(wait_ready(p->ctx, p));
-  if (!p->dt_ready) launch_keyframe(p->ctx->geom, p->fs->p, p->frame, 1, 1, p->ctx->stream);
+  if (!p->dt_ready) launch_keyframe(geom_of_set(p->ctx, p->fs), p->fs->p, p->frame, 1, 1, p->ctx->stream);
   HIPCHECK(hipGetLastError());
   p->dt_ready = false;
   p->is_kf = true;
@@ -159,7 +159,7 @@
   if (!p->owns_fs || p->is_kf || p->dt_ready) return REVO_OK;
   HIPCHECK(hipSetDevice(p->ctx->device));
   TRY(wait_ready(p->ctx, p));
-  launch_keyframe(p->ctx->geom, p->fs->p, p->frame, 1, 1, p->ctx->stream);
+  launch_keyframe(geom_of_set(p->ctx, p->fs), p->fs->p, p->frame, 1, 1, p->ctx->stream);
   HIPCHECK(hipGetLastError());
   p->dt_ready = true;
   return REVO_OK;
@@ -176,6 +176,7 @@
   const FramePlanes& P = p->fs->p;
   const size_t f = (size_t)p->frame;
   TRY(wait_ready(c, p));
+  if (what == REVO_PLANE_EDGES || what == REVO_PLANE_EDGES_ORIG || what == REVO_PLANE_EDGES3D) TRY(ensure_edge_bytes(c, p->fs, c->stream));
   HIPCHECK(hipStreamSynchronize(c->stream));
   const void* src = nullptr;
   size_t n = v.npix, esz = 1;
@@ -237,6 +238,7 @@
   if (!(p->owns_fs || p->has_colour) || !p->fs->d_bgr)
     return fail(REVO_ERR_INVALID_ARG, "batch views keep no colour image (rgbFullSize): use revo_pyramid_create");
   TRY(wait_ready(c, p));
+  TRY(ensure_edge_bytes(c, p->fs, c->stream));
   std::lock_guard<std::mutex> lk(c->mu);
   const PyrGeom& g = c->geom;
   const size_t n0 = g.lv[0].npix, slots = (size_t)g.lv[0].w * g.lv[0].nchunk;
@@ -279,6 +281,7 @@
   if (!(p->owns_fs || p->has_colour) || !p->fs->d_bgr)
     return fail(REVO_ERR_INVALID_ARG, "batch views keep no colour image (rgbFullSize): use revo_pyramid_create");
   TRY(wait_ready(c, p));
+  TRY(ensure_edge_bytes(c, p->fs, c->stream));
   const size_t n0 = c->geom.lv[0].npix, f = (size_t)p->frame;
   out->ctx = c;
   out->depth = p->fs->p.depth[0] + f * n0;
diff --git a/revo_amd/csrc/revo_host.hip b/revo_amd/csrc/revo_host.hip
--- a/revo_amd/csrc/revo_host.hip
+++ b/revo_amd/csrc/revo_host.hip
@@ -267,7 +267,7 @@
     TRY(fs->h_bgr.alloc((size_t)g.lv[0].npix * 3 * B));
     TRY(fs->h_depth.alloc((size_t)g.lv[0].npix * B));
   }
-  for (StreamMark* m : {&fs->ready, &fs->free_trk, &fs->free_vote, &fs->edt, &fs->ref}) TRY(m->create());
+  for (StreamMark* m : {&fs->ready, &fs->free_trk, &fs->free_vote, &fs->edt, &fs->ref, &fs->ebytes}) TRY(m->create());
   hipMemsetAsync(fs->p.npts, 0, sizeof(int) * REVO_L * B, c->stream);
   HIPCHECK(hipStreamSynchronize(c->stream));
   *out = fs.release();
@@ -279,6 +279,8 @@
   PyrGeom g = c->geom;
   g.frame0 = frame0;
   const int B = nframes < 0 ? fs->B : nframes;
+  g.edge_bytes_lazy = gray_only ? 1 : 0;
+  fs->lazy_edge_bytes = gray_only;
   fs->p.depth[0] = (borrow_depth && d_depth_f32) ? const_cast<float*>(d_depth_f32) : fs->own_depth0;
   launch_gray_depth(g, fs->p, d_bgr, d_depth_f32, d_depth_u16, alpha, B, s);
   for (int l = 1; l < g.n_levels; ++l) launch_pyrdown(g, fs->p, l, B, s, gray_only ? 1 : 3);
@@ -436,8 +438,9 @@
   } else {
     TRY(fs->ready.wait(s));
     behind_build = true;
+    if (fs->trk_mark) TRY(fs->trk_mark->wait_elsewhere(s));
     enqueue_list_side(c, fs, 1, 2, fs->edt_count, s);
-    launch_keyframe(c->geom, fs->p, 0, 2, fs->edt_count, s);
+    launch_keyframe(geom_of_set(c, fs), fs->p, 0, 2, fs->edt_count, s);
     HIPCHECK(hipGetLastError());
     TRY(fs->edt.record(s));
     fs->edt_pending = false;
@@ -454,7 +457,18 @@
 int wait_edt_before_rebuild(FrameSet* fs, hipStream_t s) {
   std::lock_guard<std::mutex> lk(fs->edt_mu);
   TRY(fs->edt.wait_elsewhere(s));
-  return fs->ref.wait_elsewhere(s);
+  TRY(fs->ref.wait_elsewhere(s));
+  return fs->ebytes.wait_elsewhere(s);
+}
+int ensure_edge_bytes(revo_ctx* c, FrameSet* fs, hipStream_t s) {
+  std::lock_guard<std::mutex> lk(fs->edt_mu);
+  if (!fs->edge_bytes_pending) return fs->ebytes.wait_elsewhere(s);
+  TRY(fs->ready.wait(s));
+  launch_edge_bytes(c->geom, fs->p, fs->B, s);
+  HIPCHECK(hipGetLastError());
+  TRY(fs->ebytes.record(s));
+  fs->edge_bytes_pending = false;
+  return REVO_OK;
 }
 int wait_event_polled(hipEvent_t ev) {
   const auto t0 = std::chrono::steady_clock::now();
diff --git a/revo_amd/csrc/revo_host_impl.h b/revo_amd/csrc/revo_host_impl.h
--- a/revo_amd/csrc/revo_host_impl.h
+++ b/revo_amd/csrc/revo_host_impl.h
@@ -34,6 +34,10 @@
   StreamMark edt;
   std::atomic<bool> ref_lists_pending{false};
   StreamMark ref;
+  bool lazy_edge_bytes = false;
+  std::atomic<bool> edge_bytes_pending{false};
+  StreamMark ebytes;
+  const StreamMark* trk_mark = nullptr;
   StreamMark free_trk;
   StreamMark free_vote;
   OwnedEvent h2d;
@@ -166,6 +170,12 @@
                    int nframes = -1, bool gray_only = false);
 int run_pending_edt(revo_ctx* c, FrameSet* fs, hipStream_t s, bool need_ref_lists = false);
 int wait_edt_before_rebuild(FrameSet* fs, hipStream_t s);
+int ensure_edge_bytes(revo_ctx* c, FrameSet* fs, hipStream_t s);
+inline PyrGeom geom_of_set(const revo_ctx* c, const FrameSet* fs) {
+  PyrGeom g = c->geom;
+  g.edge_bytes_lazy = fs->lazy_edge_bytes ? 1 : 0;
+  return g;
+}
 int decode_track(const revo_pair_result& r, float R[9], float T[3], float* err, int* status, revo_residual_info* info, int32_t* iters);
 int past_take(std::vector<Past>& pool, size_t need, size_t cap, Past* out, bool newest = false);
 void past_free(Past& p);
diff --git a/revo_amd/csrc/revo_mdev.hip b/revo_amd/csrc/revo_mdev.hip
--- a/revo_amd/csrc/revo_mdev.hip
+++ b/revo_amd/csrc/revo_mdev.hip
@@ -207,6 +207,7 @@
     if (past.empty() || !m->ts.check_tracking_results) continue;
     FrameSet* fs = (FrameSet*)v.set;
     TRY(fs->ready.wait_elsewhere(vs));
+    TRY(ensure_edge_bytes(c, fs, vs));
     VoteDesc& d = m->vdesc.h[nv];
     memset(&d, 0, sizeof(d));
     float inv[16];
@@ -285,6 +286,7 @@
   for (int i = 0; i < n; ++i) {
     FrameSet* src = (FrameSet*)f[i].set;
     TRY(src->ready.wait_elsewhere(s));
+    TRY(ensure_edge_bytes(c, src, s));
     const size_t sf = (size_t)f[i].frame, df = (size_t)f[i].stream;
     const FramePlanes& a = src->p;
     const FramePlanes& b = m->kf->p;
diff --git a/revo_amd/csrc/revo_pyramid.hip b/revo_amd/csrc/revo_pyramid.hip
--- a/revo_amd/csrc/revo_pyramid.hip
+++ b/revo_amd/csrc/revo_pyramid.hip
@@ -1,6 +1,7 @@
 #include "revo_dev.h"
 #include "revo_nms_px.h"
 #include "revo_edt_px.h"
+#include "revo_edge_bits.h"
 #include <type_traits>
 
 namespace {
@@ -332,7 +333,7 @@
 #define HP(i)
 #define HA(i)
 #endif
-template <bool C_IN_LDS, bool E_GLOBAL = false>
+template <bool C_IN_LDS, bool E_GLOBAL = false, bool LAZY = false>
 __device__ __forceinline__ void hyst_level(const PyrGeom& g, const FramePlanes& pl, const int l, const int f, uint32_t* s_mem) {
   static_assert(!(C_IN_LDS && E_GLOBAL), "the candidate bitmap is in LDS only when the edge bitmap is");
 #ifdef REVO_HYST_PROFILE
@@ -643,7 +644,7 @@
   uint8_t* orig = lv.has_orig ? pl.edges_orig[l] + (size_t)f * lv.npix : nullptr;
   const bool rows16 = (w & 15) == 0;
   const float inv_w = 1.0f / (float)w;
-  for (int i = tid; i < lv.npix / 16; i += HYST_THREADS) {
+  for (int i = tid; i < (LAZY ? 0 : lv.npix / 16); i += HYST_THREADS) {
     const int p = i * 16;
     int y = (int)(((float)p + 0.5f) * inv_w);
     y += (y + 1) * w <= p ? 1 : (y * w > p ? -1 : 0);
@@ -668,7 +669,8 @@
   }
   {
     uint2* csw = pl.cs[l] + (size_t)f * h * wpr;
-    for (int i = tid; i < nwords; i += HYST_THREADS) csw[i].y = E[pitch + i];
+    if (LAZY) for (int i = tid; i < nwords; i += HYST_THREADS) { const uint32_t e = E[pitch + i]; csw[i] = make_uint2(e, e); }
+    else for (int i = tid; i < nwords; i += HYST_THREADS) csw[i].y = E[pitch + i];
   }
   HP(6);
   if (lv.patch > 0) {
@@ -710,7 +712,7 @@
            hp[1] - hp[0], hp[5] - hp[1], ha[0], ha[1], ha[2], ha[3], ha[4], ha[5], dbg_runs, dbg_sweeps, dbg_bands, (int)done, ha[6], hp[6] - hp[5], hp[7] - hp[6], dbg_t, dbg_a);
 #endif
 }
-template <bool C_IN_LDS, bool E_GLOBAL = false>
+template <bool C_IN_LDS, bool E_GLOBAL = false, bool LAZY = false>
 __global__ void __launch_bounds__(HYST_THREADS) k_hyst(PyrGeom g, FramePlanes pl, int only_flagged, int n_frames) {
   BUILD_PRIO();
   extern __shared__ uint32_t s_mem[];
@@ -728,7 +730,7 @@
     const int l = item / n_frames;
     const int f = g.frame0 + item % n_frames;
     if (only_flagged && !pl.need_full[f * REVO_L + l]) continue;
-    hyst_level<C_IN_LDS, E_GLOBAL>(g, pl, l, f, s_mem);
+    hyst_level<C_IN_LDS, E_GLOBAL, LAZY>(g, pl, l, f, s_mem);
     __syncthreads();
   }
 }
@@ -977,6 +979,7 @@
   for (int k = 0; k < HYST_THREADS / 64; ++k) total += s_cnt[k];
   return total >= g.hyst_heavy_runs;
 }
+template <bool LAZY>
 __global__ void __launch_bounds__(HYST_THREADS) k_hyst_mixed(PyrGeom g, FramePlanes pl, int n_frames) {
   static_assert(HB_THREADS == HYST_THREADS, "one workgroup shape for both paths");
   extern __shared__ uint32_t s_mem[];
@@ -995,7 +998,7 @@
     if (threadIdx.x == 0) pl.hyst_heavy[f] = heavy ? 1 : 0;
     if (heavy) return;
   }
-  hyst_level<true>(g, pl, l, f, s_mem);
+  hyst_level<true, false, LAZY>(g, pl, l, f, s_mem);
 }
 
 #define HS_THREADS 256
@@ -1098,6 +1101,7 @@
 }
 
 #define HO_THREADS 512
+template <bool LAZY>
 __global__ void __launch_bounds__(HO_THREADS) k_hyst_out(PyrGeom g, FramePlanes pl, int mixed) {
   extern __shared__ uint32_t s_mem[];
   const int nB = gridDim.x / (mixed ? g.lv[0].nbands : g.total_bands);
@@ -1131,7 +1135,7 @@
   uint8_t* orig = lv.has_orig ? pl.edges_orig[l] + (size_t)f * lv.npix + (size_t)br.R0 * w : nullptr;
   const bool rows16 = (w & 15) == 0;
   const float inv_w = 1.0f / (float)w;
-  for (int i = tid; i < hb * w / 16; i += HO_THREADS) {
+  for (int i = tid; i < (LAZY ? 0 : hb * w / 16); i += HO_THREADS) {
     const int p = i * 16;
     int y = (int)(((float)p + 0.5f) * inv_w);
     y += (y + 1) * w <= p ? 1 : (y * w > p ? -1 : 0);
@@ -1156,7 +1160,8 @@
   }
   {
     uint2* csw = pl.cs[l] + ((size_t)f * h + br.R0) * wpr;
-    for (int i = tid; i < nwb; i += HO_THREADS) csw[i].y = E[i];
+    if (LAZY) for (int i = tid; i < nwb; i += HO_THREADS) csw[i] = make_uint2(E[i], E[i]);
+    else for (int i = tid; i < nwb; i += HO_THREADS) csw[i].y = E[i];
   }
   if (lv.patch > 0) {
     const int ty0 = br.R0 / lv.patch, ty1 = min(lv.hist_h, br.R1 / lv.patch);
@@ -1191,25 +1196,43 @@
   for (int l = la; l < lb; ++l) {
     const LevelGeom lv = g.lv[l], lf = g.lv[l - 1];
     if (!(g.use_edge_hist && lv.patch > 0 && lf.patch > 0)) continue;
-    const float frac = (float)pl.hist_nz[f * REVO_L + l] / (float)(lv.hist_w * lv.hist_h);
-    if (frac < g.n_percentage) {
-      const uint8_t* top = pl.edges[l - 1] + (size_t)f * lf.npix;
-      uint8_t* mod = pl.edges[l] + (size_t)f * lv.npix;
+    if (fill_gate_open(pl.hist_nz[f * REVO_L + l], lv.hist_w, lv.hist_h, g.n_percentage)) {
+      const uint2* top = pl.cs[l - 1] + (size_t)f * lf.h * lf.wpr;
+      uint2* modw = pl.cs[l] + (size_t)f * lv.h * lv.wpr;
+      uint8_t* mod = g.edge_bytes_lazy ? nullptr : pl.edges[l] + (size_t)f * lv.npix;
       const uint8_t* hist = pl.hist[l] + (size_t)f * lv.hist_w * lv.hist_h;
       const double thr = g.fill_thr[l];
       const int cw = lf.w / 2, ch = lf.h / 2;
       for (int i = blockIdx.x * 1024 + threadIdx.x; i < cw * ch; i += gridDim.x * 1024) {
         const int y = i / cw, x = i % cw;
-        const int yy = 2 * y + 1, xx = 2 * x + 1;
-        const int ty = yy / lf.patch, tx = xx / lf.patch;
-        if (ty >= lv.hist_h || tx >= lv.hist_w) continue;
-        if ((double)hist[(size_t)ty * lv.hist_w + tx] < thr && top[(size_t)yy * lf.w + xx] > 0) {
-          mod[(size_t)y * lv.w + x] = 255;
-          atomicOr(&(pl.cs[l] + (size_t)f * lv.h * lv.wpr)[(size_t)y * lv.wpr + (x >> 5)].y, 1u << (x & 31));
+        if (fill_in_pixel(y, x, lf.patch, lv.hist_w, lv.hist_h, hist, thr, [&](int yy, int xx) {
+              return edge_bit([&](int k) { return top[k].y; }, lf.wpr, yy, xx); })) {
+          if (mod) mod[(size_t)y * lv.w + x] = 255;
+          atomicOr(&modw[(size_t)y * lv.wpr + (x >> 5)].y, 1u << (x & 31));
         }
       }
     }
     __syncthreads();
+  }
+}
+
+__global__ void __launch_bounds__(256) k_edge_bytes(PyrGeom g, FramePlanes pl) {
+  const int P = (blockIdx.x * 256 + threadIdx.x) * 16;
+  if (P >= g.total_pix) return;
+  const int f = g.frame0 + blockIdx.y;
+  const int l = level_of(g, P, &LevelGeom::pix_base);
+  const LevelGeom& lv = g.lv[l];
+  const int p = P - lv.pix_base;
+  int y = (int)(((float)p + 0.5f) * (1.0f / (float)lv.w));
+  y += (y + 1) * lv.w <= p ? 1 : (y * lv.w > p ? -1 : 0);
+  const int x = p - y * lv.w;
+  const uint2* csw = pl.cs[l] + (size_t)f * lv.h * lv.wpr;
+  uint32_t o[4];
+  edge_bytes16([&](int k) { return csw[k].y; }, lv.w, lv.wpr, y, x, o);
+  *reinterpret_cast<uint4*>(pl.edges[l] + (size_t)f * lv.npix + p) = make_uint4(o[0], o[1], o[2], o[3]);
+  if (lv.has_orig) {
+    edge_bytes16([&](int k) { return csw[k].x; }, lv.w, lv.wpr, y, x, o);
+    *reinterpret_cast<uint4*>(pl.edges_orig[l] + (size_t)f * lv.npix + p) = make_uint4(o[0], o[1], o[2], o[3]);
   }
 }
 
@@ -1726,14 +1749,16 @@
   const bool in = x < lv.w;
   const uint8_t* edges = pl.edges[l] + (size_t)f * lv.npix;
   unsigned em = 0;
-  if ((lv.w & 31) == 0 && (ncols & 31) == 0) {
-    const uint2* csw = pl.cs[l] + (size_t)f * lv.h * lv.wpr;
+  const uint2* csw = pl.cs[l] + (size_t)f * lv.h * lv.wpr;
+  if (((lv.w & 31) == 0 || g.edge_bytes_lazy) && (ncols & 31) == 0) {
     const int r = threadIdx.x & 31;
     const int wc = (sidx * ncols + (col & ~31)) >> 5;
     uint32_t v = 0;
     if (yb + r < ye && wc < lv.wpr) v = csw[(size_t)(yb + r) * lv.wpr + wc].y;
     em = tile_transpose32(v, r);
     if (!in) em = 0;
+  } else if (in && g.edge_bytes_lazy) {
+    for (int y = yb; y < ye; ++y) em |= ((csw[(size_t)y * lv.wpr + (x >> 5)].y >> (x & 31)) & 1u) << (y - yb);
   } else if (in) {
 #pragma unroll 8
     for (int y = yb; y < ye; ++y) em |= (edges[(size_t)y * lv.w + x] ? 1u : 0u) << (y - yb);
@@ -1983,7 +2008,8 @@
   hipLaunchKernelGGL(k_canny_nms4, dim3(g.total_nms_blocks, 1, B), dim3(256), 0, s, g, p);
 }
 
-void launch_hyst(const PyrGeom& g, const FramePlanes& p, int B, hipStream_t s) {
+template <bool LAZY>
+static void launch_hyst_t(const PyrGeom& g, const FramePlanes& p, int B, hipStream_t s) {
   size_t e_bytes = 0, ec_bytes = 0;
   for (int l = 0; l < g.n_levels; ++l) {
     const size_t nw = (size_t)g.lv[l].h * g.lv[l].wpr;
@@ -1993,8 +2019,8 @@
   }
   static bool attr_set = false;
   if (!attr_set) {
-    (void)hipFuncSetAttribute(reinterpret_cast<const void*>(k_hyst<true>), hipFuncAttributeMaxDynamicSharedMemorySize, REVO_HYST_LDS_MAX);
-    (void)hipFuncSetAttribute(reinterpret_cast<const void*>(k_hyst<false>), hipFuncAttributeMaxDynamicSharedMemorySize, REVO_HYST_LDS_MAX);
+    (void)hipFuncSetAttribute(reinterpret_cast<const void*>(k_hyst<true, false, LAZY>), hipFuncAttributeMaxDynamicSharedMemorySize, REVO_HYST_LDS_MAX);
+    (void)hipFuncSetAttribute(reinterpret_cast<const void*>(k_hyst<false, false, LAZY>), hipFuncAttributeMaxDynamicSharedMemorySize, REVO_HYST_LDS_MAX);
     attr_set = true;
   }
   const int force = g.hyst_force;
@@ -2005,7 +2031,7 @@
     static bool attr2 = false;
     if (!attr2) {
       (void)hipFuncSetAttribute(reinterpret_cast<const void*>(k_hyst_band), hipFuncAttributeMaxDynamicSharedMemorySize, HB_LDS_WORDS * 4);
-      (void)hipFuncSetAttribute(reinterpret_cast<const void*>(k_hyst_out), hipFuncAttributeMaxDynamicSharedMemorySize, HB_LDS_WORDS * 4);
+      (void)hipFuncSetAttribute(reinterpret_cast<const void*>(k_hyst_out<LAZY>), hipFuncAttributeMaxDynamicSharedMemorySize, HB_LDS_WORDS * 4);
       (void)hipFuncSetAttribute(reinterpret_cast<const void*>(k_hyst_seam), hipFuncAttributeMaxDynamicSharedMemorySize, 64 * 1024);
       (void)hipGetLastError();
       attr2 = true;
@@ -2019,14 +2045,14 @@
     }
     hipLaunchKernelGGL(k_hyst_band, dim3(g.total_bands * B), dim3(HB_THREADS), HB_LDS_WORDS * 4, s, g, p);
     if (g.any_banded) hipLaunchKernelGGL(k_hyst_seam, dim3(g.n_levels * B), dim3(HS_THREADS), seam_lds, s, g, p, 0);
-    hipLaunchKernelGGL(k_hyst_out, dim3(g.total_bands * B), dim3(HO_THREADS), out_lds, s, g, p, 0);
+    hipLaunchKernelGGL(k_hyst_out<LAZY>, dim3(g.total_bands * B), dim3(HO_THREADS), out_lds, s, g, p, 0);
   }
   const bool mixed = !banded && fits_single && g.hyst_heavy_runs > 0 && g.total_bands > 0 && g.lv[0].nbands > 1;
   if (mixed) {
     static bool attr3 = false;
     if (!attr3) {
-      (void)hipFuncSetAttribute(reinterpret_cast<const void*>(k_hyst_mixed), hipFuncAttributeMaxDynamicSharedMemorySize, REVO_HYST_LDS_MAX);
-      (void)hipFuncSetAttribute(reinterpret_cast<const void*>(k_hyst_out), hipFuncAttributeMaxDynamicSharedMemorySize, HB_LDS_WORDS * 4);
+      (void)hipFuncSetAttribute(reinterpret_cast<const void*>(k_hyst_mixed<LAZY>), hipFuncAttributeMaxDynamicSharedMemorySize, REVO_HYST_LDS_MAX);
+      (void)hipFuncSetAttribute(reinterpret_cast<const void*>(k_hyst_out<LAZY>), hipFuncAttributeMaxDynamicSharedMemorySize, HB_LDS_WORDS * 4);
       (void)hipFuncSetAttribute(reinterpret_cast<const void*>(k_hyst_seam), hipFuncAttributeMaxDynamicSharedMemorySize, 64 * 1024);
       (void)hipGetLastError();
       attr3 = true;
@@ -2034,19 +2060,24 @@
     const LevelGeom& l0 = g.lv[0];
     const size_t seam_lds = std::max<size_t>(4, (size_t)l0.nbands * (size_t)(HB_LDS_WORDS / 2 / 32 + 64) * 4);
     const size_t out_lds = std::max<size_t>(4, (size_t)l0.band_rows * l0.wpr * 4);
-    hipLaunchKernelGGL(k_hyst_mixed, dim3((l0.nbands + g.n_levels) * B), dim3(HYST_THREADS), REVO_HYST_LDS_MAX, s, g, p, B);
+    hipLaunchKernelGGL(k_hyst_mixed<LAZY>, dim3((l0.nbands + g.n_levels) * B), dim3(HYST_THREADS), REVO_HYST_LDS_MAX, s, g, p, B);
     hipLaunchKernelGGL(k_hyst_seam, dim3(B), dim3(HS_THREADS), seam_lds, s, g, p, 1);
-    hipLaunchKernelGGL(k_hyst_out, dim3(l0.nbands * B), dim3(HO_THREADS), out_lds, s, g, p, 1);
-    hipLaunchKernelGGL(k_hyst<true>, dim3(std::min(32, g.n_levels * B)), dim3(HYST_THREADS), REVO_HYST_LDS_MAX, s, g, p, 1, B);
+    hipLaunchKernelGGL(k_hyst_out<LAZY>, dim3(l0.nbands * B), dim3(HO_THREADS), out_lds, s, g, p, 1);
+    hipLaunchKernelGGL((k_hyst<true, false, LAZY>), dim3(std::min(32, g.n_levels * B)), dim3(HYST_THREADS), REVO_HYST_LDS_MAX, s, g, p, 1, B);
     return;
   }
   const int n_wg = only_flagged ? std::min(32, g.n_levels * B) : g.n_levels * B;
   if (ec_bytes + 4096 <= REVO_HYST_LDS_MAX)
-    hipLaunchKernelGGL(k_hyst<true>, dim3(n_wg), dim3(HYST_THREADS), REVO_HYST_LDS_MAX, s, g, p, only_flagged, B);
+    hipLaunchKernelGGL((k_hyst<true, false, LAZY>), dim3(n_wg), dim3(HYST_THREADS), REVO_HYST_LDS_MAX, s, g, p, only_flagged, B);
   else if (e_bytes <= REVO_HYST_LDS_MAX)
-    hipLaunchKernelGGL(k_hyst<false>, dim3(n_wg), dim3(HYST_THREADS), e_bytes, s, g, p, only_flagged, B);
+    hipLaunchKernelGGL((k_hyst<false, false, LAZY>), dim3(n_wg), dim3(HYST_THREADS), e_bytes, s, g, p, only_flagged, B);
   else
-    hipLaunchKernelGGL((k_hyst<false, true>), dim3(n_wg), dim3(HYST_THREADS), 16, s, g, p, only_flagged, B);
+    hipLaunchKernelGGL((k_hyst<false, true, LAZY>), dim3(n_wg), dim3(HYST_THREADS), 16, s, g, p, only_flagged, B);
+}
+
+void launch_hyst(const PyrGeom& g, const FramePlanes& p, int B, hipStream_t s) {
+  if (g.edge_bytes_lazy) launch_hyst_t<true>(g, p, B, s);
+  else launch_hyst_t<false>(g, p, B, s);
 }
 
 void launch_fill(const PyrGeom& g, const FramePlanes& p, int B, hipStream_t s) {
@@ -2062,6 +2093,10 @@
     const int n = (g.lv[l - 1].w / 2) * (g.lv[l - 1].h / 2);
     hipLaunchKernelGGL(k_fill, dim3(std::min(64, (n + 1023) / 1024), 1, B), dim3(1024), 0, s, g, p, l);
   }
+}
+
+void launch_edge_bytes(const PyrGeom& g, const FramePlanes& p, int B, hipStream_t s) {
+  hipLaunchKernelGGL(k_edge_bytes, dim3((g.total_pix / 16 + 255) / 256, B), dim3(256), 0, s, g, p);
 }
 
 void launch_tile_points(const PyrGeom& g, const FramePlanes& p, int B, hipStream_t s, int which) {
diff --git a/revo_amd/csrc/revo_single.hip b/revo_amd/csrc/revo_single.hip
--- a/revo_amd/csrc/revo_single.hip
+++ b/revo_amd/csrc/revo_single.hip
@@ -148,6 +148,7 @@
   if (hl < 0 || hl >= c->geom.n_levels) return fail(REVO_ERR_LEVEL, "histogram_level outside the pyramid");
   hipStream_t vs = c->vote_stream;
   TRY(wait_ready_on(c, curr, vs));
+  TRY(ensure_edge_bytes(c, curr->fs, vs));
   float inv[16];
   mat4_inverse(T_w_curr, inv);
   int nframes = 0;
```

After: 122,500 (median of 6 runs). 1.02x the previous value.
